# seqan/slimm

Hardware: AMD Instinct MI355X
Metric: M alignment-records/sec -> final profile (higher is better)
Workload: dtype u32

## Files before the change

include/slimm_hip.h:

```cpp
#ifndef SLIMM_HIP_H
#define SLIMM_HIP_H

#include <stddef.h>
#include <stdint.h>

#ifdef __cplusplus
extern "C" {
#endif

#define SLIMM_LINEAGE_LEN 8

enum {
    SLIMM_OK = 0,
    SLIMM_E_INVALID = -1,
    SLIMM_E_HIP = -2,
    SLIMM_E_REF_RANGE = -3,
    SLIMM_E_RUN_LENGTH = -4,
    SLIMM_E_KEY_COLLISION = -5,
    SLIMM_E_REGROUP = -6,
    SLIMM_E_SPLIT = -7,
    SLIMM_E_RETRY = 2,
    SLIMM_E_NO_HITS = 1
};

// ... 141 lines not shown
int slimm_write_abundance(slimm_ctx* ctx, const char** text, uint64_t* len);
int slimm_write_abundance_file(slimm_ctx* ctx, const char* path);

typedef struct {
    uint32_t hits_count, matches_count, uniq_matches_count, uniq_hits_count, uniq_matches_count2;
    uint32_t reference_count, matched_ref_length;
    uint32_t failed_by_cov, failed_by_uniq_cov, failed_by_min_read, n_valid;
    uint32_t bin_width, min_reads, avg_read_len;
    uint32_t profile_count, profile_failed;
    float coverage_cut_off, uniq_coverage_cut_off, expected_coverage;
    uint64_t n_records, n_targets;
    uint64_t total_bins;
} slimm_stats;
int slimm_get_stats(slimm_ctx* ctx, slimm_stats* out);

typedef struct {
    uint32_t* reads_count;
    uint32_t* uniq_reads_count;
    uint32_t* uniq_reads_count2;
    uint32_t* nbins;
    uint32_t* nz_cov;
    uint32_t* nz_uniq_cov;
    uint32_t* nz_uniq_cov2;
    uint8_t* valid;
    float* abundance;
    float* uniq_abundance;
} slimm_ref_columns;
int slimm_get_ref_columns(slimm_ctx* ctx, slimm_ref_columns* out);

int slimm_get_bins(slimm_ctx* ctx, int which, uint32_t* out);

int slimm_get_read_targets(slimm_ctx* ctx, uint32_t* ref, uint32_t* gbin, uint64_t cap, uint64_t* n);
int slimm_target_ref_bits(slimm_ctx* ctx);

int slimm_taxon_count_size(slimm_ctx* ctx, int stage, uint32_t* n);
int slimm_get_taxon_counts(slimm_ctx* ctx, int stage, uint32_t* taxid, uint32_t* count);
int slimm_children_pairs_size(slimm_ctx* ctx, int stage, uint64_t* n);
int slimm_get_children_pairs(slimm_ctx* ctx, int stage, uint32_t* taxid, uint32_t* ref);

int slimm_enable_kernel_timing(slimm_ctx* ctx, int on);
int slimm_time_only_kernel(slimm_ctx* ctx, const char* name);
int slimm_kernel_times(slimm_ctx* ctx, const char** names, double* ms, uint32_t* launches, uint32_t cap,
                       uint32_t* n, int reset);

int slimm_get_bucket_sampling(slimm_ctx* ctx, uint32_t out[6]);

int slimm_grouped_records(slimm_ctx* ctx, uint64_t* ident, uint32_t* ref, uint32_t* gbin, uint64_t cap, uint64_t* n);
void slimm_group_plan(uint64_t n_records, uint32_t* passes, uint32_t* width, uint32_t* bits, uint32_t* grid);

uint32_t slimm_host_avg_read_length(const uint32_t* l_seq, uint64_t n, uint32_t sample_size);
float slimm_host_quantile_cut_off(const float* v, uint32_t n, float q);
uint32_t slimm_host_bin_of(int32_t begin_pos, uint32_t avg_read_len, uint32_t ref_len, uint32_t bin_width);
uint32_t slimm_host_canonical_read_name(const char* name, uint32_t name_len, uint16_t flag, uint16_t* flag_out);
typedef struct slimm_q18_runs {
    uint64_t short_starts;
    uint64_t short_to_plain;
    int last_short;
} slimm_q18_runs;
void slimm_host_q18_note(slimm_q18_runs* q, int starts_run, int shortened);
int slimm_host_q18_regroup_needed(const slimm_q18_runs* q);
int slimm_get_q18_runs(slimm_ctx* ctx, uint64_t* short_starts, uint64_t* short_to_plain);
typedef struct slimm_record_filter {
    uint32_t min_mapq;
    uint32_t require_flags;
    uint32_t exclude_flags;
    uint32_t min_aligned;
// ... 59 lines not shown
```

slimm_amd/capi.py:

```python
from __future__ import annotations

import ctypes as C
import os

_HERE = os.path.dirname(os.path.abspath(__file__))
LIB_PATH = os.environ.get("SLIMM_HIP_LIB") or os.path.join(_HERE, "libslimm_hip.so")

OK = 0
E_INVALID = -1
E_HIP = -2
E_REF_RANGE = -3
E_RUN_LENGTH = -4
E_KEY_COLLISION = -5
E_REGROUP = -6
E_SPLIT = -7
E_RETRY = 2
E_NO_HITS = 1

ORDER_GROUPED = 0
ORDER_ANY = 1

PROPAGATION_INDEPENDENT = 0
PROPAGATION_DEPENDENT = 1
PROPAGATION_UNDECIDED = 2
# ... 98 lines not shown
    ("slimm_staging_buffers", C.c_int, [_P, C.c_uint32, C.c_uint64, C.POINTER(_P), C.POINTER(_P), C.POINTER(_P),
                                        C.POINTER(_P)]),
    ("slimm_push_staged_async", C.c_int, [_P, C.c_uint32, C.c_uint64]),
    ("slimm_staging_wait", C.c_int, [_P, C.c_uint32]),
    ("slimm_set_records_device", C.c_int, [_P, _P, _P, _P, _P, C.c_uint64]),
    ("slimm_analyze_alignments", C.c_int, [_P]),
    ("slimm_coverage_buffer", C.c_int, [_P, C.POINTER(_P), C.POINTER(C.c_uint64)]),
    ("slimm_prepare_summary", C.c_int, [_P, C.c_uint32]),
    ("slimm_keep_bins", C.c_int, [_P, C.c_int]),
    ("slimm_coverage_summary", C.c_int, [_P, C.POINTER(_P), C.POINTER(C.c_uint64)]),
    ("slimm_finish_coverage_merged", C.c_int, [_P, _P, C.c_uint32]),
    ("slimm_merge_summary_slices", C.c_int, [_P, _P, C.c_uint32, C.c_uint32, C.POINTER(_P), C.POINTER(C.c_uint64)]),
    ("slimm_finish_coverage_reduced", C.c_int, [_P]),
    ("slimm_finish_coverage", C.c_int, [_P]),
    ("slimm_set_coverage_columns", C.c_int, [_P, _P, _P, _P, _P, C.c_uint32, C.c_uint32]),
    ("slimm_filter_alignments", C.c_int, [_P]),
    ("slimm_dense_taxa", C.c_int, [_P, C.POINTER(C.c_uint32), C.POINTER(_P)]),
    ("slimm_get_partials", C.c_int, [_P, C.POINTER(Partials)]),
    ("slimm_set_partials", C.c_int, [_P, C.POINTER(Partials)]),
    ("slimm_partials_buffer", C.c_int, [_P, C.POINTER(_P), C.POINTER(C.c_uint64)]),
    ("slimm_install_merged_partials", C.c_int, [_P, C.POINTER(C.c_uint32)]),
    ("slimm_get_reads_lca_count", C.c_int, [_P]),
    ("slimm_get_propagation_order", C.c_int, [_P, C.POINTER(C.c_int), _P, C.c_uint32, C.POINTER(C.c_uint32)]),
    ("slimm_set_propagation_walk", C.c_int, [_P, C.c_int]),
    ("slimm_set_propagation_priority", C.c_int, [_P, _P, C.c_uint32]),
    ("slimm_get_profiles", C.c_int, [_P, C.c_char_p]),
    ("slimm_write_abundance", C.c_int, [_P, C.POINTER(C.c_char_p), C.POINTER(C.c_uint64)]),
    ("slimm_write_abundance_file", C.c_int, [_P, C.c_char_p]),
    ("slimm_get_stats", C.c_int, [_P, C.POINTER(Stats)]),
    ("slimm_get_ref_columns", C.c_int, [_P, C.POINTER(RefColumns)]),
    ("slimm_get_bins", C.c_int, [_P, C.c_int, _P]),
    ("slimm_get_read_targets", C.c_int, [_P, _P, _P, C.c_uint64, C.POINTER(C.c_uint64)]),
    ("slimm_target_ref_bits", C.c_int, [_P]),
    ("slimm_get_bucket_sampling", C.c_int, [_P, _P]),
    ("slimm_taxon_count_size", C.c_int, [_P, C.c_int, C.POINTER(C.c_uint32)]),
    ("slimm_get_taxon_counts", C.c_int, [_P, C.c_int, _P, _P]),
    ("slimm_children_pairs_size", C.c_int, [_P, C.c_int, C.POINTER(C.c_uint64)]),
    ("slimm_get_children_pairs", C.c_int, [_P, C.c_int, _P, _P]),
    ("slimm_enable_kernel_timing", C.c_int, [_P, C.c_int]),
    ("slimm_time_only_kernel", C.c_int, [_P, C.c_char_p]),
    ("slimm_kernel_times", C.c_int, [_P, C.POINTER(C.c_char_p), C.POINTER(C.c_double), C.POINTER(C.c_uint32),
                                     C.c_uint32, C.POINTER(C.c_uint32), C.c_int]),
    ("slimm_push_bam_bytes", C.c_int, [_P, _P, C.c_uint64, C.c_int, C.POINTER(C.c_uint64)]),
    ("slimm_push_bgzf_blocks", C.c_int, [_P, _P, C.c_uint64, C.c_uint32, C.c_int, C.POINTER(C.c_uint64)]),
    ("slimm_push_sam_bytes", C.c_int, [_P, _P, C.c_uint64, C.c_int, C.POINTER(C.c_uint64)]),
    ("slimm_push_bgzf_sam_blocks", C.c_int, [_P, _P, C.c_uint64, C.c_uint32, C.c_int, C.POINTER(C.c_uint64)]),
    ("slimm_push_bzip2_sam_bytes", C.c_int, [_P, _P, C.c_uint64, C.c_uint32, C.c_int, C.POINTER(C.c_uint64)]),
    ("slimm_push_gzip_sam_bytes", C.c_int, [_P, _P, C.c_uint64, C.c_uint32, C.c_int, C.POINTER(C.c_uint64)]),
    ("slimm_get_gzip_stats", C.c_int, [_P, C.POINTER(C.c_uint64)]),
    ("slimm_push_zstd_sam_bytes", C.c_int, [_P, _P, C.c_uint64, C.c_uint32, C.c_int, C.POINTER(C.c_uint64)]),
    ("slimm_get_zstd_stats", C.c_int, [_P, C.POINTER(C.c_uint64)]),
    ("slimm_push_xz_sam_bytes", C.c_int, [_P, _P, C.c_uint64, C.c_uint32, C.c_int, C.POINTER(C.c_uint64)]),
    ("slimm_get_xz_stats", C.c_int, [_P, C.POINTER(C.c_uint64)]),
    ("slimm_set_reference_names", C.c_int, [_P, C.POINTER(C.c_char_p)]),
    ("slimm_bgzf_inflate", C.c_int, [C.c_int, _P, C.c_uint64, _P, C.c_uint64, C.POINTER(C.c_uint64), C.POINTER(C.c_double), C.c_char_p, C.c_uint64]),
    ("slimm_bgzf_inflate_with", C.c_int, [C.c_int, _P, C.c_uint64, _P, C.c_uint64, C.POINTER(C.c_uint64), C.POINTER(C.c_double), C.c_char_p,
                                          C.c_uint64, C.c_uint32, C.POINTER(C.c_uint32)]),
    ("slimm_partition_by_key", C.c_int, [C.c_int, _P, _P, _P, _P, _P, C.c_uint64, C.c_uint32, _P, _P, _P, _P, _P, _P, C.POINTER(C.c_double),
                                         C.c_char_p, C.c_uint64]),
    ("slimm_records_device", C.c_int, [_P, _P, _P, _P, _P, C.POINTER(C.c_uint64), C.POINTER(C.c_int)]),
    ("slimm_pin_host_buffer", C.c_int, [_P, _P, C.c_uint64]),
    ("slimm_set_input_size_hint", C.c_int, [_P, C.c_uint64]),
    ("slimm_window_memory", C.c_int, [_P, C.POINTER(C.c_uint64)]),
    ("slimm_device_memory", C.c_int, [_P, C.POINTER(C.c_uint64), C.POINTER(C.c_uint64)]),
    ("slimm_group_plan", None, [C.c_uint64, C.POINTER(C.c_uint32), C.POINTER(C.c_uint32), C.POINTER(C.c_uint32),
                                C.POINTER(C.c_uint32)]),
# ... 56 lines not shown
```

slimm_amd/csrc/context.h:

```cpp
#pragma once
#include <cerrno>
#include <fcntl.h>
#include <hip/hip_runtime.h>
#include <unistd.h>

#include <algorithm>
#include <cstdarg>
#include <cstdio>
#include <cstdlib>
#include <chrono>
#include <cstring>
#include <functional>
#include <memory>
#include <string>
#include <vector>

#include "../../include/slimm_hip.h"
#include "host_profile.hpp"
#include "force.h"
#include "bzip2_block.h"
#include "deflate_stream.h"
#include "zstd_walk.h"
#include "xz_walk.h"
#include "kernels.h"
#include "read_identity.h"

namespace slimm {



extern thread_local std::string g_create_error;

template <typename T>
struct DevBuf {
    T* p = nullptr;
    size_t cap = 0;
    ~DevBuf() { release(); }
    void release() {
        if (p) (void)hipFree(p);
        p = nullptr;
        cap = 0;
    }
    hipError_t ensure(size_t n) {
        if (n <= cap) return hipSuccess;
        release();
        hipError_t e = hipMalloc(reinterpret_cast<void**>(&p), n * sizeof(T));
        if (e == hipSuccess) cap = n;
        return e;
    }
    hipError_t ensure_later(size_t n, std::vector<void*>& old) {
        return n <= cap ? hipSuccess : grow_keeping(n, 0, 0, nullptr, false, &old);
    }
    hipError_t grow_keeping(size_t n, size_t from, size_t count, hipStream_t st, bool sync, std::vector<void*>* old) {
        DevBuf<T> nb;
        hipError_t e = nb.ensure(n);
        if (e == hipSuccess && count) e = hipMemcpyAsync(nb.p + from, p + from, count * sizeof(T), hipMemcpyDeviceToDevice, st);
        if (e == hipSuccess && sync) e = hipStreamSynchronize(st);
// ... 57 lines not shown
    bool copy_pending = false;
    bool filter_pending = false;
    bool stream_ordered = false;
    struct Staging {
        PinBuf<uint64_t> key;
        PinBuf<int32_t> ref, pos;
        PinBuf<uint16_t> flag;
        hipEvent_t done = nullptr;
        bool pending = false;
    } staging[2];

    uint32_t R = 0, T = 0;
    TileBucketing tiles;
    uint64_t Bp() const { return tiles.layout.Bp; }
    bool use_tiles() const { return tiles.plan.use_tiles; }
    std::vector<uint32_t> bin_off_h;

    DevBuf<uint32_t> d_ref_len, d_bin_off, d_lin_dense;
    DevBuf<uint2> d_geo;
    DevBuf<uint8_t> d_valid;
    DevBuf<uint4> d_rows16;
    DevBuf<uint32_t> d_level_taxon;
    DevBuf<uint32_t> d_taxon_off, d_taxon_idx;
    uint32_t taxon_shift = 0;
    uint32_t Tsel = 0;
    PinBuf<uint4> h_rows16;
    DevBuf<uint32_t> d_valid_bits;
    PinBuf<uint32_t> h_valid_bits;
    std::vector<uint32_t> valid_bits_prev;
    bool rows16_base_ready = false;
    std::vector<uint32_t> rows16_prev;
    bool use_rows16 = false;
    bool ref16 = false;
    DevBuf<uint64_t> in_key;
    DevBuf<int32_t> in_ref, in_pos;
    DevBuf<uint16_t> in_flag;
    DevBuf<uint32_t> in_check;
    bool has_check = false;
    bool packed = false;
    bool marked = false;
    WindowPipeline win;
    std::vector<slimm_ctx*> filter_peers;
    DeviceRecords rec;
    bool borrowed = false;
    uint64_t n_pushed = 0;
    DevBuf<uint64_t> c_ident, s_ident;
    DevBuf<uint2> c_pay, s_pay;
    DevBuf<uint32_t> group_hist, c_chk, s_chk;
    DevBuf<uint32_t> tgt_ref, tgt_gbin;
    TargetRefs target_refs() const { return TargetRefs{tgt_ref.p, ref16}; }
    DevBuf<uint4> slots;
    bool keep_bins = true;
    bool binsA_stored = false, binsB_stored = false;
    DevBuf<uint32_t> sel;
    DevBuf<uint32_t> filter_redo;
    DevBuf<uint32_t> slot_rbase, slot_bbase;
    hipStream_t side_stream = nullptr;
    hipEvent_t front_done = nullptr, prefix_done = nullptr;
    bool prefix_pending = false;
    uint32_t summary_slices = 0;
    bool summary_has_bits = false;
    uint32_t summary_layout = 0xffffffffu;
    DevBuf<uint32_t> d_sum_vec;
    uint32_t slice_tiles() const { return summary_slices > 1 ? (tiles.layout.ntiles + summary_slices - 1) / summary_slices : tiles.layout.ntiles; }
    uint64_t slice_words() const { return static_cast<uint64_t>(slice_tiles()) * (tiles.layout.tile_bins() / 32); }
    uint64_t summary_words() const { return 4ull * R + 16 + 2ull * std::max<uint32_t>(summary_slices, 1u) * slice_words(); }
    BitsLayout bits_layout() {
        BitsLayout b;
        if (summary_has_bits) {
            b.base = reinterpret_cast<uint64_t*>(summary.p + 4ull * R + 16);
            b.tps = slice_tiles();
            b.slice_w64 = slice_words() / 2;
        }
        return b;
    }
    bool statsA_final = false;
    bool bins_exposed = false;
    DevBuf<uint32_t> bins;
    DevBuf<uint32_t> counters;
    DevBuf<uint32_t> ref_stats;
    DevBuf<uint32_t> summary;
    DevBuf<uint32_t> lca_count, marks;
    DevBuf<uint32_t> d_partials;
// ... 117 lines not shown
```

slimm_amd/csrc/context.hip:

```cpp
#define SLIMM_RF_HOST_API
#include "context.h"

namespace slimm {

thread_local std::string g_create_error;
const char* kKernelNames[K_COUNT] = {"memset_bins", "k_group_count", "k_group_scan", "k_group_scatter", "k_group_finish",
                                     "k_front", "k_hist", "k_ref_stats", "k_filter", "k_ref_stats2",
                                     "k_tile_count", "k_tile_scan", "k_tile_scatter", "k_tile_hist",
                                     "k_tile_count2", "k_tile_scan2", "k_tile_scatter2", "k_tile_hist2",
                                     "k_pack", "k_pack2"};

int fail(slimm_ctx* c, int code, const char* fmt, ...) {
    char buf[512];
    va_list ap;
    va_start(ap, fmt);
    vsnprintf(buf, sizeof(buf), fmt, ap);
    va_end(ap);
    if (c)
        c->err = buf;
    else
        g_create_error = buf;
    return code;
}



void drain_events(slimm_ctx* c) {
    bool unrecorded = false;
    for (auto& e : c->ev_used) {
        float ms = 0.f;
        if (hipEventSynchronize(e.b) == hipSuccess && hipEventElapsedTime(&ms, e.a, e.b) == hipSuccess) {
            c->k_ms[e.id] += ms;
            c->k_n[e.id] += 1;
        } else {
            unrecorded = true;
        }
        c->ev_free.push_back(e);
    }
    c->ev_used.clear();
    if (unrecorded) (void)hipGetLastError();
}

int ensure_work_buffers(slimm_ctx* c, uint32_t n) {
    HIP_TRY(c, c->tgt_ref.ensure(n + 1));
    HIP_TRY(c, c->tgt_gbin.ensure(n + 8));
    HIP_TRY(c, c->slots.ensure(front_slots(n) + 1));
    HIP_TRY(c, c->sel.ensure(n + 8));
    HIP_TRY(c, c->slot_rbase.ensure(front_slots(n) + 8));
    HIP_TRY(c, c->slot_bbase.ensure(front_slots(n) / 1024 + 8));
    HIP_TRY(c, c->filter_redo.ensure(front_slots(n) + 1));
    HIP_TRY(c, c->tiles.reserve(n));
    if (c->order == SLIMM_ORDER_ANY) {
        HIP_TRY(c, c->c_ident.ensure(n + 1));
        HIP_TRY(c, c->c_pay.ensure(n + 1));
        HIP_TRY(c, c->s_ident.ensure(n + 1));
        HIP_TRY(c, c->s_pay.ensure(n + 1));
        HIP_TRY(c, c->group_hist.ensure(group_hist_words(group_plan(n))));
        if (c->rec.check) {
            HIP_TRY(c, c->c_chk.ensure(n + 1));
            HIP_TRY(c, c->s_chk.ensure(n + 1));
        }
    }
    return SLIMM_OK;
}

int ensure_pair_table(slimm_ctx* c, uint32_t cap) {
    if (cap <= c->pair_cap) return SLIMM_OK;
    HIP_TRY(c, c->pair_tab.ensure(cap));
    HIP_TRY(c, c->pair_list.ensure(cap / 2 + 1));
    HIP_TRY(c, c->h_pairs.ensure(cap / 2 + 1));
    c->pair_cap = cap;
    return SLIMM_OK;
}



int check_device_errors(slimm_ctx* c, uint32_t err) {
// ... 60 lines not shown
    c->host.reset(new HostProfile(hc));
    c->R = cfg->n_refs;
    c->T = c->host->n_taxa_dense();
    c->device = cfg->device;
    c->order = cfg->record_order;
    c->bin_off_h.resize(c->R + 1);
    uint64_t off = 0;
    for (uint32_t r = 0; r < c->R; ++r) {
        c->bin_off_h[r] = static_cast<uint32_t>(off);
        off += (static_cast<uint64_t>(c->host->nbins()[r]) + 3) & ~3ull;
        if (off >= kMaxBins) return fail(nullptr, SLIMM_E_INVALID, "more than 2^31 coverage bins; use a larger bin width");
    }
    c->bin_off_h[c->R] = static_cast<uint32_t>(off);
    {
        long r16 = 1;
        (void)forced("ref16", &r16);
        c->ref16 = c->R <= kRef16Max && r16 != 0;
    }
    {
        c->use_rows16 = c->host->rows16_ok() && !forced("wide_rows");
        c->Tsel = c->T;
        if (c->use_rows16) {
            const uint32_t* loff = c->host->level_offset();
            uint32_t widest = 1;
            for (int l = 0; l < 8; ++l) widest = std::max(widest, loff[l + 1] - loff[l]);
            c->taxon_shift = 0;
            while ((1u << c->taxon_shift) < widest) ++c->taxon_shift;
            c->Tsel = 8u << c->taxon_shift;
        }
    }
    const TileForces forces = TileForces::from_env();
    const TileLayout& tl = c->tiles.layout = tile_layout(off, c->Tsel, forces.tile_shift);
    if (tl.Bp + tl.Tpad >= kMaxBins) return fail(nullptr, SLIMM_E_INVALID, "more than 2^31 coverage bins; use a larger bin width");

    if (c->device >= 0) {
        slimm_ctx* cc = c.get();
        int ndev = 0;
        hipError_t e = hipGetDeviceCount(&ndev);
        if (e != hipSuccess || ndev == 0)
            return fail(nullptr, SLIMM_E_HIP, "no HIP device available (%s)", hipGetErrorString(e));
        if (c->device >= ndev) return fail(nullptr, SLIMM_E_INVALID, "device %d out of range (%d devices)", c->device, ndev);
#define HIP_TRY0(expr)                                                                                   \
    do {                                                                                                 \
        hipError_t e_ = (expr);                                                                          \
        if (e_ != hipSuccess) return fail(nullptr, SLIMM_E_HIP, "%s: %s", #expr, hipGetErrorString(e_)); \
    } while (0)
        HostTrace trc("slimm_create");
        HIP_TRY0(hipSetDevice(c->device));
        HIP_TRY0(hipStreamCreateWithFlags(&cc->stream, hipStreamNonBlocking));
        HIP_TRY0(hipEventCreateWithFlags(&cc->front_done, hipEventDisableTiming));
        HIP_TRY0(hipEventCreateWithFlags(&cc->prefix_done, hipEventDisableTiming));
        HIP_TRY0(hipEventCreateWithFlags(&cc->copy_done, hipEventDisableTiming));
        for (auto& sg : cc->staging) HIP_TRY0(hipEventCreateWithFlags(&sg.done, hipEventDisableTiming));
        trc.mark("streams + events");
        HIP_TRY0(cc->d_ref_len.ensure(c->R));
        HIP_TRY0(cc->d_bin_off.ensure(c->R + 1));
        HIP_TRY0(cc->d_lin_dense.ensure(static_cast<size_t>(c->R) * 8));
        HIP_TRY0(cc->d_valid.ensure(c->R));
        HIP_TRY0(cc->d_valid_bits.ensure(c->R / 32 + 2));
        HIP_TRY0(cc->h_valid_bits.ensure(c->R / 32 + 2));
        memset(cc->h_valid_bits.p, 0, (c->R / 32 + 2) * 4);
        HIP_TRY0(cc->bins.ensure(3 * tl.Bp + kTailWords + tl.Tpad));
        HIP_TRY0(cc->counters.ensure(CNT_WORDS));
        HIP_TRY0(cc->ref_stats.ensure(c->statsA_words() + c->statsB_words() + 64));
        HIP_TRY0(cc->lca_count.ensure(c->Tsel));
        HIP_TRY0(cc->marks.ensure(static_cast<size_t>(c->R) * (kMarkBytes / 4)));
        trc.mark("device arrays");
        HIP_TRY0(cc->h_stats.ensure(c->statsA_words() + c->statsB_words() + 64));
        HIP_TRY0(cc->h_small.ensure(CNT_WORDS + kTailWords));
        HIP_TRY0(cc->h_lca.ensure(c->T));
        HIP_TRY0(cc->h_marks.ensure(c->R));
        trc.mark("page-locked host arrays");
        HIP_TRY0(hipMemcpy(cc->d_ref_len.p, hc.ref_len.data(), c->R * 4, hipMemcpyHostToDevice));
        HIP_TRY0(hipMemcpy(cc->d_bin_off.p, c->bin_off_h.data(), (c->R + 1) * 4, hipMemcpyHostToDevice));
        {
            std::vector<uint2> geo(c->R);
            for (uint32_t i = 0; i < c->R; ++i) geo[i] = make_uint2(hc.ref_len[i], static_cast<uint32_t>(c->bin_off_h[i]));
            HIP_TRY0(cc->d_geo.ensure(c->R));
            HIP_TRY0(hipMemcpy(cc->d_geo.p, geo.data(), c->R * sizeof(uint2), hipMemcpyHostToDevice));
        }
        HIP_TRY0(hipMemcpy(cc->d_lin_dense.p, c->host->lineage_dense().data(), static_cast<size_t>(c->R) * 32,
                           hipMemcpyHostToDevice));
#undef HIP_TRY0
        if (cc->use_rows16) {
            const std::vector<uint32_t>& lt = c->host->level_taxon();
            const uint32_t* off = c->host->level_offset();
            std::vector<uint32_t> flat(static_cast<size_t>(8) << cc->taxon_shift, 0u);
            std::vector<uint32_t> inv_off(c->T + 1, 0u), inv_idx;
            for (int l = 0; l < 8; ++l)
                for (uint32_t i = off[l]; i < off[l + 1]; ++i) {
                    flat[(static_cast<size_t>(i - off[l]) << 3) | static_cast<size_t>(l)] = lt[i];
                    if (lt[i] < c->T) ++inv_off[lt[i] + 1];
                }
// ... 222 lines not shown
            {
                KernelTimer t(c, K_GROUP_SCAN);
                launch_group_scan(st, j, pass);
            }
            {
                KernelTimer t(c, K_GROUP_SCATTER);
                launch_group_scatter(st, j, pass);
            }
        }
        {
            KernelTimer t(c, K_GROUP_FINISH);
            launch_group_finish(st, j);
        }
        {
            KernelTimer t(c, K_FRONT);
            launch_front_sorted(st, n, c->c_ident.p, c->c_pay.p, c->counters.p, c->target_refs(), c->tgt_gbin.p, c->slots.p,
                                c->rec.check ? c->c_chk.p : nullptr);
        }
    } else {
        KernelTimer t(c, K_FRONT, true);
        launch_front_raw(st, c->rec, c->R, c->d_geo.p, half_read, hc.bin_width, c->counters.p, c->target_refs(), c->tgt_gbin.p,
                         c->slots.p, t.t0(), t.t1());
    }
    auto slot_prefix_beside_what_follows = [&]() -> int {
        HIP_TRY(c, need_stream(c->side_stream));
        HIP_TRY(c, hipEventRecord(c->front_done, st));
        HIP_TRY(c, hipStreamWaitEvent(c->side_stream, c->front_done, 0));
        launch_slot_read_prefix(c->side_stream, c->slots.p, nslots, c->slot_rbase.p, c->slot_bbase.p);
        HIP_TRY(c, hipEventRecord(c->prefix_done, c->side_stream));
        return SLIMM_OK;
    };
    if (c->use_tiles()) {
        job.values.vals = c->tgt_gbin.p;
        job.values.slots = c->slots.p;
        job.values.nslots = nslots;
        job.n_upper = n;
        job.a = c->cov();
        job.b = c->ucov();
        job.tail = c->tail();
        job.stats = c->ref_stats.p;
        job.store_from = c->keep_bins ? 0u : c->tiles.layout.ntiles;
        bucket(c, job);
        if (int rc = slot_prefix_beside_what_follows()) return rc;
        c->summary_has_bits = false;
        if (c->summary_slices) {
            const bool fresh = c->summary.cap < c->summary_words() || c->summary_layout != c->summary_slices;
            HIP_TRY(c, c->summary.ensure(c->summary_words()));
            if (fresh)
                HIP_TRY(c, hipMemsetAsync(c->summary.p, 0, c->summary_words() * 4, st));
            c->summary_layout = c->summary_slices;
            c->summary_has_bits = true;
        }
        job.bits = c->bits_layout();
        histogram(c, job);
        c->binsA_stored = c->keep_bins;
    } else {
        if (int rc = slot_prefix_beside_what_follows()) return rc;
        KernelTimer t(c, K_HIST);
        launch_hist(st, c->tgt_gbin.p, c->slots.p, nslots, c->counters.p, c->tail(), c->cov(), c->ucov(),
                    c->order != SLIMM_ORDER_ANY);
        c->binsA_stored = true;
    }
    c->prefix_pending = true;
    HIP_TRY(c, hipGetLastError());
    c->analyzed = true;
    tr.mark("phase A launches");
    return SLIMM_OK;
}

int slimm_get_stream(slimm_ctx* c, void** hip_stream) {
    if (!c || !hip_stream) return SLIMM_E_INVALID;
    if (c->device < 0) return fail(c, SLIMM_E_INVALID, "host-only context has no stream");
    *hip_stream = c->stream;
    return SLIMM_OK;
}

int slimm_set_stream_ordered(slimm_ctx* c, int on) {
    if (!c) return SLIMM_E_INVALID;
    c->stream_ordered = on != 0;
    return SLIMM_OK;
}

int slimm_coverage_buffer(slimm_ctx* c, void** d_ptr, uint64_t* n_words) {
    if (!c || !d_ptr || !n_words) return SLIMM_E_INVALID;
    if (!c->analyzed) return fail(c, SLIMM_E_INVALID, "call slimm_analyze_alignments first");
    if (!c->binsA_stored) return fail(c, SLIMM_E_INVALID, "the coverage arrays were not kept (slimm_keep_bins)");
    (void)hipSetDevice(c->device);
    if (!c->stream_ordered) HIP_TRY(c, hipStreamSynchronize(c->stream));
    c->bins_exposed = true;
    *d_ptr = c->bins.p;
    *n_words = 2 * c->Bp() + 16;
    return SLIMM_OK;
}
// ... 217 lines not shown
    const uint32_t R = c->R, T = c->T;
    uint32_t* const blockB = c->ref_stats.p + c->statsA_words();
    TileJob job;
    job.run = c->tiles.run(TilePhase::B, c->local_M, c->rec.n);
    {
        KernelTimer t(c, K_MEMSET);
        if (!c->use_tiles()) HIP_TRY(c, hipMemsetAsync(c->ucov2(), 0, c->Bp() * sizeof(uint32_t), st));
        ZeroArgs z;
        z.p[0] = c->marks.p;
        z.n[0] = R * (kMarkBytes / 4);
        z.p[1] = c->counters.p + CNT_ERR;
        z.n[1] = 3;
        if (c->use_tiles()) {
            z.p[2] = blockB;
            z.n[2] = 4 * R;
            c->tiles.zero_tables(z, job.run);
        } else {
            z.p[2] = c->lca_count.p;
            z.n[2] = c->Tsel;
        }
        if (!c->pair_clean) {
            z.p64 = c->pair_tab.p;
            z.n64 = c->pair_cap;
        }
        if (copy_rows) {
            z.cp_dst = reinterpret_cast<uint32_t*>(c->d_rows16.p);
            z.cp_src = reinterpret_cast<const uint32_t*>(c->h_rows16.p);
            z.cp_n = R * 4u;
        }
        z.cp2_dst = c->d_valid_bits.p;
        z.cp2_src = c->h_valid_bits.p;
        z.cp2_n = R / 32u + 1u;
        launch_zero(st, z);
    }
    const uint32_t nslots = front_slots(c->rec.n);
    HIP_TRY(c, hipStreamWaitEvent(st, c->prefix_done, 0));
    c->prefix_pending = false;
    {
        KernelTimer t(c, K_FILTER, true);
        FilterArgs fa;
        fa.tgt_ref = c->target_refs();
        fa.tgt_gbin = c->tgt_gbin.p;
        fa.slots = c->slots.p;
        fa.nslots = nslots;
        if (c->use_rows16) {
            fa.rows16 = c->d_rows16.p;
            fa.taxon_flat = c->d_level_taxon.p;
            fa.taxon_shift = c->taxon_shift;
        } else {
            fa.lin_dense = c->d_lin_dense.p;
            fa.valid = c->d_valid.p;
        }
        fa.valid_bits = c->d_valid_bits.p;
        fa.redo = c->filter_redo.p;
        fa.sel = c->sel.p;
        fa.slot_rbase = c->slot_rbase.p;
        fa.slot_bbase = c->slot_bbase.p;
        fa.marks = c->marks.p;
        fa.pair_tab = c->pair_tab.p;
        fa.pair_list = c->pair_list.p;
        fa.pair_mask = c->pair_cap - 1;
        fa.taxon_base = static_cast<uint32_t>(c->Bp());
        fa.counters = c->counters.p;
        launch_filter(st, fa, t.t0(), t.t1());
    }
    if (c->use_tiles()) {
        job.values.vals = c->sel.p;
        job.values.nslots = c->local_M;
        job.n_upper = c->rec.n;
        job.a = c->ucov2();
        job.stats = blockB;
        job.store_from = c->keep_bins ? 0u : c->tiles.layout.ntiles;
        bucket(c, job);
        histogram(c, job);
    } else {
        KernelTimer t(c, K_HIST);
        launch_sel_atomics(st, c->sel.p, c->local_M, static_cast<uint32_t>(c->Bp()), c->ucov2(), c->lca_count.p);
    }
    {
        PackArgs pk;
        pk.src[0] = c->counters.p;
        pk.n[0] = 32;
        pk.src[1] = c->marks.p;
        pk.n[1] = R;
        pk.reps[1] = kPackBytes8;
        pk.src[2] = c->use_tiles() ? c->lca_tiles() : c->lca_count.p;
        pk.n[2] = T;
        if (c->use_rows16) {
            pk.sum_k = 2;
            pk.sum_off = c->d_taxon_off.p;
            pk.sum_idx = c->d_taxon_idx.p;
        }
        if (c->use_tiles()) {
            KernelTimer t(c, K_PACK2);
            const TileTables tt = c->tiles.tables(c->counters.p);
            TILES(tt.tile_shift, launch_pack(st, blockB + 4ull * R, pk, &tt, c->ucov2(), nullptr, c->d_bin_off.p, R, blockB));
        } else {
            KernelTimer t(c, K_REF_STATS2);
            launch_ref_stats(st, c->ucov2(), nullptr, c->d_bin_off.p, R, blockB, &pk);
        }
// ... 314 lines not shown
    if (!c || !out || which < 0 || which > 2) return SLIMM_E_INVALID;
    if (c->device < 0 || !c->analyzed) return fail(c, SLIMM_E_INVALID, "no coverage bins on this context");
    if (which == 2 && !c->filtered) return fail(c, SLIMM_E_INVALID, "uniq_cov2 needs slimm_filter_alignments");
    if (which < 2 ? !c->binsA_stored : !c->binsB_stored)
        return fail(c, SLIMM_E_INVALID, "the coverage arrays were not kept (slimm_keep_bins)");
    (void)hipSetDevice(c->device);
    const uint32_t* src = which == 0 ? c->cov() : which == 1 ? c->ucov() : c->ucov2();
    std::vector<uint32_t> padded(c->Bp());
    HIP_TRY(c, hipMemcpyAsync(padded.data(), src, c->Bp() * 4, hipMemcpyDeviceToHost, c->stream));
    HIP_TRY(c, hipStreamSynchronize(c->stream));
    uint64_t k = 0;
    for (uint32_t r = 0; r < c->R; ++r) {
        uint32_t nb = c->host->nbins()[r];
        memcpy(out + k, padded.data() + c->bin_off_h[r], static_cast<size_t>(nb) * 4);
        k += nb;
    }
    return SLIMM_OK;
}

int slimm_get_read_targets(slimm_ctx* c, uint32_t* ref, uint32_t* gbin, uint64_t cap, uint64_t* n) {
    if (!c || !n) return SLIMM_E_INVALID;
    if (c->device < 0 || !c->analyzed) return fail(c, SLIMM_E_INVALID, "no targets on this context (call slimm_analyze_alignments)");
    (void)hipSetDevice(c->device);
    const uint32_t ns = front_slots(c->rec.n);
    std::vector<uint4> sl(ns);
    if (ns) HIP_TRY(c, hipMemcpyAsync(sl.data(), c->slots.p, ns * sizeof(uint4), hipMemcpyDeviceToHost, c->stream));
    HIP_TRY(c, hipStreamSynchronize(c->stream));
    uint64_t total = 0;
    for (const uint4& d : sl) total += d.y;
    *n = total;
    if (!ref && !gbin) return SLIMM_OK;
    if (cap < total) return fail(c, SLIMM_E_INVALID, "slimm_get_read_targets: %llu entries, room for %llu",
                                 static_cast<unsigned long long>(total), static_cast<unsigned long long>(cap));
    std::vector<uint16_t> ref16(ref && c->ref16 ? total : 0);
    uint64_t o = 0;
    for (const uint4& d : sl) {
        if (!d.y) continue;
        if (ref && c->ref16)
            HIP_TRY(c, hipMemcpyAsync(ref16.data() + o, reinterpret_cast<const uint16_t*>(c->tgt_ref.p) + d.x, d.y * 2ull,
                                      hipMemcpyDeviceToHost, c->stream));
        else if (ref)
            HIP_TRY(c, hipMemcpyAsync(ref + o, c->tgt_ref.p + d.x, d.y * 4ull, hipMemcpyDeviceToHost, c->stream));
        if (gbin) HIP_TRY(c, hipMemcpyAsync(gbin + o, c->tgt_gbin.p + d.x, d.y * 4ull, hipMemcpyDeviceToHost, c->stream));
        o += d.y;
    }
    HIP_TRY(c, hipStreamSynchronize(c->stream));
    if (ref && c->ref16)
        for (uint64_t k = 0; k < total; ++k) ref[k] = (ref16[k] & 0x7fffu) | ((ref16[k] & 0x8000u) << 16);
    return SLIMM_OK;
}

int slimm_target_ref_bits(slimm_ctx* c) { return c ? (c->ref16 ? 16 : 32) : SLIMM_E_INVALID; }

int slimm_get_bucket_sampling(slimm_ctx* c, uint32_t out[6]) {
    if (!c || !out) return SLIMM_E_INVALID;
    uint32_t cnt[CNT_WORDS] = {0};
    for (int i = 0; i < 6; ++i) out[i] = 0;
    if (c->device < 0) return SLIMM_OK;
    HIP_TRY(c, hipSetDevice(c->device));
    HIP_TRY(c, hipStreamSynchronize(c->stream));
    if (c->counters.p) HIP_TRY(c, hipMemcpy(cnt, c->counters.p, sizeof(cnt), hipMemcpyDeviceToHost));
    for (int ph = 0; ph < 2; ++ph) {
        const uint32_t S = c->use_tiles() ? c->tiles.sampled[ph] : 0u;
        out[3 * ph] = S;
        out[3 * ph + 1] = S > 1 ? cnt[CNT_FALLBACK + ph] : 0u;
        out[3 * ph + 2] = S > 1 ? cnt[CNT_PEAK + ph] : 0u;
    }
    return SLIMM_OK;
}

int slimm_taxon_count_size(slimm_ctx* c, int stage, uint32_t* n) {
    if (!c || !n) return SLIMM_E_INVALID;
    if (!c->counted) return fail(c, SLIMM_E_INVALID, "call slimm_get_reads_lca_count first");
    std::vector<uint32_t> t, k;
    c->host->taxon_counts(stage, t, k);
    *n = static_cast<uint32_t>(t.size());
    return SLIMM_OK;
}

int slimm_get_taxon_counts(slimm_ctx* c, int stage, uint32_t* taxid, uint32_t* count) {
    if (!c || !taxid || !count) return SLIMM_E_INVALID;
    if (!c->counted) return fail(c, SLIMM_E_INVALID, "call slimm_get_reads_lca_count first");
    std::vector<uint32_t> t, k;
    c->host->taxon_counts(stage, t, k);
    memcpy(taxid, t.data(), t.size() * 4);
// ... 164 lines not shown
```

slimm_amd/csrc/front.hip:

```cpp
#include <hip/hip_runtime.h>
#include <hip/hip_ext.h>
#include <stdint.h>

#include <algorithm>
#include <cstdlib>

#include "kernels.h"

namespace slimm {

#if defined(EXP) && EXP == 11
__device__ unsigned long long g_prof_f[4 * 8192];
#define FPROF_T(x) const unsigned long long x = __builtin_readcyclecounter()
#define FPROF_ADD(slot, a, b) if (threadIdx.x == 0) atomicAdd(&g_prof_f[(blockIdx.x & 8191u) * 4 + slot], (b) - (a))
#else
#define FPROF_T(x)
#define FPROF_ADD(slot, a, b)
#endif

namespace {

constexpr uint32_t kTagShift = 26;
constexpr uint32_t kRefField = (1u << kTagShift) - 1u;
constexpr uint32_t kNoMatch = 0xffffffffu;
// ... 290 lines not shown
        o.mapped = w.b != 0xffffffffu;
        if (o.mapped && w.b >= n_refs) {
            bad = true;
            o.mapped = false;
        }
        o.ref = w.b;
        o.aux = w.c;
        return o;
    }
    __device__ FrontRec rec(uint32_t i, bool& bad) const { return decode(raw(i), bad); }
    __device__ uint2 geo_of(const FrontRaw3& w) const { return geo[w.b < n_refs ? w.b : 0u]; }
    __device__ uint32_t gbin(const FrontRec& r, const uint2& g) const { return g.y + div_bin_width(min(r.aux + half_read, g.x)); }
};

namespace {

struct WinOut {
    uint32_t base;
    uint32_t nf, nh, nv;
};

struct Staged {
    uint32_t mate, ref, gbin;
    bool mapped;
};

#ifndef SLIMM_HASH_WALK
#define SLIMM_HASH_WALK 32
#endif
constexpr uint32_t kHashWalk = SLIMM_HASH_WALK;
static_assert(kHashWalk == 16 || kHashWalk == 24 || kHashWalk == 32 || kHashWalk == 48,
              "the threshold is one of the distances window_fast's doubling chain knows");

template <typename RefT>
__device__ __forceinline__ void window_fast(uint32_t field, uint32_t gbin, uint32_t lane, uint64_t SS, uint64_t V, uint64_t PR,
                                            WinOut& so, RefT* __restrict__ tgt_ref, uint32_t* __restrict__ tgt_gbin,
                                            uint32_t* tab) {
    const uint32_t T = (f_rank(SS >> 1) << kTagShift) | field;
    const uint64_t N0 = SS ^ PR;
    const uint64_t E2 = N0 & (N0 << 1), E4 = E2 & (E2 << 2), E8 = E4 & (E4 << 4), E12 = E8 & (E8 << 4), E16 = E8 & (E8 << 8);
    const uint64_t E24 = E16 & (E16 << 8), E32 = E16 & (E16 << 16), E48 = E32 & (E32 << 16);
    uint64_t F;
    if ((kHashWalk == 16 ? E16 : kHashWalk == 24 ? E24 : kHashWalk == 32 ? E32 : E48) != 0ull) {
        hash_clear(tab, lane);
        bool overflow = false;
        F = f_ballot(hash_first(tab, T, lane, f_bit(V), overflow));
    } else {
        const uint32_t x1 = f_shr1z(T) ^ T;
        uint32_t x = x1, differ = x1;
        const auto walk = [&](int steps) {
#pragma unroll
            for (int u = 0; u < steps; ++u) {
                x = f_shr1z(x) ^ x1;
                differ = min(differ, x);
            }
        };
        if (E2) {
            walk(2);
            if (E4) {
                walk(4);
                if (E8) {
                    walk(4);
                    if (E12) {
                        walk(4);
                        if (kHashWalk > 16 && E16) {
                            walk(8);
                            if (kHashWalk > 24 && E24) {
                                walk(8);
                                if (kHashWalk > 32 && E32) walk(16);
                            }
                        }
                    }
                }
            }
        }
        F = f_ballot(differ != 0u) & V;
    }
    const uint64_t H = f_first_after(SS, V, SS >> 1);
    const uint64_t Fr = __builtin_bitreverse64(F), Gr = __builtin_bitreverse64(F & ~H);
    const uint64_t U = H & ~__builtin_bitreverse64((~Fr + (Gr << 1)) & Fr);
    const bool uniq = f_bit(U);
    if (f_bit(F)) {
        const uint32_t p = so.base + so.nf + f_rank(F);
        tgt_ref[p] = static_cast<RefT>((field - 1u) + f_head_bit<RefT>(f_bit(H)));
        tgt_gbin[p] = gbin | (uniq ? 0x80000000u : 0u);
    }
    so.nf += static_cast<uint32_t>(__popcll(F));
    so.nh += static_cast<uint32_t>(__popcll(H));
    so.nv += static_cast<uint32_t>(__popcll(V));
}

template <typename RefT>
__device__ __forceinline__ void window_general(const Staged& rec, uint32_t lane, uint64_t RS, uint64_t V, uint32_t X,
                                               WinOut& so, RefT* __restrict__ tgt_ref,
                                               uint32_t* __restrict__ tgt_gbin) {
    const bool in_pr = lane < X;
    const bool use = f_bit(V);
    const uint64_t le = (2ull << lane) - 1ull;
    const uint32_t run_from = 63u - static_cast<uint32_t>(__builtin_clzll((RS & le) | 1ull));
    const uint64_t above = RS & ~le;
    const uint32_t run_to = above ? static_cast<uint32_t>(__builtin_ctzll(above)) : X;
    const uint32_t W = use ? ((rec.mate << 28) | rec.ref) : (0xc0000000u | lane);
    const uint32_t back = in_pr ? lane - run_from : 0u;
    bool dup = false, mate_seen = false;
    for (uint32_t d = 1; f_ballot(back >= d) != 0ull; ++d) {
        const uint32_t o = __shfl(W, static_cast<int>((lane - d) & 63u), 64);
        const bool mine = back >= d;
        dup = dup || (mine && o == W);
        mate_seen = mate_seen || (mine && (o >> 28) == (W >> 28));
    }
    const bool first = use && !dup;
    const bool head = use && !mate_seen;
    const uint32_t WF = first ? (W >> 28) : 3u;
    const uint32_t span = in_pr ? run_to - run_from : 0u;
    uint32_t smaller = 0, same_before = 0, same_total = 0;
    for (uint32_t d = 0; f_ballot(span > d) != 0ull; ++d) {
        const uint32_t j = run_from + d;
        const uint32_t o = __shfl(WF, static_cast<int>(j & 63u), 64);
        const bool mine = span > d && o != 3u && first;
        smaller += (mine && o < WF) ? 1u : 0u;
        same_total += (mine && o == WF) ? 1u : 0u;
        same_before += (mine && o == WF && j < lane) ? 1u : 0u;
    }
    const uint64_t F = f_ballot(first);
    const uint64_t H = f_ballot(head);
    if (first) {
        const uint32_t before_run = static_cast<uint32_t>(__popcll(F & ((1ull << run_from) - 1ull)));
        const uint32_t p = so.base + so.nf + before_run + smaller + same_before;
        tgt_ref[p] = static_cast<RefT>(rec.ref | f_head_bit<RefT>(head));
        tgt_gbin[p] = rec.gbin | ((head && same_total == 1u) ? 0x80000000u : 0u);
    }
    so.nf += static_cast<uint32_t>(__popcll(F));
    so.nh += static_cast<uint32_t>(__popcll(H));
    so.nv += static_cast<uint32_t>(__popcll(V));
}

template <bool kChk, typename Acc, typename RefT>
__device__ __forceinline__ uint32_t long_run(const Acc& acc, uint32_t pos, uint32_t N, uint32_t lane, WinOut& so,
                                          RefT* __restrict__ tgt_ref, uint32_t* __restrict__ tgt_gbin, bool& bad,
                                          bool& collide, uint32_t* tab) {
    uint32_t klo0, khi0;
    acc.key_at(pos, klo0, khi0);
    uint32_t end = pos;
    bool decreasing = false;
    uint32_t last_mate = 0;
    while (true) {
        const uint32_t i = end + lane;
        const bool live = i < N;
        bool b = false;
        const bool mine = acc.same_run(live ? i : N - 1u, pos, klo0, khi0);
        const FrontRec r = acc.rec(live ? i : N - 1u, b);
        const uint64_t same = f_ballot(live && mine);
        if (kChk) collide = collide | (live && mine && acc.check[i] != acc.check[pos]);
        const uint32_t n_same = static_cast<uint32_t>(__builtin_ctzll(~same | (1ull << 63)));
        const bool whole = (~same) == 0ull;
        const uint32_t n_in = whole ? 64u : n_same;
        const uint32_t mprev = f_shr1(r.mate, last_mate);
        decreasing = decreasing || (f_ballot(r.mate < mprev) & f_below(n_in)) != 0ull;
        if (n_in) last_mate = __builtin_amdgcn_readlane(r.mate, n_in - 1u);
        end += n_in;
        if (!whole) break;
    }
    const WinOut so_at_run = so;
    bool hashed = true;
    uint32_t nv_run;
    bool again;
    do {
        again = false;
        so = so_at_run;
        nv_run = 0;
// ... 24 lines not shown
                        uint32_t Ts = T;
                        for (uint32_t d = 1; d < 64u; ++d) {
                            Ts = f_shr1(Ts, kNoMatch);
                            differ = min(differ, Ts ^ T);
                        }
                    }
                    for (uint32_t eb = pos; eb < cb; eb += 64u) {
                        bool b = false;
                        const FrontRec e = acc.rec(eb + lane, b);
                        uint32_t Te = e.mapped ? ((e.mate << 28) | e.ref) : 0xe0000000u;
                        for (uint32_t d = 0; d < 64u; ++d) {
                            differ = min(differ, Te ^ T);
                            Te = f_ror1(Te);
                        }
                    }
                    first = use && differ != 0u;
                }
                const uint64_t F = f_ballot(first);
                uint64_t H = 0;
#pragma unroll
                for (uint32_t m = 0; m < 3u; ++m) {
                    const uint64_t Vm = f_ballot(use && r.mate == m);
                    if (Vm && !((head_seen >> m) & 1u)) {
                        H |= 1ull << __builtin_ctzll(Vm);
                        head_seen |= 1u << m;
                    }
                    n_first[m] += static_cast<uint32_t>(__popcll(f_ballot(first && r.mate == m)));
                }
                const bool head = f_bit(H);
                const uint32_t p = so.base + so.nf + f_rank(F);
                const FrontRaw3 rw{0u, first ? r.ref : 0u, 0u};
                const uint32_t g = first ? acc.gbin(r, acc.geo_of(rw)) : 0u;
                if (first) {
                    tgt_ref[p] = static_cast<RefT>(r.ref | f_head_bit<RefT>(head));
                    if (!head) tgt_gbin[p] = g;
                }
                uint64_t Hm = H;
                while (Hm) {
                    const uint32_t hl = static_cast<uint32_t>(__builtin_ctzll(Hm));
                    Hm &= Hm - 1ull;
                    const uint32_t m = __builtin_amdgcn_readlane(r.mate, hl);
                    head_p[m] = __builtin_amdgcn_readlane(p, hl);
                    head_g[m] = __builtin_amdgcn_readlane(g, hl);
                }
                so.nf += static_cast<uint32_t>(__popcll(F));
                so.nh += static_cast<uint32_t>(__popcll(H));
            }
            if (!again) {
#pragma unroll
                for (uint32_t m = 0; m < 3u; ++m)
                    if (((head_seen >> m) & 1u) && lane == 0u)
                        tgt_gbin[head_p[m]] = head_g[m] | (n_first[m] == 1u ? 0x80000000u : 0u);
            }
        }
    } while (again);
    so.nv += nv_run;
    return end;
}

constexpr uint32_t kStageRecs = 64u * kSlotBlocks;
constexpr uint32_t kStageGroup = 6;

__device__ __forceinline__ uint32_t next_run_start(const uint32_t* st1, uint32_t lane, uint32_t from) {
    for (uint32_t o = from; o < kStageRecs; o += 64u) {
        const uint32_t i = o + lane;
        const uint32_t w = i < kStageRecs ? st1[i] : 0u;
        const uint64_t m = f_ballot(static_cast<int32_t>(w) < 0);
        if (m) return o + static_cast<uint32_t>(__builtin_ctzll(m));
    }
    return kStageRecs;
}

template <typename RefT>
__device__ __forceinline__ bool long_run_staged(const uint32_t* st1, const uint32_t* st2, uint32_t off, uint32_t end_off,
                                                uint32_t lane, WinOut& so, RefT* __restrict__ tgt_ref,
                                                uint32_t* __restrict__ tgt_gbin, uint32_t* tab) {
    const WinOut so_at_run = so;
    {
        uint32_t head_seen = 0, last_mate = 0, nv = 0;
        uint32_t n_first[3] = {0u, 0u, 0u}, head_p[3] = {0u, 0u, 0u}, head_g[3] = {0u, 0u, 0u};
        bool falls = false;
        hash_clear(tab, lane);
        for (uint32_t o = off; o < end_off; o += 64u) {
            const uint32_t i = o + lane;
            const uint32_t n_in = min(64u, end_off - o);
            const uint32_t at = min(i, end_off - 1u);
            const uint32_t w1 = st1[at], g = st2[at];
            const uint32_t field = w1 & kRefField, mate = (w1 >> kStMateShift) & 3u;
            const uint64_t IN = f_below_nz(n_in);
            if ((f_ballot(mate < f_shr1(mate, last_mate)) & IN) != 0ull) {
                falls = true;
                break;
            }
            last_mate = __builtin_amdgcn_readlane(mate, n_in - 1u);
            const uint64_t V = f_ballot(field != kRefField) & IN;
            bool overflow = false;
            const bool first = hash_first(tab, (mate << 28) | field, i - off, f_bit(V), overflow);
            if (f_ballot(overflow) != 0ull) {
                so = so_at_run;
                return false;
            }
            const uint64_t F = f_ballot(first);
            const uint64_t M1 = f_ballot(mate == 1u), M2 = f_ballot(mate == 2u);
            const uint64_t Mm[3] = {~(M1 | M2), M1, M2};
            uint64_t H = 0;
#pragma unroll
            for (uint32_t m = 0; m < 3u; ++m) {
                const uint64_t Vm = V & Mm[m];
                if (Vm && !((head_seen >> m) & 1u)) {
                    H |= Vm & (0ull - Vm);
                    head_seen |= 1u << m;
                }
                n_first[m] += static_cast<uint32_t>(__popcll(F & Mm[m]));
            }
            const bool head = f_bit(H);
            const uint32_t p = so.base + so.nf + f_rank(F);
            if (first) {
                tgt_ref[p] = static_cast<RefT>((field - 1u) | f_head_bit<RefT>(head));
                if (!head) tgt_gbin[p] = g;
            }
            uint64_t Hm = H;
            while (Hm) {
                const uint32_t hl = static_cast<uint32_t>(__builtin_ctzll(Hm));
                Hm &= Hm - 1ull;
                const uint32_t m = __builtin_amdgcn_readlane(mate, hl);
                head_p[m] = __builtin_amdgcn_readlane(p, hl);
                head_g[m] = __builtin_amdgcn_readlane(g, hl);
            }
            nv += static_cast<uint32_t>(__popcll(V));
            so.nf += static_cast<uint32_t>(__popcll(F));
            so.nh += static_cast<uint32_t>(__popcll(H));
        }
        if (!falls) {
#pragma unroll
            for (uint32_t m = 0; m < 3u; ++m)
                if (((head_seen >> m) & 1u) && lane == 0u) tgt_gbin[head_p[m]] = head_g[m] | (n_first[m] == 1u ? 0x80000000u : 0u);
            so.nv += nv;
            return true;
        }
        so = so_at_run;
    }
    const bool decreasing = true;
    uint32_t nv_run = 0;
    for (uint32_t pass = 0; pass < 3u; ++pass) {
        uint32_t head_seen = 0;
        uint32_t n_first[3] = {0u, 0u, 0u};
        uint32_t head_p[3] = {0u, 0u, 0u}, head_g[3] = {0u, 0u, 0u};
        hash_clear(tab, lane);
        for (uint32_t o = off; o < end_off; o += 64u) {
            const uint32_t i = o + lane;
            const bool in_run = i < end_off;
            const uint32_t w1 = st1[in_run ? i : end_off - 1u], g = st2[in_run ? i : end_off - 1u];
            const uint32_t field = w1 & kRefField, mate = (w1 >> kStMateShift) & 3u;
            const bool mapped = in_run && field != kRefField;
            const bool use = mapped && (!decreasing || mate == pass);
            if (pass == 0) nv_run += static_cast<uint32_t>(__popcll(f_ballot(mapped)));
            bool overflow = false;
            const bool first = hash_first(tab, (mate << 28) | field, i - off, use, overflow);
            if (f_ballot(overflow) != 0ull) {
                so = so_at_run;
                return false;
            }
            const uint64_t F = f_ballot(first);
            uint64_t H = 0;
#pragma unroll
            for (uint32_t m = 0; m < 3u; ++m) {
                const uint64_t Vm = f_ballot(use && mate == m);
                if (Vm && !((head_seen >> m) & 1u)) {
                    H |= 1ull << __builtin_ctzll(Vm);
                    head_seen |= 1u << m;
                }
                n_first[m] += static_cast<uint32_t>(__popcll(f_ballot(first && mate == m)));
            }
            const bool head = f_bit(H);
            const uint32_t p = so.base + so.nf + f_rank(F);
            if (first) {
                tgt_ref[p] = static_cast<RefT>((field - 1u) | f_head_bit<RefT>(head));
                if (!head) tgt_gbin[p] = g;
            }
            uint64_t Hm = H;
            while (Hm) {
                const uint32_t hl = static_cast<uint32_t>(__builtin_ctzll(Hm));
                Hm &= Hm - 1ull;
                const uint32_t m = __builtin_amdgcn_readlane(mate, hl);
                head_p[m] = __builtin_amdgcn_readlane(p, hl);
                head_g[m] = __builtin_amdgcn_readlane(g, hl);
            }
            so.nf += static_cast<uint32_t>(__popcll(F));
            so.nh += static_cast<uint32_t>(__popcll(H));
        }
#pragma unroll
        for (uint32_t m = 0; m < 3u; ++m)
            if (((head_seen >> m) & 1u) && lane == 0u) tgt_gbin[head_p[m]] = head_g[m] | (n_first[m] == 1u ? 0x80000000u : 0u);
    }
    so.nv += nv_run;
    return true;
}

template <bool kClamp, bool kChk, typename Acc>
__device__ __forceinline__ void stage_slot(const Acc& acc, uint32_t B, uint32_t N, uint32_t lane, uint32_t* st1, uint32_t* st2,
                                           bool& bad, bool& collide) {
    uint32_t worst = 0;
    uint32_t plo = 0, phi = 0, q0lo = 0, q0hi = 0, q0chk = 0, pchk = 0;
    if (!Acc::kMarked) {
        const uint32_t pb = B > 0u ? B - 1u : 0u;
        uint32_t rel = (B == 0u && lane != 0u) ? lane - 1u : lane;
        if (kClamp) rel = min(rel, N - 1u - pb);
        acc.load_key(pb, rel, q0lo, q0hi);
        if (kChk) q0chk = acc.load_check(pb, rel);
    }
#pragma unroll
    for (uint32_t j0 = 0; j0 < kSlotBlocks; j0 += kStageGroup) {
        FrontLoaded rec[kStageGroup];
        uint2 geo[kStageGroup];
        uint32_t chk[kStageGroup];
#pragma unroll
        for (uint32_t u = 0; u < kStageGroup; ++u) {
            if (j0 + u >= kSlotBlocks) break;
            const uint32_t blk = kClamp ? min(B + 64u * (j0 + u), N - 1u) : B + 64u * (j0 + u);
            acc.load(blk, kClamp ? min(lane, N - 1u - blk) : lane, rec[u]);
            chk[u] = kChk ? acc.load_check(blk, kClamp ? min(lane, N - 1u - blk) : lane) : 0u;
        }
        __builtin_amdgcn_sched_barrier(0);
#pragma unroll
        for (uint32_t u = 0; u < kStageGroup; ++u) {
            if (j0 + u >= kSlotBlocks) break;
// ... 20 lines not shown
                if (B == 0u && lane == 0u) Acc::no_key(qlo, qhi);
            } else {
                qlo = f_shr1(rec[u].klo, plo);
                qhi = f_shr1(rec[u].khi, phi);
                qchk = kChk ? f_shr1(chk[u], pchk) : 0u;
            }
            const uint64_t q = (static_cast<uint64_t>(qhi) << 32) | qlo;
            if (kChk) {
                bool here = (k == q) & (chk[u] != qchk);
                if (kClamp) here = here & (64u * j + lane < N - B);
                collide = collide | here;
                pchk = static_cast<uint32_t>(__builtin_amdgcn_readlane(chk[u], 63));
            }
            bool starts;
            if constexpr (Acc::kMarked)
                starts = Acc::starts_run(rec[u]) || (B == 0u && j == 0u && lane == 0u);
            else
                starts = k != q;
            uint32_t w = field | (mate << kStMateShift) | (starts ? kStRunStart : 0u);
            if (kClamp && 64u * j + lane >= N - B) w = kRefField;
            st1[64u * j + lane] = w;
            st2[64u * j + lane] = g;
            if (!Acc::kMarked) {
                plo = static_cast<uint32_t>(__builtin_amdgcn_readlane(rec[u].klo, 63));
                phi = static_cast<uint32_t>(__builtin_amdgcn_readlane(rec[u].khi, 63));
            }
        }
    }
    bad = bad | acc.out_of_range(worst);
}

}

template <typename Acc, bool kChk, typename RefT>
__global__ __launch_bounds__(kFrontBlock, 4) void k_front(const Acc acc, uint32_t nslots, uint32_t* __restrict__ counters,
                                                       RefT* __restrict__ tgt_ref, uint32_t* __restrict__ tgt_gbin,
                                                       uint4* __restrict__ slots) {
    __shared__ uint32_t s_stage[kFrontBlock / 64][2][kStageRecs];
    __shared__ __attribute__((aligned(16))) uint32_t s_tab[kFrontBlock / 64][2 * kHashSlots];
    const uint32_t N = acc.count(counters);
    const uint32_t lane = f_lane();
    const uint32_t wave = __builtin_amdgcn_readfirstlane(threadIdx.x >> 6);
    uint32_t* const st1 = s_stage[wave][0];
    uint32_t* const st2 = s_stage[wave][1];
    uint32_t* const tab = s_tab[wave];
    bool bad = false, collide = false;
    const uint32_t slot = blockIdx.x * (kFrontBlock / 64) + wave;
    if (slot < nslots) {
        const uint32_t B = slot * kSlotRecs;
        WinOut so{B, 0u, 0u, 0u};
        FPROF_T(f0);
        if (B < N) {
            if (N - B >= kStageRecs)
                stage_slot<false, kChk>(acc, B, N, lane, st1, st2, bad, collide);
            else
                stage_slot<true, kChk>(acc, B, N, lane, st1, st2, bad, collide);
            __builtin_amdgcn_s_waitcnt(0x0f70);
            FPROF_T(f1);
            FPROF_ADD(0, f0, f1);
            uint32_t off = next_run_start(st1, lane, 0u);
            so.base = B + min(off, kSlotRecs);
            const uint32_t lim = min(kSlotRecs, N - B);
            const uint32_t* const st1_lane = st1 + lane;
            const uint32_t* const st2_lane = st2 + lane;
            while (off < lim) {
                while (static_cast<int32_t>(off) <= static_cast<int32_t>(lim) - 64) {
                    const uint32_t w1 = st1_lane[off], w2 = st2_lane[off];
                    const uint64_t RSw = f_ballot(static_cast<int32_t>(w1) < 0);
                    const uint32_t lead = static_cast<uint32_t>(__builtin_clzll(RSw));
                    if (lead == 63u) break;
                    const uint32_t X = 63u - lead;
                    const uint64_t PR = (~0ull >> 1) >> lead;
                    const uint32_t field = w1 & kRefField, mate = (w1 >> kStMateShift) & 3u, mprev = f_shr1z(mate);
                    if ((f_ballot(mate < mprev) & ~RSw & PR) != 0ull) break;
                    window_fast(field, w2, lane, (RSw | f_ballot(mate != mprev)) & PR, f_ballot(field != kRefField) & PR, PR, so, tgt_ref,
                                tgt_gbin, tab);
                    off += X;
                }
                if (off >= lim) break;
                const uint32_t w1 = st1[off + lane], w2 = st2[off + lane];
                const uint64_t RSw = f_ballot(static_cast<int32_t>(w1) < 0);
                const uint32_t pos = B + off;
                uint32_t X = pos + 64u >= N ? N - pos : 63u - static_cast<uint32_t>(__builtin_clzll(RSw | 1ull));
                if (kSlotRecs - off < 64u) {
                    const uint64_t beyond = RSw & ~f_below(kSlotRecs - off);
                    if (beyond) X = min(X, static_cast<uint32_t>(__builtin_ctzll(beyond)));
                }
                if (X) {
                    const uint32_t field = w1 & kRefField, mate = (w1 >> kStMateShift) & 3u;
                    const uint64_t PR = f_below_nz(X);
                    const uint64_t RS = RSw & PR;
                    const uint32_t mprev = f_shr1z(mate);
                    const uint64_t V = f_ballot(field != kRefField) & PR;
                    if ((f_ballot(mate < mprev) & ~RS & PR) == 0ull) {
                        window_fast(field, w2, lane, (RS | f_ballot(mate != mprev)) & PR, V, PR, so, tgt_ref, tgt_gbin, tab);
                    } else {
                        window_general<RefT>(Staged{mate, field - 1u, w2, f_bit(V)}, lane, RS, V, X, so, tgt_ref, tgt_gbin);
                    }
                    off += X;
                } else {
                    FPROF_T(l0);
                    const uint32_t end_off = next_run_start(st1, lane, off + 64u);
                    if (end_off < kStageRecs && long_run_staged(st1, st2, off, end_off, lane, so, tgt_ref, tgt_gbin, tab)) {
                        off = end_off;
                    } else {
                        const uint32_t end = long_run<kChk, Acc, RefT>(acc, pos, N, lane, so, tgt_ref, tgt_gbin, bad, collide, tab);
                        __builtin_amdgcn_s_waitcnt(0x0f70);
                        off = end - B < kStageRecs ? next_run_start(st1, lane, end - B) : kStageRecs;
                    }
                    FPROF_T(l1);
                    FPROF_ADD(3, l0, l1);
                }
            }
        }
        FPROF_T(f2);
        FPROF_ADD(1, f0, f2);
        FPROF_ADD(2, f2, f2 + 1ull);
        if (lane == 0u) slots[slot] = make_uint4(so.base, so.nf, so.nh, so.nv);
    }
    if (__any(bad) && lane == 0u) atomicOr(&counters[CNT_ERR], static_cast<uint32_t>(ERR_REF_RANGE));
    if (kChk && __any(collide) && lane == 0u) atomicOr(&counters[CNT_ERR], static_cast<uint32_t>(ERR_KEY_COLLISION));
}

uint32_t front_slots(uint32_t n_records) { return (n_records + kSlotRecs - 1u) / kSlotRecs; }

static uint32_t front_grid(uint32_t nslots) {
    const uint32_t blocks = (nslots + (kFrontBlock / 64) - 1u) / (kFrontBlock / 64);
    return std::max(1u, blocks);
}

template <typename Acc, bool kChk>
static void front_launch(hipStream_t st, const Acc& a, uint32_t ns, uint32_t* counters, TargetRefs tgt_ref, uint32_t* tgt_gbin,
                         uint4* slots, hipEvent_t t0, hipEvent_t t1) {
    if (tgt_ref.ref16)
        hipExtLaunchKernelGGL((k_front<Acc, kChk, uint16_t>), dim3(front_grid(ns)), dim3(kFrontBlock), 0, st, t0, t1, 0, a, ns,
                              counters, static_cast<uint16_t*>(tgt_ref.p), tgt_gbin, slots);
    else
        hipExtLaunchKernelGGL((k_front<Acc, kChk, uint32_t>), dim3(front_grid(ns)), dim3(kFrontBlock), 0, st, t0, t1, 0, a, ns,
                              counters, static_cast<uint32_t*>(tgt_ref.p), tgt_gbin, slots);
}

void launch_front_raw(hipStream_t st, const DeviceRecords& in, uint32_t n_refs, const uint2* geo, uint32_t half_read,
                      uint32_t bin_width, uint32_t* counters, TargetRefs tgt_ref, uint32_t* tgt_gbin, uint4* slots,
                      hipEvent_t t0, hipEvent_t t1) {
    const uint32_t ns = front_slots(in.n);
    if (!ns) return;
    FrontRawT<false> a;
    a.key = in.key;
    a.ref = in.ref;
    a.pos = in.pos;
    a.flag = in.flag;
    a.check = in.check;
    a.geo = geo;
    a.n = in.n;
    a.n_refs = n_refs;
    a.half_read = half_read;
    a.bin_width = bin_width;
    a.bw_magic = bin_width ? 0xffffffffu / bin_width : 0u;
    if (in.marked) {
        FrontMarked m;
        m.word = reinterpret_cast<const uint32_t*>(in.ref);
        m.pos = in.pos;
        m.geo = geo;
        m.n = in.n;
        m.n_refs = n_refs;
        m.half_read = half_read;
        m.bin_width = bin_width;
        m.bw_magic = a.bw_magic;
        front_launch<FrontMarked, false>(st, m, ns, counters, tgt_ref, tgt_gbin, slots, t0, t1);
    } else if (in.packed) {
        FrontPacked b;
// ... 37 lines not shown
```

slimm_amd/csrc/kernels.h:

```cpp
#pragma once
#include <hip/hip_runtime.h>
#include <stdint.h>

#include <string>
#include <vector>

#include "record_filter.h"
#include "tile_plan.h"

#if defined(__HIP_DEVICE_COMPILE__)
#define SLIMM_PIN_VGPR(x) asm volatile("" : "+v"(x))
#else
#define SLIMM_PIN_VGPR(x) (void)(x)
#endif

namespace slimm {

enum {
    CNT_V = 0,
    CNT_M = 1,
    CNT_P = 2,
    CNT_ERR = 3,
    CNT_PAIRS = 4,
    CNT_REDO = 5,
// ... 50 lines not shown
constexpr uint32_t kMarkBytes = 8;
struct ZeroArgs {
    uint32_t* p[5] = {nullptr, nullptr, nullptr, nullptr, nullptr};
    uint32_t n[5] = {0, 0, 0, 0, 0};
    uint64_t* p64 = nullptr;
    uint32_t n64 = 0;
    uint32_t* cp_dst = nullptr;
    const uint32_t* cp_src = nullptr;
    uint32_t cp_n = 0;
    uint32_t* cp2_dst = nullptr;
    const uint32_t* cp2_src = nullptr;
    uint32_t cp2_n = 0;
};
void launch_zero(hipStream_t st, const ZeroArgs& z);
void launch_copy_out(hipStream_t st, uint32_t* dst_host, const uint32_t* src, uint32_t n);

struct DeviceRecords {
    const uint64_t* key = nullptr;
    const int32_t* ref = nullptr;
    const int32_t* pos = nullptr;
    const uint16_t* flag = nullptr;
    const uint32_t* check = nullptr;
    uint32_t n = 0;
    bool packed = false;
    bool marked = false;
};


constexpr uint32_t kSlotRecs = 768;
constexpr int kFrontBlock = 64;
constexpr uint32_t kMaxRefs = (1u << 26) - 2u;
constexpr uint32_t kMaxBins = 0x7ffffff0u;
constexpr uint32_t kRef16Max = 1u << 15;
struct TargetRefs {
    void* p = nullptr;
    bool ref16 = false;
};
uint32_t front_slots(uint32_t n_records);
void launch_front_raw(hipStream_t st, const DeviceRecords& in, uint32_t n_refs, const uint2* geo, uint32_t half_read,
                      uint32_t bin_width, uint32_t* counters, TargetRefs tgt_ref, uint32_t* tgt_gbin, uint4* slots,
                      hipEvent_t t0 = nullptr, hipEvent_t t1 = nullptr);
void launch_front_sorted(hipStream_t st, uint32_t n_upper, const uint64_t* ident, const uint2* pay,
                         uint32_t* counters, TargetRefs tgt_ref, uint32_t* tgt_gbin, uint4* slots,
                         const uint32_t* cchk = nullptr);

void launch_check_grouping(hipStream_t st, const uint64_t* key, uint32_t n, uint64_t id_mask, uint64_t* tab, uint32_t tab_mask,
                           uint32_t* n_split);
void launch_hist(hipStream_t st, const uint32_t* tgt_gbin, const uint4* slots, uint32_t nslots, uint32_t* counters,
                 uint32_t* tail, uint32_t* cov, uint32_t* ucov, bool count_mapped);
void launch_ref_stats(hipStream_t st, const uint32_t* a, const uint32_t* b, const uint32_t* bin_off, uint32_t n_refs,
                      uint32_t* out, const PackArgs* pack = nullptr);
struct FilterArgs {
    TargetRefs tgt_ref;
    const uint32_t* tgt_gbin = nullptr;
    const uint4* slots = nullptr;
    uint32_t nslots = 0;
    const void* rows16 = nullptr;
    const uint32_t* taxon_flat = nullptr;
    uint32_t taxon_shift = 0;
    const uint32_t* lin_dense = nullptr;
    const uint8_t* valid = nullptr;
    const uint32_t* valid_bits = nullptr;
    uint32_t* redo = nullptr;
    uint32_t* sel = nullptr;
    const uint32_t* slot_rbase = nullptr;
    const uint32_t* slot_bbase = nullptr;
    uint32_t* marks = nullptr;
    uint64_t* pair_tab = nullptr;
    uint64_t* pair_list = nullptr;
    uint32_t pair_mask = 0, taxon_base = 0;
    uint32_t* counters = nullptr;
};
void launch_filter(hipStream_t st, const FilterArgs& a, hipEvent_t t0 = nullptr, hipEvent_t t1 = nullptr);
void launch_sel_atomics(hipStream_t st, const uint32_t* sel, uint32_t n_reads, uint32_t taxon_base, uint32_t* ucov2,
                        uint32_t* lca_count);
void launch_slot_read_prefix(hipStream_t st, const uint4* slots, uint32_t nslots, uint32_t* rbase, uint32_t* bbase);
void launch_partials_pack(hipStream_t st, const uint32_t* block_b, uint32_t R, uint32_t T, uint32_t* out);
void launch_merge_slices(hipStream_t st, const uint32_t* recv, uint32_t n_ranks, uint64_t slice_words, uint32_t lo_bin,
                         uint32_t hi_bin, const uint32_t* bin_off, uint32_t n_refs, const uint32_t* own_stats,
                         const uint32_t* own_tail, uint32_t* vec);
void launch_nonzero_bits(hipStream_t st, const uint32_t* bins, uint64_t n_bins, uint32_t* bits);
void launch_merge_summary(hipStream_t st, const uint32_t* gathered, uint64_t rank_stride, uint32_t n_ranks,
                          const uint32_t* bin_off, uint32_t n_refs, uint64_t bits_off_cov, uint64_t bits_off_ucov,
                          uint32_t* out_stats, const uint32_t* counters);

struct SlotValues {
    const uint32_t* vals = nullptr;
    const uint4* slots = nullptr;
    uint32_t nslots = 0;
    bool per_read = false;
};
struct Totals {
    const uint4* part = nullptr;
    uint32_t nparts = 0;
    uint32_t* tail = nullptr;
};
constexpr uint32_t kCountFold = 2;
constexpr uint32_t kSuperTiles = 64;
constexpr uint32_t kMaxSuper = 8192;
constexpr uint32_t kPartSub = 32768;
struct BitsLayout {
    uint64_t* base = nullptr;
    uint32_t tps = 1;
    uint64_t slice_w64 = 0;
};
struct TileTables {
    uint32_t tile_shift;
    uint16_t* bucket;
    uint32_t *tile_count, *tile_base, *tile_cursor, *split_tiles;
    uint32_t reps, stride;
    uint4 *tile_items, *part_items;
    uint32_t *mid, *sup_cursor, *matrix;
    uint4* tot_part;
    const uint32_t* tile_ref0;
    uint32_t* counters;
    uint32_t entries;
};
struct TileSample {
    uint32_t stride = 1, k = 0;
    uint32_t flag = 0;
    bool gated = false;
};
namespace tiles13 {
// ... 118 lines not shown
```

slimm_amd/csrc/kernels.hip:

```cpp
#include <hip/hip_runtime.h>
#include <hip/hip_ext.h>
#include <stdint.h>

#include <algorithm>
#include <cstdlib>
#include <type_traits>

#include "kernels.h"

namespace slimm {

constexpr int kBlock = 256;
constexpr int kWaves = kBlock / 64;

__device__ __forceinline__ uint32_t lane_id() { return __builtin_amdgcn_mbcnt_hi(~0u, __builtin_amdgcn_mbcnt_lo(~0u, 0u)); }

__device__ __forceinline__ uint32_t mask_rank(uint64_t mask) {
    return __builtin_amdgcn_mbcnt_hi(static_cast<uint32_t>(mask >> 32),
                                     __builtin_amdgcn_mbcnt_lo(static_cast<uint32_t>(mask), 0u));
}

__device__ __forceinline__ uint32_t wave_sum(uint32_t v) {
#pragma unroll
    for (int o = 32; o > 0; o >>= 1) v += __shfl_xor(v, o, 64);
    return v;
}

__global__ __launch_bounds__(kBlock) void k_hist(const uint32_t* __restrict__ tgt_gbin, const uint4* __restrict__ slots,
                                                 uint32_t nslots, uint32_t* __restrict__ counters,
                                                 uint32_t* __restrict__ tail, uint32_t* __restrict__ cov,
                                                 uint32_t* __restrict__ ucov, int count_mapped) {
    __shared__ uint32_t s_tot[3];
    if (threadIdx.x < 3) s_tot[threadIdx.x] = 0;
    __syncthreads();
    const uint32_t lane = threadIdx.x & 63u;
    const uint32_t wave = (blockIdx.x * kBlock + threadIdx.x) >> 6, n_waves = (gridDim.x * kBlock) >> 6;
    uint32_t sum_f = 0, sum_h = 0, sum_v = 0;
    for (uint32_t s = wave; s < nslots; s += n_waves) {
        const uint4 d = slots[s];
        sum_f += d.y;
        sum_h += d.z;
        sum_v += d.w;
        for (uint32_t o = lane; o < d.y; o += 64u) {
            const uint32_t g = tgt_gbin[d.x + o];
            atomicAdd(&cov[g & 0x7fffffffu], 1u);
            if (g >> 31) atomicAdd(&ucov[g & 0x7fffffffu], 1u);
        }
    }
    if (lane == 0u) {
        atomicAdd(&s_tot[0], sum_v);
        atomicAdd(&s_tot[1], sum_h);
        atomicAdd(&s_tot[2], sum_f);
    }
    __syncthreads();
    if (threadIdx.x < 3 && s_tot[threadIdx.x]) {
        const int slot = threadIdx.x == 0 ? CNT_V : threadIdx.x == 1 ? CNT_M : CNT_P;
        if (threadIdx.x != 0 || count_mapped) atomicAdd(&counters[slot], s_tot[threadIdx.x]);
        if (tail) atomicAdd(&tail[threadIdx.x], s_tot[threadIdx.x]);
    }
}

__global__ __launch_bounds__(kBlock) void k_ref_stats(const uint32_t* __restrict__ a, const uint32_t* __restrict__ b,
                                                      const uint32_t* __restrict__ bin_off, uint32_t n_refs,
                                                      uint32_t* __restrict__ out, const PackArgs pack) {
    {
        const uint32_t gid = blockIdx.x * kBlock + threadIdx.x, gsz = gridDim.x * kBlock;
        uint32_t* dst = out + 4ull * n_refs;
#pragma unroll
        for (int k = 0; k < 4; ++k) {
            for (uint32_t i = gid; i < pack.n[k]; i += gsz) dst[i] = packed_word(pack, k, i);
            dst += pack.n[k];
        }
    }
    const uint32_t ref = (blockIdx.x * kBlock + threadIdx.x) >> 6;
    if (ref >= n_refs) return;
    const uint32_t lane = threadIdx.x & 63;
    const uint32_t s = bin_off[ref], e = bin_off[ref + 1];
    uint32_t sa = 0, za = 0, sb = 0, zb = 0;
    for (uint32_t i = s + lane * 4; i < e; i += 256) {
// ... 287 lines not shown
__device__ __forceinline__ void filter_q4(const Rows& rows, const FilterOut& out, uint32_t lane, uint32_t X, uint32_t w,
                                          const typename Rows::Row& row, uint64_t valid_lanes, uint32_t sel_base, uint64_t Q4) {
    const uint64_t PR = k_below(X);
    const uint64_t H = k_ballot((w >> TgtWord<RefT>::kShift) != 0u) & PR;
    const uint32_t ref = w & TgtWord<RefT>::kRefMask;
    const uint64_t VB = valid_lanes & PR;
    uint32_t f[8];
    Rows::fields(row, f);
    uint64_t todo = Q4;
    while (todo) {
        const uint32_t o = static_cast<uint32_t>(__builtin_ctzll(todo));
        todo &= todo - 1ull;
        const uint64_t later = H & ~k_below(o + 1u);
        const uint32_t nxt = later ? static_cast<uint32_t>(__builtin_ctzll(later)) : X;
        const uint64_t Vs = VB & k_below(nxt) & ~k_below(o);
        ReadAcc acc;
        read_clear(acc);
        read_max(acc, Vs, ref, f[7]);
        const uint32_t index = rows.taxon_index(7u, acc.max_f7);
        const uint32_t taxon = rows.taxon_at(index);
        read_children(out, k_bit(Vs), ref, 8u, taxon);
        if (lane == 0u) out.sel[sel_base + static_cast<uint32_t>(__popcll(H & k_below(o + 1u))) - 1u] = out.taxon_base + index;
    }
}

template <typename RefT, typename Rows>
__device__ __forceinline__ void filter_window_now(const Rows& rows, const FilterOut& out, uint32_t lane, uint32_t X, uint32_t w,
                                                  uint32_t g, const typename Rows::Row& row, uint32_t sel_base) {
    const uint64_t vb = k_ballot(Rows::valid(row));
    const Lookup lk = filter_window<RefT>(rows, out, lane, X, w, g, row, vb, sel_base);
    if (lk.q4) filter_q4<RefT>(rows, out, lane, X, w, row, vb, sel_base, lk.q4);
}

template <typename Rows, typename RefT>
__device__ __forceinline__ void filter_span(const Rows& rows, const FilterOut& out, const RefT* __restrict__ tgt_ref,
                                         const uint32_t* __restrict__ tgt_gbin, uint32_t lane, uint32_t pos, uint32_t endp,
                                         uint32_t sel_base) {
    using TW = TgtWord<RefT>;
    while (pos < endp) {
        const uint32_t n_live = min(64u, endp - pos);
        const bool live = lane < n_live;
        const uint32_t w = live ? tgt_ref[pos + lane] : 0u;
        const uint32_t g = live ? tgt_gbin[pos + lane] : 0u;
        const uint64_t HB = k_ballot((w >> TW::kShift) != 0u) & k_below(n_live);
        const uint32_t X = pos + 64u >= endp ? n_live : 63u - static_cast<uint32_t>(__builtin_clzll(HB | 1ull));
        if (X != 0u) {
            const typename Rows::Row row = rows.load(lane < X ? (w & TW::kRefMask) : 0u);
            filter_window_now<RefT>(rows, out, lane, X, w, g, row, sel_base);
            sel_base += static_cast<uint32_t>(__popcll(HB & k_below(X)));
            pos += X;
            continue;
        }
        ReadAcc acc;
        read_clear(acc);
        uint32_t e = pos;
        while (true) {
            const bool in = e + lane < endp;
            const uint32_t ww = in ? tgt_ref[e + lane] : TW::kHead;
            const uint32_t gg = in ? tgt_gbin[e + lane] : 0u;
            uint64_t heads = k_ballot((ww >> TW::kShift) != 0u);
            if (e == pos) heads &= ~1ull;
            const uint32_t n_in = heads ? static_cast<uint32_t>(__builtin_ctzll(heads)) : 64u;
            const uint32_t rr = ww & TW::kRefMask;
            const typename Rows::Row row = rows.load(lane < n_in ? rr : 0u);
            uint32_t f[8];
            Rows::fields(row, f);
            const uint64_t Vs = k_ballot(Rows::valid(row)) & k_below(n_in);
            read_add(acc, Vs, gg, f);
            read_max(acc, Vs, rr, f[7]);
            e += n_in;
            if (n_in < 64u) break;
        }
        uint32_t sel = 0xffffffffu;
        if (acc.nv == 1u) {
            sel = acc.first_g & 0x7fffffffu;
        } else if (acc.nv > 1u) {
            uint32_t lv, index;
            const uint32_t taxon = read_taxon(rows, acc, &lv, &index);
            sel = out.taxon_base + index;
            for (uint32_t c = pos; c < e; c += 64u) {
                const bool in = c + lane < e;
                const uint32_t rr = in ? (tgt_ref[c + lane] & TW::kRefMask) : 0u;
                const typename Rows::Row row = rows.load(rr);
                read_children(out, in && Rows::valid(row), rr, lv, taxon);
            }
        }
        if (lane == 0u) out.sel[sel_base] = sel;
        sel_base += 1u;
        pos = e;
    }
}

}

constexpr uint32_t kFcRing = 128;
constexpr uint32_t kFcReads = kSlotRecs + 8;
constexpr uint32_t kFcBatch = 4;

template <typename Rows, typename RefT>
struct FilterKernArgs {
    const RefT* tgt_ref;
    const uint32_t* tgt_gbin;
    const uint4* slots;
    const uint32_t* valid_bits;
    uint32_t* redo;
    uint32_t nslots;
    Rows rows;
    FilterOut out;
};
template <typename T, typename Args>
__device__ __forceinline__ T kernarg_now(const Args& args, size_t offset) {
    T v;
#if defined(__HIP_DEVICE_COMPILE__)
    const __attribute__((address_space(4))) char* p =
        (const __attribute__((address_space(4))) char*)__builtin_amdgcn_kernarg_segment_ptr();
    asm volatile("" : "+s"(p));
    __builtin_memcpy(&v, p + offset, sizeof(T));
#else
    memcpy(&v, reinterpret_cast<const char*>(&args) + offset, sizeof(T));
#endif
    return v;
}

template <typename Rows, typename RefT>
__device__ __forceinline__ void compact_window(const FilterKernArgs<Rows, RefT>& ka, uint32_t lane, uint32_t X, uint64_t Hc,
                                               uint32_t cref, uint32_t cg, uint32_t cr, const typename Rows::Row& row,
                                               uint32_t* __restrict__ s_sel) {
    using KA = FilterKernArgs<Rows, RefT>;
    const Rows& rows = ka.rows;
    const FilterOut& out = ka.out;
    const uint64_t PR = k_below(X);
    const uint64_t H = Hc & PR;
    const uint64_t stops = (H >> 1) | (1ull << (X - 1u));
    const uint64_t single = H & stops, OW = H & ~stops;
    if (k_bit(single)) s_sel[cr] = cg & 0x7fffffffu;
    if (OW) {
        const uint64_t le = (2ull << lane) - 1ull;
        const uint32_t fvl = 63u - static_cast<uint32_t>(__builtin_clzll((H & le) | 1ull));
        const typename Rows::Row first = Rows::from_lane(row, fvl << 2);
        bool ne[8];
        Rows::differ(row, first, ne);
        const uint64_t fvr = __builtin_bitreverse64(H), nfvr = ~fvr;
        auto owners_of = [&](uint64_t D) { return __builtin_bitreverse64((nfvr + __builtin_bitreverse64(D)) & fvr); };
        uint32_t lv = 8u;
#pragma unroll
        for (int l = 3; l >= 0; --l) {
            const uint64_t bad = owners_of(k_ballot(ne[l]) & PR);
            lv = k_bit(bad) ? lv : static_cast<uint32_t>(l);
        }
        if (k_ballot(lv == 8u) & OW) {
            uint32_t up = 8u;
#pragma unroll
            for (int l = 7; l >= 4; --l) {
                const uint64_t bad = owners_of(k_ballot(ne[l]) & PR);
                up = k_bit(bad) ? up : static_cast<uint32_t>(l);
            }
            lv = lv == 8u ? up : lv;
        }
        const uint64_t Q4 = k_ballot(lv == 8u) & OW;
        if (k_bit(OW & ~Q4)) s_sel[cr] = out.taxon_base + rows.taxon_index(lv & 7u, Rows::field(row, lv & 7u));
        const uint32_t lv_read = __builtin_amdgcn_ds_bpermute(fvl << 2, lv);
// ... 110 lines not shown
                    bu = u == k ? bits[k] : bu;
                }
                const bool live = tu + lane < tend;
                H = k_ballot(live && (wu >> TW::kShift) != 0u);
                VB = k_ballot(live && ((bu >> (wu & 31u)) & 1u) != 0u);
            }
            if (k_bit(VB)) {
                const uint32_t p = __builtin_amdgcn_mbcnt_hi(static_cast<uint32_t>(VB >> 32),
                                                             __builtin_amdgcn_mbcnt_lo(static_cast<uint32_t>(VB), ccount)) & (kFcRing - 1u);
                s_ref[p] = wu & TW::kRefMask;
                s_g[p] = gu;
                s_r[p] = __builtin_amdgcn_mbcnt_hi(static_cast<uint32_t>(H >> 32),
                                                   __builtin_amdgcn_mbcnt_lo(static_cast<uint32_t>(H), rcount - 1u)) + (k_bit(H) ? 1u : 0u);
            }
            rcount += static_cast<uint32_t>(__popcll(H));
            ccount += static_cast<uint32_t>(__popcll(VB));
            const bool last = tu + 64u >= tend;
            while (ccount - cdone >= 64u || (last && ccount != cdone)) {
                __builtin_amdgcn_wave_barrier();
                const uint32_t n_live = min(64u, ccount - cdone);
                const uint32_t e = (cdone + lane) & (kFcRing - 1u);
                const uint32_t cref = lane < n_live ? s_ref[e] : 0u;
                const uint32_t cg = s_g[e], cr = lane < n_live ? s_r[e] : 0xffffffffu;
                typename Rows::Row row = ka.rows.load(cref);
                const uint32_t before = __builtin_amdgcn_update_dpp(0xffffffffu, cr, 0x138, 0xf, 0xf, false);
                const uint64_t Hc = k_ballot(lane < n_live && (lane == 0u || cr != before));
                const bool final_window = last && ccount - cdone <= 64u;
                const uint32_t X = final_window ? n_live : 63u - static_cast<uint32_t>(__builtin_clzll(Hc));
                __builtin_amdgcn_wave_barrier();
                if (__builtin_expect(X == 0u, 0)) {
                    whole_reads_walk = true;
                    break;
                }
                compact_window(ka, lane, X, Hc, cref, cg, cr, row, s_sel);
                cdone += X;
            }
            if (__builtin_expect(whole_reads_walk, 0)) break;
        }
    }
    __builtin_amdgcn_wave_barrier();
    if (__builtin_expect(whole_reads_walk, 0)) {
        uint32_t* const redo = kernarg_now<uint32_t*>(ka, offsetof(KA, redo));
        uint32_t* const counters = kernarg_now<uint32_t*>(ka, offsetof(KA, out.counters));
        if (lane == 0u) redo[atomicAdd(&counters[CNT_REDO], 1u)] = slot;
    } else {
        for (uint32_t r = lane; r < d.z; r += 64u) ka.out.sel[rb + r] = s_sel[r];
    }
}

template <typename Rows, typename RefT>
__global__ __launch_bounds__(64) void k_filter_walk(const RefT* __restrict__ tgt_ref, const uint32_t* __restrict__ tgt_gbin,
                                                    const uint4* __restrict__ slots, const uint32_t* __restrict__ redo, const Rows rows,
                                                    const FilterOut out) {
    const uint32_t lane = lane_id();
    const uint32_t n = out.counters[CNT_REDO];
    for (uint32_t i = blockIdx.x; i < n; i += gridDim.x) {
        const uint32_t slot = redo[i];
        const uint4 d = slots[slot];
        filter_span(rows, out, tgt_ref, tgt_gbin, lane, d.x, d.x + d.y, out.rbase[slot] + out.bbase[slot >> 10]);
    }
}

__global__ __launch_bounds__(256) void k_check_grouping(const uint64_t* __restrict__ key, uint32_t n, uint64_t id_mask,
                                                        uint64_t* __restrict__ tab, uint32_t tab_mask,
                                                        uint32_t* __restrict__ n_split) {
    for (uint32_t i = blockIdx.x * 256u + threadIdx.x; i < n; i += gridDim.x * 256u) {
        const uint64_t k = key[i] & id_mask;
        if (i != 0u && (key[i - 1u] & id_mask) == k) continue;
        uint32_t slot = static_cast<uint32_t>(mix64(k)) & tab_mask;
        for (uint32_t probe = 0; probe <= tab_mask; ++probe) {
            const unsigned long long old = atomicCAS(reinterpret_cast<unsigned long long*>(&tab[slot]), ~0ull,
                                                     static_cast<unsigned long long>(k));
            if (old == ~0ull) break;
            if (old == k) {
                atomicAdd(n_split, 1u);
                break;
            }
            slot = (slot + 1u) & tab_mask;
        }
    }
}
void launch_check_grouping(hipStream_t st, const uint64_t* key, uint32_t n, uint64_t id_mask, uint64_t* tab, uint32_t tab_mask,
                           uint32_t* n_split) {
    if (n) hipLaunchKernelGGL(k_check_grouping, dim3(std::min<uint32_t>((n + 255u) / 256u, 8192u)), dim3(256), 0, st, key, n,
                              id_mask, tab, tab_mask, n_split);
}

void launch_hist(hipStream_t st, const uint32_t* tgt_gbin, const uint4* slots, uint32_t nslots, uint32_t* counters,
                 uint32_t* tail, uint32_t* cov, uint32_t* ucov, bool count_mapped) {
    uint32_t blocks = std::max(1u, std::min((nslots + kWaves - 1) / kWaves, 256u * 16u));
    hipLaunchKernelGGL(k_hist, dim3(blocks), dim3(kBlock), 0, st, tgt_gbin, slots, nslots, counters, tail, cov, ucov,
                       count_mapped ? 1 : 0);
}

void launch_ref_stats(hipStream_t st, const uint32_t* a, const uint32_t* b, const uint32_t* bin_off, uint32_t n_refs,
                      uint32_t* out, const PackArgs* pack) {
    uint32_t blocks = (n_refs + kWaves - 1) / kWaves;
    PackArgs none;
    if (blocks)
        hipLaunchKernelGGL(k_ref_stats, dim3(blocks), dim3(kBlock), 0, st, a, b, bin_off, n_refs, out, pack ? *pack : none);
}

__global__ __launch_bounds__(256) void k_copy_out(uint32_t* __restrict__ dst_host, const uint32_t* __restrict__ src,
                                                  uint32_t n) {
    const uint32_t gid = blockIdx.x * 256 + threadIdx.x, gsz = gridDim.x * 256;
    const uint32_t n4 = n >> 2;
    for (uint32_t i = gid; i < n4; i += gsz)
        reinterpret_cast<uint4*>(dst_host)[i] = reinterpret_cast<const uint4*>(src)[i];
    for (uint32_t i = (n4 << 2) + gid; i < n; i += gsz) dst_host[i] = src[i];
}

void launch_copy_out(hipStream_t st, uint32_t* dst_host, const uint32_t* src, uint32_t n) {
    const uint32_t blocks = std::min<uint32_t>(64u, (n / 4 + 255u) / 256u + 1u);
    hipLaunchKernelGGL(k_copy_out, dim3(blocks), dim3(256), 0, st, dst_host, src, n);
}

__global__ __launch_bounds__(256) void k_zero(const ZeroArgs z) {
    const uint32_t gid = blockIdx.x * 256 + threadIdx.x, gsz = gridDim.x * 256;
#pragma unroll
    for (int k = 0; k < 5; ++k)
        for (uint32_t i = gid; i < z.n[k]; i += gsz) z.p[k][i] = 0u;
    for (uint32_t i = gid; i < z.n64; i += gsz) z.p64[i] = ~0ull;
    const uint32_t n4 = z.cp_n >> 2;
    for (uint32_t i = gid; i < n4; i += gsz) reinterpret_cast<uint4*>(z.cp_dst)[i] = reinterpret_cast<const uint4*>(z.cp_src)[i];
    for (uint32_t i = (n4 << 2) + gid; i < z.cp_n; i += gsz) z.cp_dst[i] = z.cp_src[i];
// ... 92 lines not shown
                                                        uint32_t* __restrict__ ucov2, uint32_t* __restrict__ lca_count) {
    for (uint32_t i = blockIdx.x * kBlock + threadIdx.x; i < n_reads; i += gridDim.x * kBlock) {
        const uint32_t v = sel[i];
        if (v == 0xffffffffu) continue;
        if (v < taxon_base)
            atomicAdd(&ucov2[v], 1u);
        else
            atomicAdd(&lca_count[v - taxon_base], 1u);
    }
}

void launch_sel_atomics(hipStream_t st, const uint32_t* sel, uint32_t n_reads, uint32_t taxon_base, uint32_t* ucov2,
                        uint32_t* lca_count) {
    uint32_t blocks = std::max(1u, std::min((n_reads + kBlock - 1) / kBlock, 256u * 16u));
    hipLaunchKernelGGL(k_sel_atomics, dim3(blocks), dim3(kBlock), 0, st, sel, n_reads, taxon_base, ucov2, lca_count);
}

void launch_filter(hipStream_t st, const FilterArgs& a, hipEvent_t t0, hipEvent_t t1) {
    if (!a.nslots) return;
    FilterOut out;
    out.sel = a.sel;
    out.rbase = a.slot_rbase;
    out.bbase = a.slot_bbase;
    out.marks = reinterpret_cast<uint8_t*>(a.marks);
    out.pair_tab = a.pair_tab;
    out.pair_list = a.pair_list;
    out.pair_mask = a.pair_mask;
    out.taxon_base = a.taxon_base;
    out.counters = a.counters;
    const uint32_t grid = a.nslots;
    auto launch = [&](const auto& r, auto ref_word) {
        using Rows = std::decay_t<decltype(r)>;
        using RefT = decltype(ref_word);
        const RefT* const tgt_ref = static_cast<const RefT*>(a.tgt_ref.p);
        const FilterKernArgs<Rows, RefT> ka{tgt_ref, a.tgt_gbin, a.slots, a.valid_bits, a.redo, a.nslots, r, out};
        hipExtLaunchKernelGGL((k_filter_compact<Rows, RefT>), dim3(grid), dim3(64), 0, st, t0, t1, 0, ka);
        hipLaunchKernelGGL((k_filter_walk<Rows, RefT>), dim3(std::min(a.nslots, 256u)), dim3(64), 0, st, tgt_ref, a.tgt_gbin, a.slots,
                           a.redo, r, out);
    };
    if (a.rows16) {
        Rows16 r;
        r.rows = reinterpret_cast<const uint4*>(a.rows16);
        r.taxon_flat = a.taxon_flat;
        r.shift = a.taxon_shift;
        if (a.tgt_ref.ref16) launch(r, uint16_t{});
        else launch(r, uint32_t{});
    } else {
        Rows32 r;
        r.lin4 = reinterpret_cast<const uint4*>(a.lin_dense);
        r.valid_of = a.valid;
        if (a.tgt_ref.ref16) launch(r, uint16_t{});
        else launch(r, uint32_t{});
    }
}

}

namespace slimm {

__global__ __launch_bounds__(256) void k_nonzero_bits(const uint32_t* __restrict__ bins, uint64_t n_words64,
                                                      uint64_t* __restrict__ bits) {
    const uint64_t w = (static_cast<uint64_t>(blockIdx.x) * 256 + threadIdx.x) >> 6;
    const uint32_t lane = threadIdx.x & 63u;
    const uint64_t stride = (static_cast<uint64_t>(gridDim.x) * 256) >> 6;
    for (uint64_t k = w; k < n_words64; k += stride) {
        const uint64_t m = __ballot(bins[k * 64 + lane] != 0u);
        if (lane == 0) bits[k] = m;
    }
}

__device__ __forceinline__ uint32_t or_over_ranks(const uint32_t* __restrict__ gathered, uint64_t rank_stride,
// ... 111 lines not shown
```

slimm_amd/csrc/tile_hist.hip:

```cpp
#include <hip/hip_runtime.h>
#include <type_traits>
#include <stdint.h>

#include <algorithm>

#include "kernels.h"

#ifndef SLIMM_TILE_SHIFT
#error "tile_hist.hip is compiled with -DSLIMM_TILE_SHIFT=13 or 14"
#endif
#if SLIMM_TILE_SHIFT == 13
#define SLIMM_TILE_NS tiles13
#elif SLIMM_TILE_SHIFT == 14
#define SLIMM_TILE_NS tiles14
#else
#error "a bucket entry holds 14 bits of bin and the unique bit"
#endif

namespace slimm {
namespace SLIMM_TILE_NS {

constexpr uint32_t kTileShift = SLIMM_TILE_SHIFT;
constexpr uint32_t kTileBins = 1u << kTileShift;
constexpr uint32_t kSuperShift = kTileShift + 6;
// ... 106 lines not shown
    return n;
}

struct __attribute__((packed, aligned(4))) Quad {
    uint32_t a, b, c, d;
};
__device__ __forceinline__ void piece_load(const uint32_t* __restrict__ vals, uint32_t base, uint32_t n, uint32_t lane,
                                           uint32_t* v) {
    const uint32_t i = 4u * lane;
    Quad q{0xffffffffu, 0xffffffffu, 0xffffffffu, 0xffffffffu};
    if (i < n) q = *reinterpret_cast<const Quad*>(vals + base + i);
    v[0] = i < n ? q.a : 0xffffffffu;
    v[1] = i + 1u < n ? q.b : 0xffffffffu;
    v[2] = i + 2u < n ? q.c : 0xffffffffu;
    v[3] = i + 3u < n ? q.d : 0xffffffffu;
}

__device__ __forceinline__ bool piece_load_packed(SlotWalk& w, const uint32_t* __restrict__ vals, uint32_t lane, uint32_t* v) {
    uint32_t base_a = 0, base_b = 0;
    const uint32_t n_a = slot_next(w, &base_a);
    const uint32_t q_a = (n_a + 3u) >> 2;
    const uint32_t n_b = (n_a != 0u && q_a < 64u) ? slot_next(w, &base_b, 4u * (64u - q_a)) : 0u;
    const bool second = lane >= q_a;
    const uint32_t i = 4u * (second ? lane - q_a : lane), n = second ? n_b : n_a;
    Quad q{0xffffffffu, 0xffffffffu, 0xffffffffu, 0xffffffffu};
    if (i < n) q = *reinterpret_cast<const Quad*>(vals + (second ? base_b : base_a) + i);
    v[0] = i < n ? q.a : 0xffffffffu;
    v[1] = i + 1u < n ? q.b : 0xffffffffu;
    v[2] = i + 2u < n ? q.c : 0xffffffffu;
    v[3] = i + 3u < n ? q.d : 0xffffffffu;
    return n_a != 0u;
}

__device__ __forceinline__ uint32_t tile_of(uint32_t v) { return (v & 0x7fffffffu) >> kTileShift; }

template <int kMode>
__global__ __launch_bounds__(kTBlock * kCountFold) void k_tile_count(const uint32_t* __restrict__ vals, const uint4* __restrict__ slots,
                                                        uint32_t nslots, int per_read, uint32_t ntiles,
                                                        uint32_t* __restrict__ tile_count_all, uint32_t reps,
                                                        uint32_t rep_stride, uint4* __restrict__ part,
                                                        uint32_t* __restrict__ matrix, uint32_t S,
                                                        const uint32_t* __restrict__ gate) {
    HIP_DYNAMIC_SHARED(uint32_t, s_hist)
    __shared__ uint32_t s_sum[3];
    if (kMode == 2 && *gate == 0u) return;
    if (threadIdx.x < 3) s_sum[threadIdx.x] = 0;
    uint32_t* __restrict__ tile_count = tile_count_all + static_cast<size_t>(blockIdx.x % reps) * rep_stride;
    for (uint32_t i = threadIdx.x; i < ntiles; i += kTBlock * kCountFold) s_hist[i] = 0;
    __syncthreads();
    const uint32_t lane = threadIdx.x & 63u;
    SlotWalk w = slot_walk(slots, nslots, per_read != 0, kCountFold);
    if (kMode == 1) {
        const uint32_t waves = blockDim.x >> 6, wave = w.d_wave;
        const uint32_t first = tile_sample_first(wave, waves, S);
        if (slots) {
            const uint32_t lo = w.s - wave;
            if (part) {
                uint32_t v = 0, h = 0, f = 0;
                for (uint32_t s = lo + threadIdx.x; s < w.s_end; s += blockDim.x) {
                    const uint4 d = slots[s];
                    f += d.y;
                    h += d.z;
                    v += d.w;
                }
                v = wave_sum_dpp(v);
                h = wave_sum_dpp(h);
                f = wave_sum_dpp(f);
                if (lane == 0u) {
                    atomicAdd(&s_sum[0], v);
                    atomicAdd(&s_sum[1], h);
                    atomicAdd(&s_sum[2], f);
                }
            }
            w.s = lo + first;
            w.nd = w.s < w.s_end ? slots[w.s] : make_uint4(0u, 0u, 0u, 0u);
        } else {
            w.d_wave = first;
        }
        w.step = tile_sample_step(waves, S);
    }
    while (true) {
        uint32_t v[16];
        bool any = false;
#pragma unroll
        for (int u = 0; u < 4; ++u) {
            uint32_t base = 0;
            const uint32_t n = slot_next(w, &base);
            any = any || n != 0u;
            piece_load(vals, base, n, lane, v + 4 * u);
        }
        if (!any) break;
#pragma unroll
        for (int u = 0; u < 16; ++u)
            if (v[u] != 0xffffffffu) atomicAdd(&s_hist[tile_of(v[u])], 1u);
    }
    if (kMode != 1 && part && lane == 0u) {
        atomicAdd(&s_sum[0], w.sum_v);
        atomicAdd(&s_sum[1], w.sum_h);
        atomicAdd(&s_sum[2], w.sum_f);
    }
    __syncthreads();
    if (part && threadIdx.x == 0) part[blockIdx.x] = make_uint4(s_sum[0], s_sum[1], s_sum[2], 0u);
    if (matrix) {
        uint32_t* __restrict__ row = matrix + static_cast<size_t>(blockIdx.x) * rep_stride;
        for (uint32_t i = threadIdx.x; i < ntiles; i += kTBlock * kCountFold) row[i] = s_hist[i];
        return;
    }
    for (uint32_t i = threadIdx.x; i < ntiles; i += kTBlock * kCountFold) {
        uint32_t h = s_hist[i];
        if (h) atomicAdd(&tile_count[i], h);
    }
}

__global__ __launch_bounds__(256) void k_matrix_prefix(uint32_t* __restrict__ matrix, uint32_t nrows, uint32_t ntiles,
                                                       uint32_t row_stride, uint32_t* __restrict__ total) {
    const uint32_t t = blockIdx.x * 256u + threadIdx.x;
    if (t >= ntiles) return;
    uint32_t run = 0;
    uint32_t r = 0;
    for (; r + 16u <= nrows; r += 16u) {
        uint32_t v[16];
#pragma unroll
        for (uint32_t u = 0; u < 16u; ++u) v[u] = matrix[static_cast<size_t>(r + u) * row_stride + t];
#pragma unroll
        for (uint32_t u = 0; u < 16u; ++u) {
            matrix[static_cast<size_t>(r + u) * row_stride + t] = run;
            run += v[u];
// ... 235 lines not shown
constexpr int kDirectPieces = 32;
constexpr uint32_t kTileSlots = 4096;
constexpr uint32_t kRoundCap = (kTBlock / 64) * kRoundPieces * 64;

template <int kPieces, bool kWide>
__device__ __forceinline__ bool round_load(SlotWalk& w, const uint32_t* __restrict__ vals, uint32_t lane,
                                           uint32_t (&v)[kPieces]) {
    static_assert(kPieces % 4 == 0, "values come four to a lane");
    bool any = false;
    if (kWide) {
#pragma unroll
        for (int k = 0; k < kPieces; k += 4) any = piece_load_packed(w, vals, lane, v + k) || any;
    } else {
#pragma unroll
        for (int k = 0; k < kPieces; ++k) {
            uint32_t base = 0;
            const uint32_t n = slot_next(w, &base, 64u);
            any = any || n != 0u;
            v[k] = lane < n ? vals[base + lane] : 0xffffffffu;
        }
    }
    return any;
}

constexpr uint32_t kEntryBits = kTileShift + 1;
static_assert(kEntryBits <= 16, "bucket entries are 16-bit");
__device__ __forceinline__ uint32_t entry_of(uint32_t v) { return (v & kTileMask) | ((v >> 31) << kTileShift); }

__device__ __forceinline__ uint32_t block_excl_scan_4096(uint32_t* s, uint32_t* s_wtot);

__device__ __forceinline__ void scatter_round_ordered(const uint32_t (&v)[kRoundPieces], uint32_t ntiles,
                                                      const uint32_t* s_mine, uint32_t* __restrict__ tile_cursor,
                                                      uint16_t* __restrict__ bucket, uint32_t* s_cnt, uint32_t* s_loff,
                                                      uint32_t* s_stage, uint32_t* s_wtot) {
    const uint32_t tid = threadIdx.x;
    TPROF_T(p0);
    for (uint32_t i = tid; i < kTileSlots; i += kTBlock) s_cnt[i] = 0;
    __syncthreads();
    TPROF_T(p1);
    TPROF_ADD(1, p0, p1);
    uint32_t r[kRoundPieces];
#pragma unroll
    for (int k = 0; k < kRoundPieces; ++k) r[k] = v[k] != 0xffffffffu ? atomicAdd(&s_cnt[tile_of(v[k])], 1u) : 0u;
    __syncthreads();
    TPROF_T(p2);
    TPROF_ADD(2, p1, p2);
    uint32_t got[kTileSlots / kTBlock];
#pragma unroll
    for (uint32_t j = 0; j < kTileSlots / kTBlock; ++j) {
        const uint32_t i = j * kTBlock + tid;
        const uint32_t h = s_cnt[i];
        s_loff[i] = h;
        got[j] = 0u;
        if (h && i < ntiles) got[j] = atomicAdd(&tile_cursor[i], h);
    }
    __syncthreads();
    TPROF_T(p3);
    TPROF_ADD(3, p2, p3);
    const uint32_t total = block_excl_scan_4096(s_loff, s_wtot);
#pragma unroll
    for (uint32_t j = 0; j < kTileSlots / kTBlock; ++j) {
        const uint32_t i = j * kTBlock + tid;
        s_cnt[i] = got[j] + s_mine[i] - s_loff[i];
    }
    TPROF_T(p4);
    TPROF_ADD(4, p3, p4);
#pragma unroll
    for (int k = 0; k < kRoundPieces; ++k) {
        if (v[k] == 0xffffffffu) continue;
        const uint32_t t = tile_of(v[k]);
        s_stage[s_loff[t] + r[k]] = (t << kEntryBits) | entry_of(v[k]);
    }
    __syncthreads();
    TPROF_T(p5);
    TPROF_ADD(5, p4, p5);
    for (uint32_t j = tid; j < total; j += kTBlock) {
        const uint32_t e = s_stage[j];
        bucket[s_cnt[e >> kEntryBits] + j] = static_cast<uint16_t>(e & ((1u << kEntryBits) - 1u));
    }
    __syncthreads();
    TPROF_T(p6);
    TPROF_ADD(6, p5, p6);
}

template <int kPieces>
__device__ __forceinline__ void scatter_round_direct(const uint32_t (&v)[kPieces], uint32_t ntiles,
                                                     const uint32_t* __restrict__ tile_base,
                                                     uint32_t* __restrict__ tile_cursor, uint16_t* __restrict__ bucket,
                                                     uint32_t* s_hist, uint32_t last) {
    constexpr int kMaxTilesPerThread = 8;
    for (uint32_t i = threadIdx.x; i < ntiles; i += kTBlock) s_hist[i] = 0;
    __syncthreads();
#pragma unroll
    for (int k = 0; k < kPieces; ++k)
        if (v[k] != 0xffffffffu) atomicAdd(&s_hist[tile_of(v[k])], 1u);
    __syncthreads();
    for (uint32_t i0 = 0; i0 < ntiles; i0 += kMaxTilesPerThread * kTBlock) {
        uint32_t got[kMaxTilesPerThread];
#pragma unroll
        for (int j = 0; j < kMaxTilesPerThread; ++j) {
            const uint32_t i = i0 + j * kTBlock + threadIdx.x;
            const uint32_t h = i < ntiles ? s_hist[i] : 0u;
            got[j] = 0u;
            if (h) got[j] = atomicAdd(&tile_cursor[i], h);
        }
#pragma unroll
        for (int j = 0; j < kMaxTilesPerThread; ++j) {
            const uint32_t i = i0 + j * kTBlock + threadIdx.x;
            if (i < ntiles) s_hist[i] = got[j] + tile_base[i];
        }
    }
    __syncthreads();
#pragma unroll
    for (int k = 0; k < kPieces; ++k) {
        if (v[k] == 0xffffffffu) continue;
        const uint32_t pos = atomicAdd(&s_hist[tile_of(v[k])], 1u);
        bucket[min(pos, last)] = static_cast<uint16_t>(entry_of(v[k]));
    }
    __syncthreads();
}

template <int kPieces = kRoundPieces, bool kWide = true, typename Body>
__device__ __forceinline__ void bucketing_rounds(SlotWalk& walk, const uint32_t* __restrict__ vals, uint32_t* s_more,
                                                 Body body) {
    while (true) {
        uint32_t v[kPieces];
        const bool mine = round_load<kPieces, kWide>(walk, vals, threadIdx.x & 63u, v);
        if ((threadIdx.x & 63u) == 0) s_more[threadIdx.x >> 6] = mine ? 1u : 0u;
        __syncthreads();
        uint32_t any = 0;
#pragma unroll
        for (int w = 0; w < kTBlock / 64; ++w) any |= s_more[w];
        __syncthreads();
        if (!any) break;
        body(v);
    }
}

__device__ __forceinline__ void zero_split_tiles(const uint32_t* tile_base, uint32_t ntiles, uint32_t* __restrict__ cov,
                                                 uint32_t* __restrict__ ucov, uint32_t tile_sub) {
    for (uint32_t tile = blockIdx.x; tile < ntiles; tile += gridDim.x) {
        if (tile_base[tile + 1] - tile_base[tile] <= tile_sub) continue;
        uint4* oc = reinterpret_cast<uint4*>(cov + static_cast<size_t>(tile) * kTileBins);
        uint4* ou = reinterpret_cast<uint4*>((ucov ? ucov : cov) + static_cast<size_t>(tile) * kTileBins);
        const uint4 z = make_uint4(0, 0, 0, 0);
        for (uint32_t i = threadIdx.x; i < kTileBins / 4; i += kTBlock) {
            oc[i] = z;
            if (ucov) ou[i] = z;
        }
    }
}

__global__ __launch_bounds__(kTBlock) void k_tile_scatter(const uint32_t* __restrict__ vals, const uint4* __restrict__ slots,
                                                          uint32_t nslots, int per_read, uint32_t ntiles,
                                                          const uint32_t* __restrict__ tile_base,
                                                          uint32_t* __restrict__ tile_cursor_all,
                                                          uint16_t* __restrict__ bucket, uint32_t* __restrict__ cov,
                                                          uint32_t* __restrict__ ucov,
                                                          const uint32_t* __restrict__ rep_base_all, uint32_t reps,
                                                          uint32_t rep_stride, uint32_t tile_sub, uint32_t last,
                                                          const uint32_t* __restrict__ gate) {
    HIP_DYNAMIC_SHARED(uint32_t, s_hist)
    __shared__ uint32_t s_more[kTBlock / 64];
    if (gate && *gate == 0u) return;
    const uint32_t lid = xcd_logical_id();
    const size_t rep_off = static_cast<size_t>((lid / kCountFold) % reps) * rep_stride;
    uint32_t* __restrict__ tile_cursor = tile_cursor_all + rep_off;
    const uint32_t* __restrict__ rep_base = rep_base_all + rep_off;
    zero_split_tiles(tile_base, ntiles, cov, ucov, tile_sub);
    SlotWalk walk = slot_walk(slots, nslots, per_read != 0, 1, lid);
    bucketing_rounds<kDirectPieces, false>(walk, vals, s_more, [&](const uint32_t (&v)[kDirectPieces]) {
        scatter_round_direct(v, ntiles, rep_base, tile_cursor, bucket, s_hist, last);
    });
}

#ifndef SLIMM_BIG_PIECES
#define SLIMM_BIG_PIECES 24
#endif
constexpr int kBigBlock = kTBlock * kCountFold;
constexpr int kBigPieces = SLIMM_BIG_PIECES;
constexpr uint32_t kBigRound = kBigBlock * kBigPieces;
static_assert(kBigPieces % 8 == 0, "values come four to a lane; the rounds' LDS operations in batches of eight");
template <int kE>
__global__ __launch_bounds__(kBigBlock) void k_tile_scatter_big(const uint32_t* __restrict__ vals, const uint4* __restrict__ slots,
                                                                uint32_t nslots, int per_read, uint32_t ntiles,
                                                                const uint32_t* __restrict__ tile_base,
                                                                uint32_t* __restrict__ tile_cursor_all,
                                                                uint16_t* __restrict__ bucket, uint32_t* __restrict__ cov,
                                                                uint32_t* __restrict__ ucov,
                                                                const uint32_t* __restrict__ rep_base_all, uint32_t reps,
                                                                uint32_t rep_stride, uint32_t tile_sub, uint32_t last,
                                                                const uint32_t* __restrict__ gate) {
    HIP_DYNAMIC_SHARED(uint32_t, s_dyn)
    __shared__ uint32_t s_more[kBigBlock / 64], s_wtot[kBigBlock / 64];
    constexpr uint32_t kNoTile = kE * kBigBlock;
    if (gate && *gate == 0u) return;
    static_assert(kBigPieces * (kBigBlock / 64) < 65536 && kBigRound < 65536, "ranks are packed as 16-bit halves");
    uint32_t* const s_tab = s_dyn;
    uint32_t* const s_dst = s_dyn + kNoTile + 64;
    uint32_t* const s_stage = s_dst + kNoTile + 64;
    const uint32_t tid = threadIdx.x, lane = tid & 63u, wave = tid >> 6;
    const uint32_t no_tile = kNoTile + lane;
    const size_t rep_off = static_cast<size_t>(blockIdx.x % reps) * rep_stride;
    uint32_t* __restrict__ tile_cursor = tile_cursor_all + rep_off;
    const uint32_t* __restrict__ rep_base = rep_base_all + rep_off;
    uint32_t at[kE];
#pragma unroll
    for (int u = 0; u < kE; ++u) {
        const uint32_t i = u * kBigBlock + tid;
        at[u] = rep_base[i < ntiles ? i : 0u];
    }
    TPROF_T(q0);
    if (tid < kTBlock) zero_split_tiles(tile_base, ntiles, cov, ucov, tile_sub);
    SlotWalk walk = slot_walk(slots, nslots, per_read != 0, kCountFold);
    uint32_t v[kBigPieces];
    bool mine = round_load<kBigPieces, true>(walk, vals, lane, v);
    if (lane == 0u) s_more[wave] = mine ? 1u : 0u;
#pragma unroll
    for (int u = 0; u < kE; ++u) s_tab[u * kBigBlock + tid] = 0u;
    if (tid < 64u) s_tab[kNoTile + tid] = 0u, s_dst[kNoTile + tid] = 0u;
    __syncthreads();
    TPROF_T(q1);
    if (wave < 8u) TPROF_ADD(0, q0, q1);
    while (true) {
        TPROF_T(p1);
        uint32_t any = 0;
#pragma unroll
        for (int w = 0; w < kBigBlock / 64; ++w) any |= s_more[w];
        if (!any) break;
        uint32_t r2[kBigPieces / 2];
#pragma unroll
        for (int k0 = 0; k0 < kBigPieces; k0 += 8) {
            uint32_t r[8];
#pragma unroll
            for (int k = 0; k < 8; ++k) r[k] = atomicAdd(&s_tab[v[k0 + k] != 0xffffffffu ? tile_of(v[k0 + k]) : no_tile], 1u);
#pragma unroll
            for (int k = 0; k < 8; k += 2) r2[(k0 + k) / 2] = r[k] | (r[k + 1] << 16);
            __builtin_amdgcn_sched_barrier(0);
        }
        __syncthreads();
        TPROF_T(p2);
        if (wave < 8u) TPROF_ADD(2, p1, p2);
        uint32_t got[kE], sum = 0;
        {
            uint32_t h[kE];
            uint32_t* __restrict__ cursor = tile_cursor + (any >> 1);
#pragma unroll
            for (int u = 0; u < kE; ++u) {
                const uint32_t i = u * kBigBlock + tid;
                h[u] = s_tab[i];
                got[u] = 0u;
                if (h[u] && i < ntiles) got[u] = atomicAdd(&cursor[i], h[u]);
                sum += h[u];
            }
            uint32_t inc = sum;
#pragma unroll
            for (int o = 1; o < 64; o <<= 1) {
                const uint32_t a = __shfl_up(inc, o, 64);
                if (lane >= static_cast<uint32_t>(o)) inc += a;
            }
            if (lane == 63u) s_wtot[wave] = inc;
            sum = inc - sum;
            __syncthreads();
            uint32_t run = sum;
#pragma unroll
            for (int w = 0; w < kBigBlock / 64; ++w)
                if (w < static_cast<int>(wave)) run += s_wtot[w];
#pragma unroll
            for (int u = 0; u < kE; ++u) {
                s_tab[u * kBigBlock + tid] = run;
                s_dst[u * kBigBlock + tid] = at[u] - run;
                run += h[u];
            }
        }
        uint32_t total = 0;
#pragma unroll
        for (int w = 0; w < kBigBlock / 64; ++w) total += s_wtot[w];
        if (tid < 64u) s_tab[kNoTile + tid] = 0u;
        __syncthreads();
        TPROF_T(p3);
        if (wave < 8u) TPROF_ADD(3, p2, p3);
#pragma unroll
        for (int k0 = 0; k0 < kBigPieces; k0 += 8) {
            uint32_t at_[8];
#pragma unroll
            for (int k = 0; k < 8; ++k) at_[k] = s_tab[v[k0 + k] != 0xffffffffu ? tile_of(v[k0 + k]) : no_tile];
#pragma unroll
            for (int k = 0; k < 8; ++k) {
                const uint32_t t = tile_of(v[k0 + k]);
                const uint32_t rk = (k & 1) ? r2[(k0 + k) / 2] >> 16 : r2[(k0 + k) / 2] & 0xffffu;
                s_stage[v[k0 + k] != 0xffffffffu ? at_[k] + rk : kBigRound + lane] = (t << kEntryBits) | entry_of(v[k0 + k]);
            }
        }
        TPROF_T(p4);
        if (wave < 8u) TPROF_ADD(4, p3, p4);
#pragma unroll
        for (int u = 0; u < kE; ++u) s_dst[u * kBigBlock + tid] += got[u];
        TPROF_T(p4b);
        if (wave < 8u) TPROF_ADD(1, p4, p4b);
        mine = round_load<kBigPieces, true>(walk, vals, lane, v);
        if (lane == 0u) s_more[wave] = mine ? 1u : 0u;
        __syncthreads();
        TPROF_T(p5);
        if (wave < 8u) TPROF_ADD(5, p4b, p5);
#pragma unroll
        for (int u = 0; u < kE; ++u) s_tab[u * kBigBlock + tid] = 0u;
#pragma unroll
        for (int k0 = 0; k0 < kBigPieces; k0 += 4) {
            if (static_cast<uint32_t>(k0) * kBigBlock >= total) break;
            uint32_t e[4], d[4];
#pragma unroll
            for (int k = 0; k < 4; ++k) e[k] = s_stage[(k0 + k) * kBigBlock + tid];
#pragma unroll
            for (int k = 0; k < 4; ++k) d[k] = s_dst[min(e[k] >> kEntryBits, kNoTile)];
#pragma unroll
            for (int k = 0; k < 4; ++k) {
                const uint32_t j = (k0 + k) * kBigBlock + tid;
                if (j < total) bucket[min(d[k] + j, last)] = static_cast<uint16_t>(e[k] & ((1u << kEntryBits) - 1u));
            }
        }
        __syncthreads();
        TPROF_T(p6);
        if (wave < 8u) TPROF_ADD(6, p5, p6);
    }
    TPROF_T(q2);
    if (wave < 8u) TPROF_ADD(7, q0, q2);
}
constexpr size_t big_lds_bytes(int e) { return (2u * static_cast<size_t>(e) * kBigBlock + kBigRound + 192u) * 4u; }
constexpr int kBigE = 6;
static_assert(big_lds_bytes(kBigE) <= 160u * 1024u - 256u, "the two tables and the stage share a CU's LDS");
static_assert(kBigE * kBigBlock == kBigRoundTiles, "kernels.h tells the context which layouts take these rounds");
static_assert(kTileShift + 1 + 14 <= 32, "a stage entry holds the tile and the bucket entry");

__global__ __launch_bounds__(kTBlock * kCountFold) void k_tile_scatter_matrix(
    const uint32_t* __restrict__ vals, const uint4* __restrict__ slots, uint32_t nslots, int per_read, uint32_t ntiles,
    const uint32_t* __restrict__ tile_base, const uint32_t* __restrict__ matrix, uint32_t row_stride,
    uint16_t* __restrict__ bucket, uint32_t* __restrict__ cov, uint32_t* __restrict__ ucov, uint32_t tile_sub) {
    HIP_DYNAMIC_SHARED(uint32_t, s_cur)
    const uint32_t* __restrict__ row = matrix + static_cast<size_t>(blockIdx.x) * row_stride;
    for (uint32_t i = threadIdx.x; i < ntiles; i += kTBlock * kCountFold) s_cur[i] = tile_base[i] + row[i];
    if (threadIdx.x < kTBlock) zero_split_tiles(tile_base, ntiles, cov, ucov, tile_sub);
    __syncthreads();
    const uint32_t lane = threadIdx.x & 63u;
    SlotWalk w = slot_walk(slots, nslots, per_read != 0, kCountFold);
    while (true) {
        uint32_t v[8];
        bool any = false;
#pragma unroll
        for (int u = 0; u < 8; u += 4) {
            uint32_t base = 0;
            const uint32_t n = slot_next(w, &base);
            any = any || n != 0u;
            piece_load(vals, base, n, lane, v + u);
        }
        if (!any) break;
#pragma unroll
        for (int u = 0; u < 8; ++u) {
            if (v[u] == 0xffffffffu) continue;
            const uint32_t pos = atomicAdd(&s_cur[tile_of(v[u])], 1u);
            bucket[pos] = static_cast<uint16_t>(entry_of(v[u]));
        }
    }
}

constexpr uint32_t kFusedTiles = 4096;
__device__ __forceinline__ uint32_t block_excl_scan_4096(uint32_t* s, uint32_t* s_wtot) {
    const uint32_t tid = threadIdx.x, lane = tid & 63u, wave = tid >> 6;
    uint32_t v[8], sum = 0;
#pragma unroll
    for (int u = 0; u < 8; ++u) {
        v[u] = s[tid * 8 + u];
        sum += v[u];
    }
    uint32_t inc = sum;
#pragma unroll
    for (int o = 1; o < 64; o <<= 1) {
        const uint32_t a = __shfl_up(inc, o, 64);
        if (lane >= static_cast<uint32_t>(o)) inc += a;
    }
    if (lane == 63) s_wtot[wave] = inc;
    __syncthreads();
    uint32_t before = 0, total = 0;
#pragma unroll
    for (int w = 0; w < 8; ++w) {
        const uint32_t t = s_wtot[w];
        if (w < static_cast<int>(wave)) before += t;
        total += t;
    }
    uint32_t run = before + inc - sum;
#pragma unroll
    for (int u = 0; u < 8; ++u) {
        s[tid * 8 + u] = run;
        run += v[u];
    }
    __syncthreads();
    return total;
}

__global__ __launch_bounds__(kTBlock) void k_tile_scatter_fused(const uint32_t* __restrict__ vals,
                                                                const uint4* __restrict__ slots, uint32_t nslots,
                                                                int per_read, uint32_t* __restrict__ counters,
                                                                uint32_t ntiles, const uint32_t* __restrict__ tile_count_all,
                                                                uint32_t* __restrict__ tile_cursor_all,
                                                                uint16_t* __restrict__ bucket, uint32_t* __restrict__ cov,
                                                                uint32_t* __restrict__ ucov, uint32_t rep_stride,
                                                                uint4* __restrict__ items, uint32_t* __restrict__ split_tiles,
                                                                const uint4* __restrict__ part, uint32_t nparts,
                                                                uint32_t* __restrict__ tail, uint32_t tile_sub) {
    __shared__ uint32_t s_stage[kRoundCap];
    __shared__ uint32_t s_mine[kFusedTiles];
    __shared__ uint32_t s_cnt[kFusedTiles];
    __shared__ uint32_t s_loff[kFusedTiles];
    static_assert(kRoundCap >= kFusedTiles + 1, "the stage doubles as the tile_base table");
    static_assert(kFusedScanTiles + 32 <= kFusedTiles, "room for the small arrays behind the last tile");
    uint32_t* const s_wtot = s_mine + kFusedTiles - 32;
    uint32_t* const s_more = s_mine + kFusedTiles - 24;
    uint32_t& s_nsplit = s_mine[kFusedTiles - 16];
    uint32_t* const s_base = s_stage;
    const uint32_t tid = threadIdx.x;
    const uint32_t lid = xcd_logical_id();
    const uint32_t my_rep = (lid / kCountFold) % kTileReps;
    TPROF_T(q0);
    if (tid == 0) s_nsplit = 0;
#pragma unroll
    for (int q = 0; q < 8; ++q) {
        const uint32_t i = q * kTBlock + tid;
        uint32_t c = 0, mine = 0;
        if (i < ntiles) {
            uint32_t v[kTileReps];
#pragma unroll
            for (uint32_t rep = 0; rep < kTileReps; ++rep) v[rep] = tile_count_all[static_cast<size_t>(rep) * rep_stride + i];
#pragma unroll
            for (uint32_t rep = 0; rep < kTileReps; ++rep) {
                if (rep < my_rep) mine += v[rep];
                c += v[rep];
            }
        }
        s_base[i] = c;
        if (i < ntiles) s_mine[i] = mine;
    }
    __syncthreads();
// ... 9 lines not shown
        if (part) publish_totals(part, nparts, counters, tail, s_loff);
        uint32_t* s_piece = s_cnt;
#pragma unroll
        for (int q = 0; q < 8; ++q) {
            const uint32_t i = q * kTBlock + tid;
            const uint32_t c = i < ntiles ? s_base[i + 1] - s_base[i] : 0u;
            s_piece[i] = i < ntiles ? (c ? (c + tile_sub - 1) / tile_sub : 1u) : 0u;
        }
        __syncthreads();
        const uint32_t n_items = block_excl_scan_4096(s_piece, s_wtot);
        for (uint32_t i = tid; i < ntiles; i += kTBlock) {
            const uint32_t b0 = s_base[i], c = s_base[i + 1] - b0;
            const uint32_t pieces = c ? (c + tile_sub - 1) / tile_sub : 1u;
            if (pieces > 1) split_tiles[atomicAdd(&s_nsplit, 1u)] = i;
            for (uint32_t k = 0; k < pieces; ++k) {
                const uint32_t lo = b0 + k * tile_sub;
                items[s_piece[i] + k] = make_uint4(i, lo, min(lo + tile_sub, b0 + c), pieces);
            }
        }
        __syncthreads();
        if (tid == 0) {
            counters[CNT_ITEMS] = n_items;
            counters[CNT_ITEMS2] = 0;
            counters[CNT_SPLIT] = s_nsplit;
        }
    }
    zero_split_tiles(s_base, ntiles, cov, ucov, tile_sub);
    __syncthreads();
    uint32_t* __restrict__ tile_cursor = tile_cursor_all + static_cast<size_t>(my_rep) * rep_stride;
    SlotWalk walk = slot_walk(slots, nslots, per_read != 0, 1, lid);
    TPROF_T(q1);
    TPROF_ADD(0, q0, q1);
    bucketing_rounds(walk, vals, s_more, [&](const uint32_t (&v)[kRoundPieces]) {
        scatter_round_ordered(v, ntiles, s_mine, tile_cursor, bucket, s_cnt, s_loff, s_stage, s_wtot);
    });
    TPROF_T(q2);
    TPROF_ADD(7, q0, q2);
}

__global__ __launch_bounds__(kTBlock) void k_part_super(const uint32_t* __restrict__ vals, const uint4* __restrict__ slots,
                                                        uint32_t nslots, int per_read, uint32_t ntiles,
                                                        const uint32_t* __restrict__ tile_base,
                                                        uint32_t* __restrict__ sup_cursor, uint32_t* __restrict__ mid,
                                                        uint32_t* __restrict__ cov, uint32_t* __restrict__ ucov,
                                                        uint32_t tile_sub) {
    __shared__ uint32_t s_cur[kMaxSuper];
    __shared__ uint32_t s_more[kTBlock / 64];
    const uint32_t nsup = (ntiles + kSuperTiles - 1) / kSuperTiles;
    zero_split_tiles(tile_base, ntiles, cov, ucov, tile_sub);
    SlotWalk walk = slot_walk(slots, nslots, per_read != 0);
    bucketing_rounds(walk, vals, s_more, [&](const uint32_t (&v)[kRoundPieces]) {
        for (uint32_t i = threadIdx.x; i < nsup; i += kTBlock) s_cur[i] = 0;
        __syncthreads();
#pragma unroll
        for (int k = 0; k < kRoundPieces; ++k)
            if (v[k] != 0xffffffffu) atomicAdd(&s_cur[(v[k] & 0x7fffffffu) >> kSuperShift], 1u);
        __syncthreads();
        for (uint32_t i = threadIdx.x; i < nsup; i += kTBlock) {
            const uint32_t h = s_cur[i];
            if (h) s_cur[i] = tile_base[i * kSuperTiles] + atomicAdd(&sup_cursor[i], h);
        }
        __syncthreads();
#pragma unroll
        for (int k = 0; k < kRoundPieces; ++k) {
            if (v[k] == 0xffffffffu) continue;
            const uint32_t g = v[k] & 0x7fffffffu;
            const uint32_t pos = atomicAdd(&s_cur[g >> kSuperShift], 1u);
            mid[pos] = (g & kSuperMask) | ((v[k] >> 31) << kSuperShift);
        }
        __syncthreads();
    });
}

__global__ __launch_bounds__(kTBlock) void k_part_tile(const uint32_t* __restrict__ mid, const uint4* __restrict__ items2,
                                                       const uint32_t* __restrict__ counters,
                                                       const uint32_t* __restrict__ tile_base,
                                                       uint32_t* __restrict__ tile_cursor, uint32_t ntiles,
                                                       uint16_t* __restrict__ bucket) {
    __shared__ uint32_t s_cur[kSuperTiles];
    if (blockIdx.x >= counters[CNT_ITEMS2]) return;
    const uint4 it = items2[blockIdx.x];
    const uint32_t sup = it.x, lo = it.y, hi = it.z;
    const uint32_t tile0 = sup * kSuperTiles;
    if (threadIdx.x < kSuperTiles) s_cur[threadIdx.x] = 0;
    __syncthreads();
    for (uint32_t e0 = lo; e0 < hi; e0 += 4 * kTBlock) {
        uint32_t v[4];
#pragma unroll
        for (int u = 0; u < 4; ++u) {
            uint32_t e = e0 + u * kTBlock + threadIdx.x;
            v[u] = (e < hi) ? mid[e] : 0xffffffffu;
        }
#pragma unroll
        for (int u = 0; u < 4; ++u)
            if (v[u] != 0xffffffffu) atomicAdd(&s_cur[(v[u] & kSuperMask) >> kTileShift], 1u);
    }
    __syncthreads();
    if (threadIdx.x < kSuperTiles) {
        const uint32_t h = s_cur[threadIdx.x], tile = tile0 + threadIdx.x;
        if (h && tile < ntiles) s_cur[threadIdx.x] = tile_base[tile] + atomicAdd(&tile_cursor[tile], h);
    }
// ... 474 lines not shown
    }
}

void launch_pack(hipStream_t st, uint32_t* dst, const PackArgs& pack, const TileTables* t, const uint32_t* a, const uint32_t* b,
                 const uint32_t* bin_off, uint32_t n_refs, uint32_t* stats, const BitsLayout& bits) {
    const uint32_t blocks = 256;
    const uint32_t* const split_tiles = t ? t->split_tiles : nullptr;
    const uint32_t* const counters = t ? t->counters : nullptr;
    const uint32_t* const tile_ref0 = t ? t->tile_ref0 : nullptr;
    if (b)
        hipLaunchKernelGGL(k_pack<true>, dim3(blocks), dim3(512), 0, st, dst, pack, split_tiles, counters, a, b, bin_off,
                           n_refs, tile_ref0, stats, bits);
    else
        hipLaunchKernelGGL(k_pack<false>, dim3(blocks), dim3(512), 0, st, dst, pack, split_tiles, counters, a, a, bin_off,
                           n_refs, tile_ref0, stats, bits);
}

uint32_t tile_count_grid(uint32_t grid) { return (grid + kCountFold - 1) / kCountFold; }

int tile_hist_setup(uint32_t ntiles) {
    const size_t bytes = static_cast<size_t>(ntiles) * 4;
    if (!tile_tables_fit_lds(ntiles)) return -1;
    for (auto* k : {k_tile_count<0>, k_tile_count<1>, k_tile_count<2>})
        if (hipFuncSetAttribute(reinterpret_cast<const void*>(k), hipFuncAttributeMaxDynamicSharedMemorySize, static_cast<int>(bytes)) !=
            hipSuccess)
            return -1;
    if ((ntiles + kSuperTiles - 1) / kSuperTiles > kMaxSuper) return -1;
    if (hipFuncSetAttribute(reinterpret_cast<const void*>(k_tile_scatter), hipFuncAttributeMaxDynamicSharedMemorySize,
                            static_cast<int>(bytes)) != hipSuccess)
        return -1;
    if (hipFuncSetAttribute(reinterpret_cast<const void*>(k_tile_scatter_matrix), hipFuncAttributeMaxDynamicSharedMemorySize,
                            static_cast<int>(bytes)) != hipSuccess)
        return -1;
    if (hipFuncSetAttribute(reinterpret_cast<const void*>(k_tile_scatter_big<kBigE>), hipFuncAttributeMaxDynamicSharedMemorySize,
                            static_cast<int>(big_lds_bytes(kBigE))) != hipSuccess)
        return -1;
    return 0;
}

void launch_tile_count(hipStream_t st, uint32_t grid, uint32_t ntiles, const SlotValues& in, const TileTables& t, bool totals,
                       bool matrix, const TileSample& sm) {
    auto* const k = sm.gated ? k_tile_count<2> : sm.stride > 1u ? k_tile_count<1> : k_tile_count<0>;
    hipLaunchKernelGGL(k, dim3(tile_count_grid(grid)), dim3(kTBlock * kCountFold), static_cast<size_t>(ntiles) * 4, st, in.vals, in.slots,
                       in.nslots, in.per_read ? 1 : 0, ntiles, t.tile_count, t.reps, t.stride, totals ? t.tot_part : nullptr,
                       matrix ? t.matrix : nullptr, sm.stride, t.counters + sm.flag);
}

void launch_matrix_prefix(hipStream_t st, uint32_t grid, uint32_t ntiles, const TileTables& t) {
    hipLaunchKernelGGL(k_matrix_prefix, dim3((ntiles + 255u) / 256u), dim3(256), 0, st, t.matrix, tile_count_grid(grid), ntiles,
                       t.stride, t.tile_count);
}

void launch_tile_scan(hipStream_t st, uint32_t ntiles, const TileTables& t, uint32_t reps, bool two_level, const Totals& tot,
                      uint32_t tile_sub, const TileSample& sm) {
    hipLaunchKernelGGL(sm.stride > 1u ? k_tile_scan<true> : k_tile_scan<false>, dim3(1), dim3(1024), 0, st, t.tile_count, ntiles, t.tile_base, t.tile_cursor, t.tile_items,
                       t.counters, t.part_items, t.sup_cursor, t.split_tiles, reps, t.stride, two_level ? 1 : 0, tot.part,
                       tot.nparts, tot.tail, tile_sub, sm.stride, sm.k, t.entries, sm.flag, sm.gated ? 1 : 0);
}

uint32_t part_items_upper(uint32_t ntiles, uint32_t n_upper) {
    return (ntiles + kSuperTiles - 1) / kSuperTiles + n_upper / kPartSub + 1;
}

void launch_tile_scatter(hipStream_t st, TilePath path, uint32_t grid, uint32_t ntiles, uint32_t n_upper, const SlotValues& in,
                         const TileTables& t, uint32_t* cov, uint32_t* ucov, const Totals& tot, uint32_t tile_sub,
                         const TileSample& sm) {
    const bool fit = sm.stride > 1u;
    const uint32_t last = t.entries - 1u;
    const uint32_t* const gate = sm.gated ? t.counters + sm.flag : nullptr;
    if (fit) tile_sub = 0xffffffffu;
    const int per_read = in.per_read ? 1 : 0;
    const size_t lds = static_cast<size_t>(ntiles) * 4;
    switch (path) {
    case TilePath::Fused:
        hipLaunchKernelGGL(k_tile_scatter_fused, dim3(grid), dim3(kTBlock), 0, st, in.vals, in.slots, in.nslots, per_read,
                           t.counters, ntiles, t.tile_count, t.tile_cursor, t.bucket, cov, ucov, t.stride, t.tile_items,
                           t.split_tiles, tot.part, tot.nparts, tot.tail, tile_sub);
        break;
    case TilePath::OrderedRounds:
        hipLaunchKernelGGL(k_tile_scatter_big<kBigE>, dim3(tile_count_grid(grid)), dim3(kBigBlock), big_lds_bytes(kBigE), st,
                           in.vals, in.slots, in.nslots, per_read, ntiles, t.tile_base, t.tile_cursor, t.bucket, cov, ucov,
                           t.tile_count, t.reps, t.stride, tile_sub, last, gate);
        break;
    case TilePath::DirectRounds:
        hipLaunchKernelGGL(k_tile_scatter, dim3(grid), dim3(kTBlock), lds, st, in.vals, in.slots, in.nslots, per_read, ntiles,
                           t.tile_base, t.tile_cursor, t.bucket, cov, ucov, t.tile_count, t.reps, t.stride, tile_sub, last, gate);
        break;
    case TilePath::Matrix:
        hipLaunchKernelGGL(k_tile_scatter_matrix, dim3(tile_count_grid(grid)), dim3(kTBlock * kCountFold), lds, st, in.vals,
                           in.slots, in.nslots, per_read, ntiles, t.tile_base, t.matrix, t.stride, t.bucket, cov, ucov, tile_sub);
        break;
    case TilePath::TwoLevel:
        hipLaunchKernelGGL(k_part_super, dim3(grid), dim3(kTBlock), 0, st, in.vals, in.slots, in.nslots, per_read, ntiles,
                           t.tile_base, t.sup_cursor, t.mid, cov, ucov, tile_sub);
        hipLaunchKernelGGL(k_part_tile, dim3(part_items_upper(ntiles, n_upper)), dim3(kTBlock), 0, st, t.mid, t.part_items,
                           t.counters, t.tile_base, t.tile_cursor, ntiles, t.bucket);
        break;
    case TilePath::DirectAtomics:
        break;
    }
}

void launch_tile_fit(hipStream_t st, uint32_t ntiles, const TileTables& t, uint32_t* cov, uint32_t* ucov, uint32_t tile_sub,
                     const TileSample& sm) {
    const uint32_t peak = CNT_PEAK + (sm.flag - CNT_FALLBACK);
    hipLaunchKernelGGL(k_tile_fit, dim3(std::min(ntiles, 256u)), dim3(1024), 0, st, t.tile_count, t.tile_base, t.tile_cursor,
                       ntiles, t.stride, t.tile_items, t.split_tiles, t.counters, cov, ucov, tile_sub, sm.flag, peak);
}

uint32_t tile_items_upper(uint32_t ntiles, uint32_t n_upper) { return ntiles + n_upper / std::min(kTileSub, kTileSubB) + 1; }

void launch_tile_hist(hipStream_t st, uint32_t ntiles, uint32_t n_upper, const TileTables& t, uint32_t* cov, uint32_t* ucov,
                      const uint32_t* bin_off, uint32_t n_refs, uint32_t* stats, const BitsLayout& bits, uint32_t store_from,
                      bool wide, bool stretched) {
    const uint32_t grid = tile_items_upper(ntiles, n_upper);
    const uint32_t* const rb = stretched ? t.tile_count : nullptr;
    const uint32_t* const rf = stretched ? t.tile_cursor : nullptr;
    if (ucov && wide)
        hipLaunchKernelGGL((k_tile_hist<true, false>), dim3(grid), dim3(hist_block<true, false>()), 0, st, t.bucket, t.tile_items, t.counters, cov, ucov, bin_off,
                           n_refs, t.tile_ref0, stats, bits, store_from, rb, rf, t.stride);
    else if (ucov)
        hipLaunchKernelGGL((k_tile_hist<true, true>), dim3(grid), dim3(hist_block<true, true>()), 0, st, t.bucket, t.tile_items, t.counters, cov, ucov, bin_off,
                           n_refs, t.tile_ref0, stats, bits, store_from, rb, rf, t.stride);
    else
        hipLaunchKernelGGL((k_tile_hist<false, false>), dim3(grid), dim3(hist_block<false, false>()), 0, st, t.bucket, t.tile_items, t.counters, cov, cov, bin_off,
                           n_refs, t.tile_ref0, stats, bits, store_from, rb, rf, t.stride);
}
// ... 18 lines not shown
```

slimm_amd/profiler.py:

```python
from __future__ import annotations

import ctypes as C
from typing import Dict, List, Optional, Tuple

import numpy as np

from . import capi
from .workload import Options, Records, Taxonomy, Workload


def _p(a: np.ndarray):
    return a.ctypes.data_as(C.c_void_p)


class DeviceArray:

    def __init__(self, ptr: int, n: int, typestr: str = "<i4"):
        self.ptr, self.n = ptr, n
        self.__cuda_array_interface__ = {"shape": (n,), "typestr": typestr, "data": (ptr, False), "version": 2}


class Slimm:
    def _config(self, taxonomy, options, ref_names, ref_len, avg_read_len, device, grouped, lineage):
        self.ref_names = list(ref_names)
# ... 544 lines not shown
        return self.write_abundance(None)

    def stats(self) -> Dict[str, float]:
        s = capi.Stats()
        self._check(self.L.slimm_get_stats(self.ctx, C.byref(s)))
        return {n: getattr(s, n) for n, _ in capi.Stats._fields_}

    def ref_columns(self) -> Dict[str, np.ndarray]:
        R = self.n_refs
        out = {n: np.zeros(R, dtype=np.uint32) for n in ("reads_count", "uniq_reads_count", "uniq_reads_count2", "nbins",
                                                         "nz_cov", "nz_uniq_cov", "nz_uniq_cov2")}
        out["valid"] = np.zeros(R, dtype=np.uint8)
        out["abundance"] = np.zeros(R, dtype=np.float32)
        out["uniq_abundance"] = np.zeros(R, dtype=np.float32)
        cols = capi.RefColumns(**{k: _p(v) for k, v in out.items()})
        self._check(self.L.slimm_get_ref_columns(self.ctx, C.byref(cols)))
        return out

    def bins(self, which: int) -> np.ndarray:
        out = np.zeros(int(self.stats()["total_bins"]), dtype=np.uint32)
        self._check(self.L.slimm_get_bins(self.ctx, which, _p(out)))
        return out

    def read_targets(self):
        n = C.c_uint64()
        self._check(self.L.slimm_get_read_targets(self.ctx, None, None, 0, C.byref(n)))
        ref = np.zeros(n.value, dtype=np.uint32)
        gbin = np.zeros(n.value, dtype=np.uint32)
        self._check(self.L.slimm_get_read_targets(self.ctx, _p(ref), _p(gbin), n.value, C.byref(n)))
        return ref, gbin

    def target_ref_bits(self) -> int:
        return self.L.slimm_target_ref_bits(self.ctx)

    def bucket_sampling(self) -> Dict[str, Dict[str, int]]:
        v = np.zeros(6, dtype=np.uint32)
        self._check(self.L.slimm_get_bucket_sampling(self.ctx, _p(v)))
        return {ph: {"stride": int(v[3 * i]), "fallback": int(v[3 * i + 1]), "peak_1024": int(v[3 * i + 2])}
                for i, ph in enumerate("AB")}

    def taxon_counts(self, stage: int = 1) -> Dict[int, int]:
        n = C.c_uint32()
        self._check(self.L.slimm_taxon_count_size(self.ctx, stage, C.byref(n)))
        t = np.zeros(n.value, dtype=np.uint32)
        c = np.zeros(n.value, dtype=np.uint32)
        self._check(self.L.slimm_get_taxon_counts(self.ctx, stage, _p(t), _p(c)))
        return {int(a): int(b) for a, b in zip(t, c)}

    def children_pairs(self, stage: int = 1) -> set:
        n = C.c_uint64()
        self._check(self.L.slimm_children_pairs_size(self.ctx, stage, C.byref(n)))
        t = np.zeros(n.value, dtype=np.uint32)
        r = np.zeros(n.value, dtype=np.uint32)
        self._check(self.L.slimm_get_children_pairs(self.ctx, stage, _p(t), _p(r)))
        return set(zip(t.tolist(), r.tolist()))

    def enable_kernel_timing(self, on: bool = True):
        self._check(self.L.slimm_enable_kernel_timing(self.ctx, int(on)))

    def time_only_kernel(self, name: Optional[str]):
        self._check(self.L.slimm_time_only_kernel(self.ctx, name.encode() if name else None))

    def kernel_times(self, reset: bool = True) -> Dict[str, Tuple[float, int]]:
        cap = 32
        names = (C.c_char_p * cap)()
        ms = (C.c_double * cap)()
# ... 222 lines not shown
```

Before: 117,300.

## Pack per-read targets into one 4-byte word with span table for ref lookup

Adds an optional word4 mode where each read target stores only the global bin plus a head bit in one 32-bit word, dropping the separate tgt_ref array. The reference id is recovered through a new span table built on device, and on the host by binary search over bin offsets. Downstream tile and histogram kernels get a value mask or bit width so they ignore the extra head bit. This is meant to cut front-stage write traffic and memory footprint, at the cost of fewer usable bin bits and an extra span-build kernel. The mode appears to be gated on the forced 'word4' setting, which defaults to 0.

```diff
diff --git a/include/slimm_hip.h b/include/slimm_hip.h
--- a/include/slimm_hip.h
+++ b/include/slimm_hip.h
@@ -197,6 +197,7 @@
 
 int slimm_get_read_targets(slimm_ctx* ctx, uint32_t* ref, uint32_t* gbin, uint64_t cap, uint64_t* n);
 int slimm_target_ref_bits(slimm_ctx* ctx);
+int slimm_target_bytes(slimm_ctx* ctx);
 
 int slimm_taxon_count_size(slimm_ctx* ctx, int stage, uint32_t* n);
 int slimm_get_taxon_counts(slimm_ctx* ctx, int stage, uint32_t* taxid, uint32_t* count);
diff --git a/slimm_amd/capi.py b/slimm_amd/capi.py
--- a/slimm_amd/capi.py
+++ b/slimm_amd/capi.py
@@ -154,6 +154,7 @@
     ("slimm_get_bins", C.c_int, [_P, C.c_int, _P]),
     ("slimm_get_read_targets", C.c_int, [_P, _P, _P, C.c_uint64, C.POINTER(C.c_uint64)]),
     ("slimm_target_ref_bits", C.c_int, [_P]),
+    ("slimm_target_bytes", C.c_int, [_P]),
     ("slimm_get_bucket_sampling", C.c_int, [_P, _P]),
     ("slimm_taxon_count_size", C.c_int, [_P, C.c_int, C.POINTER(C.c_uint32)]),
     ("slimm_get_taxon_counts", C.c_int, [_P, C.c_int, _P, _P]),
diff --git a/slimm_amd/csrc/context.h b/slimm_amd/csrc/context.h
--- a/slimm_amd/csrc/context.h
+++ b/slimm_amd/csrc/context.h
@@ -23,6 +23,7 @@
 #include "zstd_walk.h"
 #include "xz_walk.h"
 #include "kernels.h"
+#include "span_plan.h"
 #include "read_identity.h"
 
 namespace slimm {
@@ -146,6 +147,17 @@
     std::vector<uint32_t> rows16_prev;
     bool use_rows16 = false;
     bool ref16 = false;
+    bool word4 = false;
+    uint32_t span_shift = 0, span_nblocks = 0;
+    DevBuf<uint32_t> d_span_bits;
+    DevBuf<uint4> d_span;
+    SpanTables span_tables() const {
+        SpanTables t;
+        t.bits = d_span_bits.p, t.span = d_span.p, t.bin_off = d_bin_off.p, t.valid_bits = d_valid_bits.p;
+        t.nblocks = span_nblocks, t.shift = span_shift, t.n_refs = R;
+        return t;
+    }
+    uint32_t value_mask() const { return word4 ? kW4BinMask : 0x7fffffffu; }
     DevBuf<uint64_t> in_key;
     DevBuf<int32_t> in_ref, in_pos;
     DevBuf<uint16_t> in_flag;
@@ -162,7 +174,7 @@
     DevBuf<uint2> c_pay, s_pay;
     DevBuf<uint32_t> group_hist, c_chk, s_chk;
     DevBuf<uint32_t> tgt_ref, tgt_gbin;
-    TargetRefs target_refs() const { return TargetRefs{tgt_ref.p, ref16}; }
+    TargetRefs target_refs() const { return word4 ? TargetRefs{nullptr, false, true} : TargetRefs{tgt_ref.p, ref16, false}; }
     DevBuf<uint4> slots;
     bool keep_bins = true;
     bool binsA_stored = false, binsB_stored = false;
diff --git a/slimm_amd/csrc/context.hip b/slimm_amd/csrc/context.hip
--- a/slimm_amd/csrc/context.hip
+++ b/slimm_amd/csrc/context.hip
@@ -42,7 +42,7 @@
 }
 
 int ensure_work_buffers(slimm_ctx* c, uint32_t n) {
-    HIP_TRY(c, c->tgt_ref.ensure(n + 1));
+    if (!c->word4) HIP_TRY(c, c->tgt_ref.ensure(n + 1));
     HIP_TRY(c, c->tgt_gbin.ensure(n + 8));
     HIP_TRY(c, c->slots.ensure(front_slots(n) + 1));
     HIP_TRY(c, c->sel.ensure(n + 8));
@@ -169,6 +169,16 @@
     const TileForces forces = TileForces::from_env();
     const TileLayout& tl = c->tiles.layout = tile_layout(off, c->Tsel, forces.tile_shift);
     if (tl.Bp + tl.Tpad >= kMaxBins) return fail(nullptr, SLIMM_E_INVALID, "more than 2^31 coverage bins; use a larger bin width");
+    {
+        long w4 = 0, lim = 0, sh = 0;
+        (void)forced("word4", &w4);
+        const uint64_t limit = forced("word4_bins", &lim) && lim > 0 && static_cast<uint64_t>(lim) < kWord4Bins
+                                   ? static_cast<uint64_t>(lim) : kWord4Bins;
+        c->word4 = w4 != 0 && word4_fits(static_cast<uint64_t>(tl.Bp) + tl.Tpad, limit);
+        (void)forced("span_shift", &sh);
+        c->span_shift = span_shift(off, c->R, sh);
+        c->span_nblocks = span_blocks(off, c->span_shift);
+    }
 
     if (c->device >= 0) {
         slimm_ctx* cc = c.get();
@@ -196,6 +206,10 @@
         HIP_TRY0(cc->d_valid.ensure(c->R));
         HIP_TRY0(cc->d_valid_bits.ensure(c->R / 32 + 2));
         HIP_TRY0(cc->h_valid_bits.ensure(c->R / 32 + 2));
+        if (c->word4) {
+            HIP_TRY0(cc->d_span_bits.ensure(c->span_nblocks / 32 + 4));
+            HIP_TRY0(cc->d_span.ensure(c->span_nblocks + 1ull));
+        }
         memset(cc->h_valid_bits.p, 0, (c->R / 32 + 2) * 4);
         HIP_TRY0(cc->bins.ensure(3 * tl.Bp + kTailWords + tl.Tpad));
         HIP_TRY0(cc->counters.ensure(CNT_WORDS));
@@ -484,6 +498,7 @@
     };
     if (c->use_tiles()) {
         job.values.vals = c->tgt_gbin.p;
+        job.values.mask = c->value_mask();
         job.values.slots = c->slots.p;
         job.values.nslots = nslots;
         job.n_upper = n;
@@ -510,7 +525,7 @@
         if (int rc = slot_prefix_beside_what_follows()) return rc;
         KernelTimer t(c, K_HIST);
         launch_hist(st, c->tgt_gbin.p, c->slots.p, nslots, c->counters.p, c->tail(), c->cov(), c->ucov(),
-                    c->order != SLIMM_ORDER_ANY);
+                    c->order != SLIMM_ORDER_ANY, c->value_mask());
         c->binsA_stored = true;
     }
     c->prefix_pending = true;
@@ -794,6 +809,7 @@
         z.cp2_src = c->h_valid_bits.p;
         z.cp2_n = R / 32u + 1u;
         launch_zero(st, z);
+        if (c->word4) launch_span_build(st, c->span_tables(), c->d_span_bits.p, c->d_span.p);
     }
     const uint32_t nslots = front_slots(c->rec.n);
     HIP_TRY(c, hipStreamWaitEvent(st, c->prefix_done, 0));
@@ -814,6 +830,7 @@
             fa.valid = c->d_valid.p;
         }
         fa.valid_bits = c->d_valid_bits.p;
+        fa.span = c->span_tables();
         fa.redo = c->filter_redo.p;
         fa.sel = c->sel.p;
         fa.slot_rbase = c->slot_rbase.p;
@@ -828,6 +845,7 @@
     }
     if (c->use_tiles()) {
         job.values.vals = c->sel.p;
+        job.values.mask = c->value_mask();
         job.values.nslots = c->local_M;
         job.n_upper = c->rec.n;
         job.a = c->ucov2();
@@ -1208,25 +1226,39 @@
     if (!ref && !gbin) return SLIMM_OK;
     if (cap < total) return fail(c, SLIMM_E_INVALID, "slimm_get_read_targets: %llu entries, room for %llu",
                                  static_cast<unsigned long long>(total), static_cast<unsigned long long>(cap));
-    std::vector<uint16_t> ref16(ref && c->ref16 ? total : 0);
+    std::vector<uint16_t> ref16(ref && c->ref16 && !c->word4 ? total : 0);
     uint64_t o = 0;
     for (const uint4& d : sl) {
         if (!d.y) continue;
-        if (ref && c->ref16)
+        if (ref && c->ref16 && !c->word4)
             HIP_TRY(c, hipMemcpyAsync(ref16.data() + o, reinterpret_cast<const uint16_t*>(c->tgt_ref.p) + d.x, d.y * 2ull,
                                       hipMemcpyDeviceToHost, c->stream));
-        else if (ref)
+        else if (ref && !c->word4)
             HIP_TRY(c, hipMemcpyAsync(ref + o, c->tgt_ref.p + d.x, d.y * 4ull, hipMemcpyDeviceToHost, c->stream));
-        if (gbin) HIP_TRY(c, hipMemcpyAsync(gbin + o, c->tgt_gbin.p + d.x, d.y * 4ull, hipMemcpyDeviceToHost, c->stream));
+        if (gbin || (ref && c->word4))
+            HIP_TRY(c, hipMemcpyAsync((gbin ? gbin : ref) + o, c->tgt_gbin.p + d.x, d.y * 4ull, hipMemcpyDeviceToHost, c->stream));
         o += d.y;
     }
     HIP_TRY(c, hipStreamSynchronize(c->stream));
-    if (ref && c->ref16)
+    if (c->word4) {
+        const std::vector<uint32_t>& bo = c->bin_off_h;
+        for (uint64_t k = 0; k < total; ++k) {
+            const uint32_t w = (gbin ? gbin : ref)[k];
+            if (ref) {
+                const uint32_t r = static_cast<uint32_t>(std::upper_bound(bo.begin(), bo.begin() + c->R, w & kW4BinMask) - bo.begin()) - 1u;
+                ref[k] = r | ((w & kW4Head) << 1);
+            }
+            if (gbin) gbin[k] = w & ~kW4Head;
+        }
+    }
+    if (ref && c->ref16 && !c->word4)
         for (uint64_t k = 0; k < total; ++k) ref[k] = (ref16[k] & 0x7fffu) | ((ref16[k] & 0x8000u) << 16);
     return SLIMM_OK;
 }
 
 int slimm_target_ref_bits(slimm_ctx* c) { return c ? (c->ref16 ? 16 : 32) : SLIMM_E_INVALID; }
+
+int slimm_target_bytes(slimm_ctx* c) { return c ? (c->word4 ? 4 : c->ref16 ? 6 : 8) : SLIMM_E_INVALID; }
 
 int slimm_get_bucket_sampling(slimm_ctx* c, uint32_t out[6]) {
     if (!c || !out) return SLIMM_E_INVALID;
diff --git a/slimm_amd/csrc/front.hip b/slimm_amd/csrc/front.hip
--- a/slimm_amd/csrc/front.hip
+++ b/slimm_amd/csrc/front.hip
@@ -346,7 +346,7 @@
 static_assert(kHashWalk == 16 || kHashWalk == 24 || kHashWalk == 32 || kHashWalk == 48,
               "the threshold is one of the distances window_fast's doubling chain knows");
 
-template <typename RefT>
+template <typename RefT, bool kW4>
 __device__ __forceinline__ void window_fast(uint32_t field, uint32_t gbin, uint32_t lane, uint64_t SS, uint64_t V, uint64_t PR,
                                             WinOut& so, RefT* __restrict__ tgt_ref, uint32_t* __restrict__ tgt_gbin,
                                             uint32_t* tab) {
@@ -396,15 +396,19 @@
     const bool uniq = f_bit(U);
     if (f_bit(F)) {
         const uint32_t p = so.base + so.nf + f_rank(F);
-        tgt_ref[p] = static_cast<RefT>((field - 1u) + f_head_bit<RefT>(f_bit(H)));
-        tgt_gbin[p] = gbin | (uniq ? 0x80000000u : 0u);
+        if constexpr (kW4) {
+            tgt_gbin[p] = gbin | (f_bit(H) ? kW4Head : 0u) | (uniq ? 0x80000000u : 0u);
+        } else {
+            tgt_ref[p] = static_cast<RefT>((field - 1u) + f_head_bit<RefT>(f_bit(H)));
+            tgt_gbin[p] = gbin | (uniq ? 0x80000000u : 0u);
+        }
     }
     so.nf += static_cast<uint32_t>(__popcll(F));
     so.nh += static_cast<uint32_t>(__popcll(H));
     so.nv += static_cast<uint32_t>(__popcll(V));
 }
 
-template <typename RefT>
+template <typename RefT, bool kW4>
 __device__ __forceinline__ void window_general(const Staged& rec, uint32_t lane, uint64_t RS, uint64_t V, uint32_t X,
                                                WinOut& so, RefT* __restrict__ tgt_ref,
                                                uint32_t* __restrict__ tgt_gbin) {
@@ -441,15 +445,19 @@
     if (first) {
         const uint32_t before_run = static_cast<uint32_t>(__popcll(F & ((1ull << run_from) - 1ull)));
         const uint32_t p = so.base + so.nf + before_run + smaller + same_before;
-        tgt_ref[p] = static_cast<RefT>(rec.ref | f_head_bit<RefT>(head));
-        tgt_gbin[p] = rec.gbin | ((head && same_total == 1u) ? 0x80000000u : 0u);
+        if constexpr (kW4) {
+            tgt_gbin[p] = rec.gbin | (head ? kW4Head : 0u) | ((head && same_total == 1u) ? 0x80000000u : 0u);
+        } else {
+            tgt_ref[p] = static_cast<RefT>(rec.ref | f_head_bit<RefT>(head));
+            tgt_gbin[p] = rec.gbin | ((head && same_total == 1u) ? 0x80000000u : 0u);
+        }
     }
     so.nf += static_cast<uint32_t>(__popcll(F));
     so.nh += static_cast<uint32_t>(__popcll(H));
     so.nv += static_cast<uint32_t>(__popcll(V));
 }
 
-template <bool kChk, typename Acc, typename RefT>
+template <bool kChk, bool kW4, typename Acc, typename RefT>
 __device__ __forceinline__ uint32_t long_run(const Acc& acc, uint32_t pos, uint32_t N, uint32_t lane, WinOut& so,
                                           RefT* __restrict__ tgt_ref, uint32_t* __restrict__ tgt_gbin, bool& bad,
                                           bool& collide, uint32_t* tab) {
@@ -540,7 +548,7 @@
                 const FrontRaw3 rw{0u, first ? r.ref : 0u, 0u};
                 const uint32_t g = first ? acc.gbin(r, acc.geo_of(rw)) : 0u;
                 if (first) {
-                    tgt_ref[p] = static_cast<RefT>(r.ref | f_head_bit<RefT>(head));
+                    if constexpr (!kW4) tgt_ref[p] = static_cast<RefT>(r.ref | f_head_bit<RefT>(head));
                     if (!head) tgt_gbin[p] = g;
                 }
                 uint64_t Hm = H;
@@ -558,7 +566,7 @@
 #pragma unroll
                 for (uint32_t m = 0; m < 3u; ++m)
                     if (((head_seen >> m) & 1u) && lane == 0u)
-                        tgt_gbin[head_p[m]] = head_g[m] | (n_first[m] == 1u ? 0x80000000u : 0u);
+                        tgt_gbin[head_p[m]] = head_g[m] | (kW4 ? kW4Head : 0u) | (n_first[m] == 1u ? 0x80000000u : 0u);
             }
         }
     } while (again);
@@ -579,7 +587,7 @@
     return kStageRecs;
 }
 
-template <typename RefT>
+template <typename RefT, bool kW4>
 __device__ __forceinline__ bool long_run_staged(const uint32_t* st1, const uint32_t* st2, uint32_t off, uint32_t end_off,
                                                 uint32_t lane, WinOut& so, RefT* __restrict__ tgt_ref,
                                                 uint32_t* __restrict__ tgt_gbin, uint32_t* tab) {
@@ -624,7 +632,7 @@
             const bool head = f_bit(H);
             const uint32_t p = so.base + so.nf + f_rank(F);
             if (first) {
-                tgt_ref[p] = static_cast<RefT>((field - 1u) | f_head_bit<RefT>(head));
+                if constexpr (!kW4) tgt_ref[p] = static_cast<RefT>((field - 1u) | f_head_bit<RefT>(head));
                 if (!head) tgt_gbin[p] = g;
             }
             uint64_t Hm = H;
@@ -642,7 +650,8 @@
         if (!falls) {
 #pragma unroll
             for (uint32_t m = 0; m < 3u; ++m)
-                if (((head_seen >> m) & 1u) && lane == 0u) tgt_gbin[head_p[m]] = head_g[m] | (n_first[m] == 1u ? 0x80000000u : 0u);
+                if (((head_seen >> m) & 1u) && lane == 0u)
+                    tgt_gbin[head_p[m]] = head_g[m] | (kW4 ? kW4Head : 0u) | (n_first[m] == 1u ? 0x80000000u : 0u);
             so.nv += nv;
             return true;
         }
@@ -683,7 +692,7 @@
             const bool head = f_bit(H);
             const uint32_t p = so.base + so.nf + f_rank(F);
             if (first) {
-                tgt_ref[p] = static_cast<RefT>((field - 1u) | f_head_bit<RefT>(head));
+                if constexpr (!kW4) tgt_ref[p] = static_cast<RefT>((field - 1u) | f_head_bit<RefT>(head));
                 if (!head) tgt_gbin[p] = g;
             }
             uint64_t Hm = H;
@@ -699,7 +708,8 @@
         }
 #pragma unroll
         for (uint32_t m = 0; m < 3u; ++m)
-            if (((head_seen >> m) & 1u) && lane == 0u) tgt_gbin[head_p[m]] = head_g[m] | (n_first[m] == 1u ? 0x80000000u : 0u);
+            if (((head_seen >> m) & 1u) && lane == 0u)
+                    tgt_gbin[head_p[m]] = head_g[m] | (kW4 ? kW4Head : 0u) | (n_first[m] == 1u ? 0x80000000u : 0u);
     }
     so.nv += nv_run;
     return true;
@@ -786,7 +796,7 @@
 
 }
 
-template <typename Acc, bool kChk, typename RefT>
+template <typename Acc, bool kChk, typename RefT, bool kW4>
 __global__ __launch_bounds__(kFrontBlock, 4) void k_front(const Acc acc, uint32_t nslots, uint32_t* __restrict__ counters,
                                                        RefT* __restrict__ tgt_ref, uint32_t* __restrict__ tgt_gbin,
                                                        uint4* __restrict__ slots) {
@@ -827,7 +837,7 @@
                     const uint64_t PR = (~0ull >> 1) >> lead;
                     const uint32_t field = w1 & kRefField, mate = (w1 >> kStMateShift) & 3u, mprev = f_shr1z(mate);
                     if ((f_ballot(mate < mprev) & ~RSw & PR) != 0ull) break;
-                    window_fast(field, w2, lane, (RSw | f_ballot(mate != mprev)) & PR, f_ballot(field != kRefField) & PR, PR, so, tgt_ref,
+                    window_fast<RefT, kW4>(field, w2, lane, (RSw | f_ballot(mate != mprev)) & PR, f_ballot(field != kRefField) & PR, PR, so, tgt_ref,
                                 tgt_gbin, tab);
                     off += X;
                 }
@@ -847,18 +857,18 @@
                     const uint32_t mprev = f_shr1z(mate);
                     const uint64_t V = f_ballot(field != kRefField) & PR;
                     if ((f_ballot(mate < mprev) & ~RS & PR) == 0ull) {
-                        window_fast(field, w2, lane, (RS | f_ballot(mate != mprev)) & PR, V, PR, so, tgt_ref, tgt_gbin, tab);
+                        window_fast<RefT, kW4>(field, w2, lane, (RS | f_ballot(mate != mprev)) & PR, V, PR, so, tgt_ref, tgt_gbin, tab);
                     } else {
-                        window_general<RefT>(Staged{mate, field - 1u, w2, f_bit(V)}, lane, RS, V, X, so, tgt_ref, tgt_gbin);
+                        window_general<RefT, kW4>(Staged{mate, field - 1u, w2, f_bit(V)}, lane, RS, V, X, so, tgt_ref, tgt_gbin);
                     }
                     off += X;
                 } else {
                     FPROF_T(l0);
                     const uint32_t end_off = next_run_start(st1, lane, off + 64u);
-                    if (end_off < kStageRecs && long_run_staged(st1, st2, off, end_off, lane, so, tgt_ref, tgt_gbin, tab)) {
+                    if (end_off < kStageRecs && long_run_staged<RefT, kW4>(st1, st2, off, end_off, lane, so, tgt_ref, tgt_gbin, tab)) {
                         off = end_off;
                     } else {
-                        const uint32_t end = long_run<kChk, Acc, RefT>(acc, pos, N, lane, so, tgt_ref, tgt_gbin, bad, collide, tab);
+                        const uint32_t end = long_run<kChk, kW4, Acc, RefT>(acc, pos, N, lane, so, tgt_ref, tgt_gbin, bad, collide, tab);
                         __builtin_amdgcn_s_waitcnt(0x0f70);
                         off = end - B < kStageRecs ? next_run_start(st1, lane, end - B) : kStageRecs;
                     }
@@ -886,11 +896,14 @@
 template <typename Acc, bool kChk>
 static void front_launch(hipStream_t st, const Acc& a, uint32_t ns, uint32_t* counters, TargetRefs tgt_ref, uint32_t* tgt_gbin,
                          uint4* slots, hipEvent_t t0, hipEvent_t t1) {
-    if (tgt_ref.ref16)
-        hipExtLaunchKernelGGL((k_front<Acc, kChk, uint16_t>), dim3(front_grid(ns)), dim3(kFrontBlock), 0, st, t0, t1, 0, a, ns,
+    if (tgt_ref.word4)
+        hipExtLaunchKernelGGL((k_front<Acc, kChk, uint32_t, true>), dim3(front_grid(ns)), dim3(kFrontBlock), 0, st, t0, t1, 0, a, ns,
+                              counters, static_cast<uint32_t*>(nullptr), tgt_gbin, slots);
+    else if (tgt_ref.ref16)
+        hipExtLaunchKernelGGL((k_front<Acc, kChk, uint16_t, false>), dim3(front_grid(ns)), dim3(kFrontBlock), 0, st, t0, t1, 0, a, ns,
                               counters, static_cast<uint16_t*>(tgt_ref.p), tgt_gbin, slots);
     else
-        hipExtLaunchKernelGGL((k_front<Acc, kChk, uint32_t>), dim3(front_grid(ns)), dim3(kFrontBlock), 0, st, t0, t1, 0, a, ns,
+        hipExtLaunchKernelGGL((k_front<Acc, kChk, uint32_t, false>), dim3(front_grid(ns)), dim3(kFrontBlock), 0, st, t0, t1, 0, a, ns,
                               counters, static_cast<uint32_t*>(tgt_ref.p), tgt_gbin, slots);
 }
 
diff --git a/slimm_amd/csrc/kernels.h b/slimm_amd/csrc/kernels.h
--- a/slimm_amd/csrc/kernels.h
+++ b/slimm_amd/csrc/kernels.h
@@ -106,10 +106,23 @@
 constexpr uint32_t kMaxRefs = (1u << 26) - 2u;
 constexpr uint32_t kMaxBins = 0x7ffffff0u;
 constexpr uint32_t kRef16Max = 1u << 15;
+constexpr uint32_t kWord4Bins = 1u << 30;
+constexpr uint32_t kW4Head = 1u << 30;
+constexpr uint32_t kW4BinMask = kW4Head - 1u;
 struct TargetRefs {
     void* p = nullptr;
     bool ref16 = false;
-};
+    bool word4 = false;
+};
+constexpr uint32_t kSpanMore = 1u << 31;
+struct SpanTables {
+    const uint32_t* bits = nullptr;
+    const uint4* span = nullptr;
+    const uint32_t* bin_off = nullptr;
+    const uint32_t* valid_bits = nullptr;
+    uint32_t nblocks = 0, shift = 0, n_refs = 0;
+};
+void launch_span_build(hipStream_t st, const SpanTables& t, uint32_t* bits, uint4* span);
 uint32_t front_slots(uint32_t n_records);
 void launch_front_raw(hipStream_t st, const DeviceRecords& in, uint32_t n_refs, const uint2* geo, uint32_t half_read,
                       uint32_t bin_width, uint32_t* counters, TargetRefs tgt_ref, uint32_t* tgt_gbin, uint4* slots,
@@ -121,7 +134,7 @@
 void launch_check_grouping(hipStream_t st, const uint64_t* key, uint32_t n, uint64_t id_mask, uint64_t* tab, uint32_t tab_mask,
                            uint32_t* n_split);
 void launch_hist(hipStream_t st, const uint32_t* tgt_gbin, const uint4* slots, uint32_t nslots, uint32_t* counters,
-                 uint32_t* tail, uint32_t* cov, uint32_t* ucov, bool count_mapped);
+                 uint32_t* tail, uint32_t* cov, uint32_t* ucov, bool count_mapped, uint32_t vmask = 0x7fffffffu);
 void launch_ref_stats(hipStream_t st, const uint32_t* a, const uint32_t* b, const uint32_t* bin_off, uint32_t n_refs,
                       uint32_t* out, const PackArgs* pack = nullptr);
 struct FilterArgs {
@@ -135,6 +148,7 @@
     const uint32_t* lin_dense = nullptr;
     const uint8_t* valid = nullptr;
     const uint32_t* valid_bits = nullptr;
+    SpanTables span;
     uint32_t* redo = nullptr;
     uint32_t* sel = nullptr;
     const uint32_t* slot_rbase = nullptr;
@@ -163,6 +177,7 @@
     const uint4* slots = nullptr;
     uint32_t nslots = 0;
     bool per_read = false;
+    uint32_t mask = 0x7fffffffu;
 };
 struct Totals {
     const uint4* part = nullptr;
diff --git a/slimm_amd/csrc/kernels.hip b/slimm_amd/csrc/kernels.hip
--- a/slimm_amd/csrc/kernels.hip
+++ b/slimm_amd/csrc/kernels.hip
@@ -29,7 +29,7 @@
 __global__ __launch_bounds__(kBlock) void k_hist(const uint32_t* __restrict__ tgt_gbin, const uint4* __restrict__ slots,
                                                  uint32_t nslots, uint32_t* __restrict__ counters,
                                                  uint32_t* __restrict__ tail, uint32_t* __restrict__ cov,
-                                                 uint32_t* __restrict__ ucov, int count_mapped) {
+                                                 uint32_t* __restrict__ ucov, int count_mapped, uint32_t vmask) {
     __shared__ uint32_t s_tot[3];
     if (threadIdx.x < 3) s_tot[threadIdx.x] = 0;
     __syncthreads();
@@ -43,8 +43,8 @@
         sum_v += d.w;
         for (uint32_t o = lane; o < d.y; o += 64u) {
             const uint32_t g = tgt_gbin[d.x + o];
-            atomicAdd(&cov[g & 0x7fffffffu], 1u);
-            if (g >> 31) atomicAdd(&ucov[g & 0x7fffffffu], 1u);
+            atomicAdd(&cov[g & vmask], 1u);
+            if (g >> 31) atomicAdd(&ucov[g & vmask], 1u);
         }
     }
     if (lane == 0u) {
@@ -398,16 +398,60 @@
     if (lk.q4) filter_q4<RefT>(rows, out, lane, X, w, row, vb, sel_base, lk.q4);
 }
 
-template <typename Rows, typename RefT>
-__device__ __forceinline__ void filter_span(const Rows& rows, const FilterOut& out, const RefT* __restrict__ tgt_ref,
-                                         const uint32_t* __restrict__ tgt_gbin, uint32_t lane, uint32_t pos, uint32_t endp,
-                                         uint32_t sel_base) {
+__device__ __forceinline__ uint32_t ref_of_bin(const uint32_t* __restrict__ bin_off, uint32_t n_refs, uint32_t bin, uint32_t from) {
+    uint32_t step = 1u;
+    while (from + step < n_refs && bin_off[from + step] <= bin) step <<= 1;
+    uint32_t lo = from + (step >> 1), hi = min(from + step, n_refs);
+    while (lo + 1u < hi) {
+        const uint32_t mid = (lo + hi) >> 1;
+        const bool up = bin_off[mid] <= bin;
+        lo = up ? mid : lo;
+        hi = up ? hi : mid;
+    }
+    return lo;
+}
+
+__device__ __forceinline__ uint32_t ref_of_bin_any(const uint32_t* __restrict__ bin_off, uint32_t n_refs, uint32_t bin) {
+    uint32_t lo = 0u, hi = n_refs;
+    while (lo + 1u < hi) {
+        const uint32_t mid = (lo + hi) >> 1;
+        const bool up = bin_off[mid] <= bin;
+        lo = up ? mid : lo;
+        hi = up ? hi : mid;
+    }
+    return lo;
+}
+
+template <typename RefT>
+struct TgtTwo {
+    using Ref = RefT;
+    const RefT* __restrict__ tgt_ref;
+    const uint32_t* __restrict__ tgt_gbin;
+    __device__ __forceinline__ uint32_t w(uint32_t i) const { return tgt_ref[i]; }
+    __device__ __forceinline__ uint32_t g(uint32_t i) const { return tgt_gbin[i]; }
+};
+struct TgtOne {
+    using Ref = uint32_t;
+    const uint32_t* __restrict__ tgt_gbin;
+    const uint32_t* __restrict__ bin_off;
+    uint32_t n_refs;
+    __device__ __forceinline__ uint32_t w(uint32_t i) const {
+        const uint32_t gg = tgt_gbin[i];
+        return ref_of_bin_any(bin_off, n_refs, gg & kW4BinMask) | ((gg & kW4Head) << 1);
+    }
+    __device__ __forceinline__ uint32_t g(uint32_t i) const { return tgt_gbin[i] & ~kW4Head; }
+};
+
+template <typename Rows, typename Src>
+__device__ __forceinline__ void filter_span(const Rows& rows, const FilterOut& out, const Src& src, uint32_t lane, uint32_t pos,
+                                         uint32_t endp, uint32_t sel_base) {
+    using RefT = typename Src::Ref;
     using TW = TgtWord<RefT>;
     while (pos < endp) {
         const uint32_t n_live = min(64u, endp - pos);
         const bool live = lane < n_live;
-        const uint32_t w = live ? tgt_ref[pos + lane] : 0u;
-        const uint32_t g = live ? tgt_gbin[pos + lane] : 0u;
+        const uint32_t w = live ? src.w(pos + lane) : 0u;
+        const uint32_t g = live ? src.g(pos + lane) : 0u;
         const uint64_t HB = k_ballot((w >> TW::kShift) != 0u) & k_below(n_live);
         const uint32_t X = pos + 64u >= endp ? n_live : 63u - static_cast<uint32_t>(__builtin_clzll(HB | 1ull));
         if (X != 0u) {
@@ -422,8 +466,8 @@
         uint32_t e = pos;
         while (true) {
             const bool in = e + lane < endp;
-            const uint32_t ww = in ? tgt_ref[e + lane] : TW::kHead;
-            const uint32_t gg = in ? tgt_gbin[e + lane] : 0u;
+            const uint32_t ww = in ? src.w(e + lane) : TW::kHead;
+            const uint32_t gg = in ? src.g(e + lane) : 0u;
             uint64_t heads = k_ballot((ww >> TW::kShift) != 0u);
             if (e == pos) heads &= ~1ull;
             const uint32_t n_in = heads ? static_cast<uint32_t>(__builtin_ctzll(heads)) : 64u;
@@ -446,7 +490,7 @@
             sel = out.taxon_base + index;
             for (uint32_t c = pos; c < e; c += 64u) {
                 const bool in = c + lane < e;
-                const uint32_t rr = in ? (tgt_ref[c + lane] & TW::kRefMask) : 0u;
+                const uint32_t rr = in ? (src.w(c + lane) & TW::kRefMask) : 0u;
                 const typename Rows::Row row = rows.load(rr);
                 read_children(out, in && Rows::valid(row), rr, lv, taxon);
             }
@@ -488,11 +532,10 @@
     return v;
 }
 
-template <typename Rows, typename RefT>
-__device__ __forceinline__ void compact_window(const FilterKernArgs<Rows, RefT>& ka, uint32_t lane, uint32_t X, uint64_t Hc,
+template <typename Rows, typename KA>
+__device__ __forceinline__ void compact_window(const KA& ka, uint32_t lane, uint32_t X, uint64_t Hc,
                                                uint32_t cref, uint32_t cg, uint32_t cr, const typename Rows::Row& row,
                                                uint32_t* __restrict__ s_sel) {
-    using KA = FilterKernArgs<Rows, RefT>;
     const Rows& rows = ka.rows;
     const FilterOut& out = ka.out;
     const uint64_t PR = k_below(X);
@@ -669,7 +712,7 @@
                     whole_reads_walk = true;
                     break;
                 }
-                compact_window(ka, lane, X, Hc, cref, cg, cr, row, s_sel);
+                compact_window<Rows>(ka, lane, X, Hc, cref, cg, cr, row, s_sel);
                 cdone += X;
             }
             if (__builtin_expect(whole_reads_walk, 0)) break;
@@ -685,17 +728,217 @@
     }
 }
 
-template <typename Rows, typename RefT>
-__global__ __launch_bounds__(64) void k_filter_walk(const RefT* __restrict__ tgt_ref, const uint32_t* __restrict__ tgt_gbin,
-                                                    const uint4* __restrict__ slots, const uint32_t* __restrict__ redo, const Rows rows,
-                                                    const FilterOut out) {
+template <typename Rows, typename Src>
+__global__ __launch_bounds__(64) void k_filter_walk(const Src src, const uint4* __restrict__ slots,
+                                                    const uint32_t* __restrict__ redo, const Rows rows, const FilterOut out) {
     const uint32_t lane = lane_id();
     const uint32_t n = out.counters[CNT_REDO];
     for (uint32_t i = blockIdx.x; i < n; i += gridDim.x) {
         const uint32_t slot = redo[i];
         const uint4 d = slots[slot];
-        filter_span(rows, out, tgt_ref, tgt_gbin, lane, d.x, d.x + d.y, out.rbase[slot] + out.bbase[slot >> 10]);
-    }
+        filter_span(rows, out, src, lane, d.x, d.x + d.y, out.rbase[slot] + out.bbase[slot >> 10]);
+    }
+}
+
+template <typename Rows>
+struct FilterKernArgs4 {
+    const uint32_t* tgt_gbin;
+    const uint4* slots;
+    const uint32_t* span_bits;
+    const uint4* span;
+    uint32_t* redo;
+    uint32_t nslots, shift, no_entry;
+    Rows rows;
+    FilterOut out;
+    SpanTables tables;
+};
+
+constexpr uint32_t kNoRef = 0xffffffffu;
+
+template <typename KA>
+__device__ __forceinline__ uint32_t span_resolve(const KA& ka, uint32_t g, const uint4& e, uint32_t off_mask) {
+    const uint32_t off = g & off_mask, hi1 = e.z >> 16;
+    const bool in0 = (off >= (e.x & 0xffffu)) & (off <= (e.x >> 16));
+    const bool in1 = (off >= (e.z & 0xffffu)) & (off <= hi1);
+    uint32_t ref = in0 ? (e.y & ~kSpanMore) : in1 ? (e.w & ~kSpanMore) : kNoRef;
+    const bool miss = (off > hi1) & ((e.w & kSpanMore) != 0u);
+    if (__builtin_expect(k_ballot(miss) != 0ull, 0)) {
+        const SpanTables tb = kernarg_now<SpanTables>(ka, offsetof(KA, tables));
+        const uint32_t r = miss ? ref_of_bin(tb.bin_off, tb.n_refs, g & kW4BinMask, e.w & ~kSpanMore) : 0u;
+        const bool v = ((tb.valid_bits[r >> 5] >> (r & 31u)) & 1u) != 0u;
+        ref = (miss & v) ? r : ref;
+    }
+    return ref;
+}
+
+template <typename Rows>
+__global__ __launch_bounds__(64, 8) void k_filter_compact4(const FilterKernArgs4<Rows> ka) {
+    using KA = FilterKernArgs4<Rows>;
+    const uint32_t* __restrict__ const tgt_gbin = ka.tgt_gbin;
+    const uint32_t* __restrict__ const span_bits = ka.span_bits;
+    const uint4* __restrict__ const span = ka.span;
+    __shared__ uint32_t s_ref[kFcRing], s_g[kFcRing], s_r[kFcRing];
+    __shared__ __attribute__((aligned(16))) uint32_t s_sel[kFcReads];
+    const uint32_t lane = lane_id();
+    const uint32_t slot = blockIdx.x;
+    if (slot >= ka.nslots) return;
+    const uint4 d = ka.slots[slot];
+    const uint32_t rb = ka.out.rbase[slot] + ka.out.bbase[slot >> 10];
+    const uint32_t t0 = d.x, tend = d.x + d.y;
+    const uint32_t shift = ka.shift, off_mask = (1u << shift) - 1u;
+    bool whole_reads_walk = d.z > kFcReads;
+    if (!whole_reads_walk)
+        for (uint32_t r = 4u * lane; r < d.z; r += 256u) *reinterpret_cast<uint4*>(&s_sel[r]) = make_uint4(~0u, ~0u, ~0u, ~0u);
+    __builtin_amdgcn_wave_barrier();
+    uint32_t rcount = 0, ccount = 0, cdone = 0;
+    uint32_t g1[kFcBatch], g2[kFcBatch], b1[kFcBatch];
+    auto ask = [&](uint32_t t, uint32_t (&to)[kFcBatch]) {
+        if (t + 64u * kFcBatch <= tend) {
+            const uint32_t* pg = tgt_gbin + t;
+#pragma unroll
+            for (uint32_t u = 0; u < kFcBatch; ++u) to[u] = pg[lane + 64u * u];
+            __builtin_amdgcn_sched_barrier(0);
+        } else {
+#pragma unroll
+            for (uint32_t u = 0; u < kFcBatch; ++u) to[u] = tgt_gbin[min(t + 64u * u + lane, tend - 1u)];
+        }
+    };
+    auto ask_bits = [&]() {
+#pragma unroll
+        for (uint32_t u = 0; u < kFcBatch; ++u) b1[u] = span_bits[(g1[u] & kW4BinMask) >> (shift + 5u)];
+    };
+    if (!whole_reads_walk && t0 < tend) {
+        ask(t0, g1);
+        if (t0 + 64u * kFcBatch < tend) ask(t0 + 64u * kFcBatch, g2);
+        __builtin_amdgcn_sched_barrier(0);
+        ask_bits();
+    }
+    for (uint32_t t = t0; t < tend && !whole_reads_walk; t += 64u * kFcBatch) {
+        uint32_t g[kFcBatch], rf[kFcBatch];
+        uint4 e[kFcBatch];
+#pragma unroll
+        for (uint32_t u = 0; u < kFcBatch; ++u) {
+            g[u] = g1[u];
+            const uint32_t blk = (g[u] & kW4BinMask) >> shift;
+            e[u] = span[((b1[u] >> (blk & 31u)) & 1u) != 0u ? blk : ka.no_entry];
+        }
+        __builtin_amdgcn_sched_barrier(0);
+        if (t + 64u * kFcBatch < tend) {
+#pragma unroll
+            for (uint32_t u = 0; u < kFcBatch; ++u) g1[u] = g2[u];
+            ask_bits();
+        }
+        __builtin_amdgcn_sched_barrier(0);
+        if (t + 128u * kFcBatch < tend) ask(t + 128u * kFcBatch, g2);
+        __builtin_amdgcn_sched_barrier(0);
+#pragma unroll
+        for (uint32_t u = 0; u < kFcBatch; ++u) rf[u] = span_resolve(ka, g[u], e[u], off_mask);
+        __builtin_amdgcn_sched_barrier(0);
+        const bool full = t + 64u * kFcBatch <= tend;
+        const uint32_t nchunks = full ? kFcBatch : (tend - t + 63u) >> 6;
+#pragma unroll 1
+        for (uint32_t u = 0; u < nchunks; ++u) {
+            const uint32_t tu = t + 64u * u;
+            uint32_t gu, ref;
+            auto pick = [&](uint32_t gk, uint32_t rk) {
+                SLIMM_PIN_VGPR(gk);
+                gu = gk;
+                ref = rk;
+            };
+            if (full) {
+                if (u < 2u) {
+                    if (u == 0u) pick(g[0], rf[0]);
+                    else pick(g[1], rf[1]);
+                } else {
+                    if (u == 2u) pick(g[2], rf[2]);
+                    else pick(g[3], rf[3]);
+                }
+            } else {
+                gu = g[0], ref = rf[0];
+#pragma unroll
+                for (uint32_t k = 1; k < kFcBatch; ++k) {
+                    gu = u == k ? g[k] : gu;
+                    ref = u == k ? rf[k] : ref;
+                }
+            }
+            const bool live = full || tu + lane < tend;
+            const uint64_t H = k_ballot(live && (gu & kW4Head) != 0u);
+            const bool valid = live && ref != kNoRef;
+            const uint64_t VB = k_ballot(valid);
+            if (k_bit(VB)) {
+                const uint32_t p = __builtin_amdgcn_mbcnt_hi(static_cast<uint32_t>(VB >> 32),
+                                                             __builtin_amdgcn_mbcnt_lo(static_cast<uint32_t>(VB), ccount)) & (kFcRing - 1u);
+                s_ref[p] = ref;
+                s_g[p] = gu & kW4BinMask;
+                s_r[p] = __builtin_amdgcn_mbcnt_hi(static_cast<uint32_t>(H >> 32),
+                                                   __builtin_amdgcn_mbcnt_lo(static_cast<uint32_t>(H), rcount - 1u)) + (k_bit(H) ? 1u : 0u);
+            }
+            rcount += static_cast<uint32_t>(__popcll(H));
+            ccount += static_cast<uint32_t>(__popcll(VB));
+            const bool last = tu + 64u >= tend;
+            while (ccount - cdone >= 64u || (last && ccount != cdone)) {
+                __builtin_amdgcn_wave_barrier();
+                const uint32_t n_live = min(64u, ccount - cdone);
+                const uint32_t en = (cdone + lane) & (kFcRing - 1u);
+                const uint32_t cref = lane < n_live ? s_ref[en] : 0u;
+                const uint32_t cg = s_g[en], cr = lane < n_live ? s_r[en] : 0xffffffffu;
+                typename Rows::Row row = ka.rows.load(cref);
+                const uint32_t before = __builtin_amdgcn_update_dpp(0xffffffffu, cr, 0x138, 0xf, 0xf, false);
+                const uint64_t Hc = k_ballot(lane < n_live && (lane == 0u || cr != before));
+                const bool final_window = last && ccount - cdone <= 64u;
+                const uint32_t X = final_window ? n_live : 63u - static_cast<uint32_t>(__builtin_clzll(Hc));
+                __builtin_amdgcn_wave_barrier();
+                if (__builtin_expect(X == 0u, 0)) {
+                    whole_reads_walk = true;
+                    break;
+                }
+                compact_window<Rows>(ka, lane, X, Hc, cref, cg, cr, row, s_sel);
+                cdone += X;
+            }
+            if (__builtin_expect(whole_reads_walk, 0)) break;
+        }
+    }
+    __builtin_amdgcn_wave_barrier();
+    if (__builtin_expect(whole_reads_walk, 0)) {
+        uint32_t* const redo = kernarg_now<uint32_t*>(ka, offsetof(KA, redo));
+        uint32_t* const counters = kernarg_now<uint32_t*>(ka, offsetof(KA, out.counters));
+        if (lane == 0u) redo[atomicAdd(&counters[CNT_REDO], 1u)] = slot;
+    } else {
+        for (uint32_t r = lane; r < d.z; r += 64u) ka.out.sel[rb + r] = s_sel[r];
+    }
+}
+
+__global__ __launch_bounds__(256) void k_span_build(const SpanTables t, uint32_t* __restrict__ bits, uint4* __restrict__ span) {
+    const uint32_t b = blockIdx.x * 256u + threadIdx.x;
+    const uint2 none = make_uint2(0xffffu, 0u);
+    uint2 e0 = none, e1 = none;
+    uint32_t found = 0;
+    if (b < t.nblocks) {
+        const uint32_t total = t.bin_off[t.n_refs];
+        const uint32_t first = b << t.shift;
+        const uint32_t end = min(first + (1u << t.shift), total);
+        for (uint32_t r = ref_of_bin_any(t.bin_off, t.n_refs, first); r < t.n_refs && found < 3u; ++r) {
+            const uint32_t lo = t.bin_off[r], hi = t.bin_off[r + 1u];
+            if (lo >= end) break;
+            if (hi <= lo || hi <= first || ((t.valid_bits[r >> 5] >> (r & 31u)) & 1u) == 0u) continue;
+            const uint2 en = make_uint2((max(lo, first) - first) | ((min(hi, end) - 1u - first) << 16), r);
+            if (found == 0u) e0 = en;
+            if (found == 1u) e1 = en;
+            ++found;
+        }
+        if (found >= 2u) e0.y |= kSpanMore;
+        if (found >= 3u) e1.y |= kSpanMore;
+        span[b] = make_uint4(e0.x, e0.y, e1.x, e1.y);
+    }
+    if (b == 0u) span[t.nblocks] = make_uint4(none.x, none.y, none.x, none.y);
+    const uint64_t flagged = k_ballot(found != 0u);
+    if ((threadIdx.x & 63u) == 0u && b < t.nblocks) {
+        bits[b >> 5] = static_cast<uint32_t>(flagged);
+        bits[(b >> 5) + 1u] = static_cast<uint32_t>(flagged >> 32);
+    }
+}
+void launch_span_build(hipStream_t st, const SpanTables& t, uint32_t* bits, uint4* span) {
+    hipLaunchKernelGGL(k_span_build, dim3((t.nblocks + 255u) / 256u), dim3(256), 0, st, t, bits, span);
 }
 
 __global__ __launch_bounds__(256) void k_check_grouping(const uint64_t* __restrict__ key, uint32_t n, uint64_t id_mask,
@@ -724,10 +967,10 @@
 }
 
 void launch_hist(hipStream_t st, const uint32_t* tgt_gbin, const uint4* slots, uint32_t nslots, uint32_t* counters,
-                 uint32_t* tail, uint32_t* cov, uint32_t* ucov, bool count_mapped) {
+                 uint32_t* tail, uint32_t* cov, uint32_t* ucov, bool count_mapped, uint32_t vmask) {
     uint32_t blocks = std::max(1u, std::min((nslots + kWaves - 1) / kWaves, 256u * 16u));
     hipLaunchKernelGGL(k_hist, dim3(blocks), dim3(kBlock), 0, st, tgt_gbin, slots, nslots, counters, tail, cov, ucov,
-                       count_mapped ? 1 : 0);
+                       count_mapped ? 1 : 0, vmask);
 }
 
 void launch_ref_stats(hipStream_t st, const uint32_t* a, const uint32_t* b, const uint32_t* bin_off, uint32_t n_refs,
@@ -886,11 +1129,19 @@
     auto launch = [&](const auto& r, auto ref_word) {
         using Rows = std::decay_t<decltype(r)>;
         using RefT = decltype(ref_word);
+        if (a.tgt_ref.word4) {
+            const FilterKernArgs4<Rows> ka{a.tgt_gbin, a.slots, a.span.bits, a.span.span, a.redo, a.nslots, a.span.shift,
+                                           a.span.nblocks, r, out, a.span};
+            hipExtLaunchKernelGGL((k_filter_compact4<Rows>), dim3(grid), dim3(64), 0, st, t0, t1, 0, ka);
+            hipLaunchKernelGGL((k_filter_walk<Rows, TgtOne>), dim3(std::min(a.nslots, 256u)), dim3(64), 0, st,
+                               TgtOne{a.tgt_gbin, a.span.bin_off, a.span.n_refs}, a.slots, a.redo, r, out);
+            return;
+        }
         const RefT* const tgt_ref = static_cast<const RefT*>(a.tgt_ref.p);
         const FilterKernArgs<Rows, RefT> ka{tgt_ref, a.tgt_gbin, a.slots, a.valid_bits, a.redo, a.nslots, r, out};
         hipExtLaunchKernelGGL((k_filter_compact<Rows, RefT>), dim3(grid), dim3(64), 0, st, t0, t1, 0, ka);
-        hipLaunchKernelGGL((k_filter_walk<Rows, RefT>), dim3(std::min(a.nslots, 256u)), dim3(64), 0, st, tgt_ref, a.tgt_gbin, a.slots,
-                           a.redo, r, out);
+        hipLaunchKernelGGL((k_filter_walk<Rows, TgtTwo<RefT>>), dim3(std::min(a.nslots, 256u)), dim3(64), 0, st,
+                           TgtTwo<RefT>{tgt_ref, a.tgt_gbin}, a.slots, a.redo, r, out);
     };
     if (a.rows16) {
         Rows16 r;
diff --git a/slimm_amd/csrc/span_plan.h b/slimm_amd/csrc/span_plan.h
--- /dev/null
+++ b/slimm_amd/csrc/span_plan.h
@@ -0,0 +1,24 @@
+#pragma once
+#include <cstdint>
+
+namespace slimm {
+
+constexpr uint32_t kSpanMinShift = 2;
+constexpr uint32_t kSpanShiftLimit = 16;
+
+inline bool word4_fits(uint64_t bp_plus_tpad, uint64_t limit) { return bp_plus_tpad < limit; }
+
+inline uint32_t span_shift(uint64_t total_bins, uint32_t n_refs, long forced = 0) {
+    if (forced > 0) {
+        const uint32_t f = static_cast<uint32_t>(forced);
+        return f < kSpanMinShift ? kSpanMinShift : f > kSpanShiftLimit ? kSpanShiftLimit : f;
+    }
+    uint32_t s = kSpanMinShift;
+    while (s < kSpanShiftLimit && ((total_bins + (1ull << s) - 1ull) >> s) > n_refs) ++s;
+    return s;
+}
+inline uint32_t span_blocks(uint64_t total_bins, uint32_t shift) {
+    return static_cast<uint32_t>((total_bins + (1ull << shift) - 1ull) >> shift);
+}
+
+}
diff --git a/slimm_amd/csrc/tile_hist.hip b/slimm_amd/csrc/tile_hist.hip
--- a/slimm_amd/csrc/tile_hist.hip
+++ b/slimm_amd/csrc/tile_hist.hip
@@ -162,7 +162,14 @@
     return n_a != 0u;
 }
 
-__device__ __forceinline__ uint32_t tile_of(uint32_t v) { return (v & 0x7fffffffu) >> kTileShift; }
+__device__ __forceinline__ uint32_t index_field(uint32_t v, uint32_t from, uint32_t width) {
+#if defined(__HIP_DEVICE_COMPILE__)
+    return __builtin_amdgcn_ubfe(v, from, width);
+#else
+    return (v >> from) & ((1u << width) - 1u);
+#endif
+}
+__device__ __forceinline__ uint32_t tile_of(uint32_t v, uint32_t vbits) { return index_field(v, kTileShift, vbits - kTileShift); }
 
 template <int kMode>
 __global__ __launch_bounds__(kTBlock * kCountFold) void k_tile_count(const uint32_t* __restrict__ vals, const uint4* __restrict__ slots,
@@ -170,7 +177,7 @@
                                                         uint32_t* __restrict__ tile_count_all, uint32_t reps,
                                                         uint32_t rep_stride, uint4* __restrict__ part,
                                                         uint32_t* __restrict__ matrix, uint32_t S,
-                                                        const uint32_t* __restrict__ gate) {
+                                                        const uint32_t* __restrict__ gate, uint32_t vbits) {
     HIP_DYNAMIC_SHARED(uint32_t, s_hist)
     __shared__ uint32_t s_sum[3];
     if (kMode == 2 && *gate == 0u) return;
@@ -222,7 +229,7 @@
         if (!any) break;
 #pragma unroll
         for (int u = 0; u < 16; ++u)
-            if (v[u] != 0xffffffffu) atomicAdd(&s_hist[tile_of(v[u])], 1u);
+            if (v[u] != 0xffffffffu) atomicAdd(&s_hist[tile_of(v[u], vbits)], 1u);
     }
     if (kMode != 1 && part && lane == 0u) {
         atomicAdd(&s_sum[0], w.sum_v);
@@ -524,7 +531,7 @@
 __device__ __forceinline__ void scatter_round_ordered(const uint32_t (&v)[kRoundPieces], uint32_t ntiles,
                                                       const uint32_t* s_mine, uint32_t* __restrict__ tile_cursor,
                                                       uint16_t* __restrict__ bucket, uint32_t* s_cnt, uint32_t* s_loff,
-                                                      uint32_t* s_stage, uint32_t* s_wtot) {
+                                                      uint32_t* s_stage, uint32_t* s_wtot, uint32_t vbits) {
     const uint32_t tid = threadIdx.x;
     TPROF_T(p0);
     for (uint32_t i = tid; i < kTileSlots; i += kTBlock) s_cnt[i] = 0;
@@ -533,7 +540,7 @@
     TPROF_ADD(1, p0, p1);
     uint32_t r[kRoundPieces];
 #pragma unroll
-    for (int k = 0; k < kRoundPieces; ++k) r[k] = v[k] != 0xffffffffu ? atomicAdd(&s_cnt[tile_of(v[k])], 1u) : 0u;
+    for (int k = 0; k < kRoundPieces; ++k) r[k] = v[k] != 0xffffffffu ? atomicAdd(&s_cnt[tile_of(v[k], vbits)], 1u) : 0u;
     __syncthreads();
     TPROF_T(p2);
     TPROF_ADD(2, p1, p2);
@@ -560,7 +567,7 @@
 #pragma unroll
     for (int k = 0; k < kRoundPieces; ++k) {
         if (v[k] == 0xffffffffu) continue;
-        const uint32_t t = tile_of(v[k]);
+        const uint32_t t = tile_of(v[k], vbits);
         s_stage[s_loff[t] + r[k]] = (t << kEntryBits) | entry_of(v[k]);
     }
     __syncthreads();
@@ -579,13 +586,13 @@
 __device__ __forceinline__ void scatter_round_direct(const uint32_t (&v)[kPieces], uint32_t ntiles,
                                                      const uint32_t* __restrict__ tile_base,
                                                      uint32_t* __restrict__ tile_cursor, uint16_t* __restrict__ bucket,
-                                                     uint32_t* s_hist, uint32_t last) {
+                                                     uint32_t* s_hist, uint32_t last, uint32_t vbits) {
     constexpr int kMaxTilesPerThread = 8;
     for (uint32_t i = threadIdx.x; i < ntiles; i += kTBlock) s_hist[i] = 0;
     __syncthreads();
 #pragma unroll
     for (int k = 0; k < kPieces; ++k)
-        if (v[k] != 0xffffffffu) atomicAdd(&s_hist[tile_of(v[k])], 1u);
+        if (v[k] != 0xffffffffu) atomicAdd(&s_hist[tile_of(v[k], vbits)], 1u);
     __syncthreads();
     for (uint32_t i0 = 0; i0 < ntiles; i0 += kMaxTilesPerThread * kTBlock) {
         uint32_t got[kMaxTilesPerThread];
@@ -606,7 +613,7 @@
 #pragma unroll
     for (int k = 0; k < kPieces; ++k) {
         if (v[k] == 0xffffffffu) continue;
-        const uint32_t pos = atomicAdd(&s_hist[tile_of(v[k])], 1u);
+        const uint32_t pos = atomicAdd(&s_hist[tile_of(v[k], vbits)], 1u);
         bucket[min(pos, last)] = static_cast<uint16_t>(entry_of(v[k]));
     }
     __syncthreads();
@@ -651,7 +658,7 @@
                                                           uint32_t* __restrict__ ucov,
                                                           const uint32_t* __restrict__ rep_base_all, uint32_t reps,
                                                           uint32_t rep_stride, uint32_t tile_sub, uint32_t last,
-                                                          const uint32_t* __restrict__ gate) {
+                                                          const uint32_t* __restrict__ gate, uint32_t vbits) {
     HIP_DYNAMIC_SHARED(uint32_t, s_hist)
     __shared__ uint32_t s_more[kTBlock / 64];
     if (gate && *gate == 0u) return;
@@ -662,7 +669,7 @@
     zero_split_tiles(tile_base, ntiles, cov, ucov, tile_sub);
     SlotWalk walk = slot_walk(slots, nslots, per_read != 0, 1, lid);
     bucketing_rounds<kDirectPieces, false>(walk, vals, s_more, [&](const uint32_t (&v)[kDirectPieces]) {
-        scatter_round_direct(v, ntiles, rep_base, tile_cursor, bucket, s_hist, last);
+        scatter_round_direct(v, ntiles, rep_base, tile_cursor, bucket, s_hist, last, vbits);
     });
 }
 
@@ -673,7 +680,7 @@
 constexpr int kBigPieces = SLIMM_BIG_PIECES;
 constexpr uint32_t kBigRound = kBigBlock * kBigPieces;
 static_assert(kBigPieces % 8 == 0, "values come four to a lane; the rounds' LDS operations in batches of eight");
-template <int kE>
+template <int kE, uint32_t kBits>
 __global__ __launch_bounds__(kBigBlock) void k_tile_scatter_big(const uint32_t* __restrict__ vals, const uint4* __restrict__ slots,
                                                                 uint32_t nslots, int per_read, uint32_t ntiles,
                                                                 const uint32_t* __restrict__ tile_base,
@@ -683,6 +690,7 @@
                                                                 const uint32_t* __restrict__ rep_base_all, uint32_t reps,
                                                                 uint32_t rep_stride, uint32_t tile_sub, uint32_t last,
                                                                 const uint32_t* __restrict__ gate) {
+    constexpr uint32_t vbits = kBits;
     HIP_DYNAMIC_SHARED(uint32_t, s_dyn)
     __shared__ uint32_t s_more[kBigBlock / 64], s_wtot[kBigBlock / 64];
     constexpr uint32_t kNoTile = kE * kBigBlock;
@@ -725,7 +733,7 @@
         for (int k0 = 0; k0 < kBigPieces; k0 += 8) {
             uint32_t r[8];
 #pragma unroll
-            for (int k = 0; k < 8; ++k) r[k] = atomicAdd(&s_tab[v[k0 + k] != 0xffffffffu ? tile_of(v[k0 + k]) : no_tile], 1u);
+            for (int k = 0; k < 8; ++k) r[k] = atomicAdd(&s_tab[v[k0 + k] != 0xffffffffu ? tile_of(v[k0 + k], vbits) : no_tile], 1u);
 #pragma unroll
             for (int k = 0; k < 8; k += 2) r2[(k0 + k) / 2] = r[k] | (r[k + 1] << 16);
             __builtin_amdgcn_sched_barrier(0);
@@ -776,10 +784,10 @@
         for (int k0 = 0; k0 < kBigPieces; k0 += 8) {
             uint32_t at_[8];
 #pragma unroll
-            for (int k = 0; k < 8; ++k) at_[k] = s_tab[v[k0 + k] != 0xffffffffu ? tile_of(v[k0 + k]) : no_tile];
+            for (int k = 0; k < 8; ++k) at_[k] = s_tab[v[k0 + k] != 0xffffffffu ? tile_of(v[k0 + k], vbits) : no_tile];
 #pragma unroll
             for (int k = 0; k < 8; ++k) {
-                const uint32_t t = tile_of(v[k0 + k]);
+                const uint32_t t = tile_of(v[k0 + k], vbits);
                 const uint32_t rk = (k & 1) ? r2[(k0 + k) / 2] >> 16 : r2[(k0 + k) / 2] & 0xffffu;
                 s_stage[v[k0 + k] != 0xffffffffu ? at_[k] + rk : kBigRound + lane] = (t << kEntryBits) | entry_of(v[k0 + k]);
             }
@@ -827,7 +835,8 @@
 __global__ __launch_bounds__(kTBlock * kCountFold) void k_tile_scatter_matrix(
     const uint32_t* __restrict__ vals, const uint4* __restrict__ slots, uint32_t nslots, int per_read, uint32_t ntiles,
     const uint32_t* __restrict__ tile_base, const uint32_t* __restrict__ matrix, uint32_t row_stride,
-    uint16_t* __restrict__ bucket, uint32_t* __restrict__ cov, uint32_t* __restrict__ ucov, uint32_t tile_sub) {
+    uint16_t* __restrict__ bucket, uint32_t* __restrict__ cov, uint32_t* __restrict__ ucov, uint32_t tile_sub,
+    uint32_t vbits) {
     HIP_DYNAMIC_SHARED(uint32_t, s_cur)
     const uint32_t* __restrict__ row = matrix + static_cast<size_t>(blockIdx.x) * row_stride;
     for (uint32_t i = threadIdx.x; i < ntiles; i += kTBlock * kCountFold) s_cur[i] = tile_base[i] + row[i];
@@ -849,7 +858,7 @@
 #pragma unroll
         for (int u = 0; u < 8; ++u) {
             if (v[u] == 0xffffffffu) continue;
-            const uint32_t pos = atomicAdd(&s_cur[tile_of(v[u])], 1u);
+            const uint32_t pos = atomicAdd(&s_cur[tile_of(v[u], vbits)], 1u);
             bucket[pos] = static_cast<uint16_t>(entry_of(v[u]));
         }
     }
@@ -898,7 +907,8 @@
                                                                 uint32_t* __restrict__ ucov, uint32_t rep_stride,
                                                                 uint4* __restrict__ items, uint32_t* __restrict__ split_tiles,
                                                                 const uint4* __restrict__ part, uint32_t nparts,
-                                                                uint32_t* __restrict__ tail, uint32_t tile_sub) {
+                                                                uint32_t* __restrict__ tail, uint32_t tile_sub,
+                                                                uint32_t vbits) {
     __shared__ uint32_t s_stage[kRoundCap];
     __shared__ uint32_t s_mine[kFusedTiles];
     __shared__ uint32_t s_cnt[kFusedTiles];
@@ -974,7 +984,7 @@
     TPROF_T(q1);
     TPROF_ADD(0, q0, q1);
     bucketing_rounds(walk, vals, s_more, [&](const uint32_t (&v)[kRoundPieces]) {
-        scatter_round_ordered(v, ntiles, s_mine, tile_cursor, bucket, s_cnt, s_loff, s_stage, s_wtot);
+        scatter_round_ordered(v, ntiles, s_mine, tile_cursor, bucket, s_cnt, s_loff, s_stage, s_wtot, vbits);
     });
     TPROF_T(q2);
     TPROF_ADD(7, q0, q2);
@@ -985,7 +995,7 @@
                                                         const uint32_t* __restrict__ tile_base,
                                                         uint32_t* __restrict__ sup_cursor, uint32_t* __restrict__ mid,
                                                         uint32_t* __restrict__ cov, uint32_t* __restrict__ ucov,
-                                                        uint32_t tile_sub) {
+                                                        uint32_t tile_sub, uint32_t vbits) {
     __shared__ uint32_t s_cur[kMaxSuper];
     __shared__ uint32_t s_more[kTBlock / 64];
     const uint32_t nsup = (ntiles + kSuperTiles - 1) / kSuperTiles;
@@ -996,7 +1006,7 @@
         __syncthreads();
 #pragma unroll
         for (int k = 0; k < kRoundPieces; ++k)
-            if (v[k] != 0xffffffffu) atomicAdd(&s_cur[(v[k] & 0x7fffffffu) >> kSuperShift], 1u);
+            if (v[k] != 0xffffffffu) atomicAdd(&s_cur[index_field(v[k], kSuperShift, vbits - kSuperShift)], 1u);
         __syncthreads();
         for (uint32_t i = threadIdx.x; i < nsup; i += kTBlock) {
             const uint32_t h = s_cur[i];
@@ -1006,9 +1016,8 @@
 #pragma unroll
         for (int k = 0; k < kRoundPieces; ++k) {
             if (v[k] == 0xffffffffu) continue;
-            const uint32_t g = v[k] & 0x7fffffffu;
-            const uint32_t pos = atomicAdd(&s_cur[g >> kSuperShift], 1u);
-            mid[pos] = (g & kSuperMask) | ((v[k] >> 31) << kSuperShift);
+            const uint32_t pos = atomicAdd(&s_cur[index_field(v[k], kSuperShift, vbits - kSuperShift)], 1u);
+            mid[pos] = (v[k] & kSuperMask) | ((v[k] >> 31) << kSuperShift);
         }
         __syncthreads();
     });
@@ -1549,18 +1558,21 @@
     if (hipFuncSetAttribute(reinterpret_cast<const void*>(k_tile_scatter_matrix), hipFuncAttributeMaxDynamicSharedMemorySize,
                             static_cast<int>(bytes)) != hipSuccess)
         return -1;
-    if (hipFuncSetAttribute(reinterpret_cast<const void*>(k_tile_scatter_big<kBigE>), hipFuncAttributeMaxDynamicSharedMemorySize,
-                            static_cast<int>(big_lds_bytes(kBigE))) != hipSuccess)
-        return -1;
+    for (auto* k : {k_tile_scatter_big<kBigE, 31u>, k_tile_scatter_big<kBigE, 30u>})
+        if (hipFuncSetAttribute(reinterpret_cast<const void*>(k), hipFuncAttributeMaxDynamicSharedMemorySize,
+                                static_cast<int>(big_lds_bytes(kBigE))) != hipSuccess)
+            return -1;
     return 0;
 }
+
+static uint32_t value_bits(const SlotValues& in) { return in.mask == kW4BinMask ? 30u : 31u; }
 
 void launch_tile_count(hipStream_t st, uint32_t grid, uint32_t ntiles, const SlotValues& in, const TileTables& t, bool totals,
                        bool matrix, const TileSample& sm) {
     auto* const k = sm.gated ? k_tile_count<2> : sm.stride > 1u ? k_tile_count<1> : k_tile_count<0>;
     hipLaunchKernelGGL(k, dim3(tile_count_grid(grid)), dim3(kTBlock * kCountFold), static_cast<size_t>(ntiles) * 4, st, in.vals, in.slots,
                        in.nslots, in.per_read ? 1 : 0, ntiles, t.tile_count, t.reps, t.stride, totals ? t.tot_part : nullptr,
-                       matrix ? t.matrix : nullptr, sm.stride, t.counters + sm.flag);
+                       matrix ? t.matrix : nullptr, sm.stride, t.counters + sm.flag, value_bits(in));
 }
 
 void launch_matrix_prefix(hipStream_t st, uint32_t grid, uint32_t ntiles, const TileTables& t) {
@@ -1592,24 +1604,25 @@
     case TilePath::Fused:
         hipLaunchKernelGGL(k_tile_scatter_fused, dim3(grid), dim3(kTBlock), 0, st, in.vals, in.slots, in.nslots, per_read,
                            t.counters, ntiles, t.tile_count, t.tile_cursor, t.bucket, cov, ucov, t.stride, t.tile_items,
-                           t.split_tiles, tot.part, tot.nparts, tot.tail, tile_sub);
+                           t.split_tiles, tot.part, tot.nparts, tot.tail, tile_sub, value_bits(in));
         break;
     case TilePath::OrderedRounds:
-        hipLaunchKernelGGL(k_tile_scatter_big<kBigE>, dim3(tile_count_grid(grid)), dim3(kBigBlock), big_lds_bytes(kBigE), st,
+        hipLaunchKernelGGL((value_bits(in) == 30u ? k_tile_scatter_big<kBigE, 30u> : k_tile_scatter_big<kBigE, 31u>),
+                           dim3(tile_count_grid(grid)), dim3(kBigBlock), big_lds_bytes(kBigE), st,
                            in.vals, in.slots, in.nslots, per_read, ntiles, t.tile_base, t.tile_cursor, t.bucket, cov, ucov,
                            t.tile_count, t.reps, t.stride, tile_sub, last, gate);
         break;
     case TilePath::DirectRounds:
         hipLaunchKernelGGL(k_tile_scatter, dim3(grid), dim3(kTBlock), lds, st, in.vals, in.slots, in.nslots, per_read, ntiles,
-                           t.tile_base, t.tile_cursor, t.bucket, cov, ucov, t.tile_count, t.reps, t.stride, tile_sub, last, gate);
+                           t.tile_base, t.tile_cursor, t.bucket, cov, ucov, t.tile_count, t.reps, t.stride, tile_sub, last, gate, value_bits(in));
         break;
     case TilePath::Matrix:
         hipLaunchKernelGGL(k_tile_scatter_matrix, dim3(tile_count_grid(grid)), dim3(kTBlock * kCountFold), lds, st, in.vals,
-                           in.slots, in.nslots, per_read, ntiles, t.tile_base, t.matrix, t.stride, t.bucket, cov, ucov, tile_sub);
+                           in.slots, in.nslots, per_read, ntiles, t.tile_base, t.matrix, t.stride, t.bucket, cov, ucov, tile_sub, value_bits(in));
         break;
     case TilePath::TwoLevel:
         hipLaunchKernelGGL(k_part_super, dim3(grid), dim3(kTBlock), 0, st, in.vals, in.slots, in.nslots, per_read, ntiles,
-                           t.tile_base, t.sup_cursor, t.mid, cov, ucov, tile_sub);
+                           t.tile_base, t.sup_cursor, t.mid, cov, ucov, tile_sub, value_bits(in));
         hipLaunchKernelGGL(k_part_tile, dim3(part_items_upper(ntiles, n_upper)), dim3(kTBlock), 0, st, t.mid, t.part_items,
                            t.counters, t.tile_base, t.tile_cursor, ntiles, t.bucket);
         break;
diff --git a/slimm_amd/profiler.py b/slimm_amd/profiler.py
--- a/slimm_amd/profiler.py
+++ b/slimm_amd/profiler.py
@@ -600,6 +600,9 @@
 
     def target_ref_bits(self) -> int:
         return self.L.slimm_target_ref_bits(self.ctx)
+
+    def target_bytes(self) -> int:
+        return self.L.slimm_target_bytes(self.ctx)
 
     def bucket_sampling(self) -> Dict[str, Dict[str, int]]:
         v = np.zeros(6, dtype=np.uint32)
```

Result: slower. 115,500 (-1.5%).
